# OllieBoyne/FIND

Hardware: AMD Instinct MI355X
Metric: deformed vertices x rendered views / sec (fwd+bwd) (higher is better)
Workload: dtype f32; 1 GPU; train_3d.yaml network-stage step: 16 feet x 6890-vertex template per GPU, 10002-vertex GT scans, chamf(5000)+smooth+texture(1000) losses, backward, Adam(main_params) step; nothing rendered, views:=1; feet_per_gpu=16, template_verts=6890, parallelism=dp1

## Files before the change

find_amd/_lib.py:

```python
import ctypes
import os
from ctypes import POINTER, Structure, c_char_p, c_float, c_int, c_int16, c_int32, c_int64, c_void_p

_PKG = os.path.dirname(os.path.abspath(__file__))
LIB_PATH = os.path.join(_PKG, 'lib', 'libfind_hip.so')
MAX_LAYERS = 8
ABI_VERSION = 3

_lib = None


class MlpParams(Structure):
	_fields_ = [
		('width', c_int32), ('in_dim', c_int32), ('pe_size', c_int32), ('n_trunk', c_int32),
		('n_disp', c_int32), ('n_col', c_int32), ('lat_disp', c_int32), ('lat_col', c_int32),
		('B', c_void_p),
		('trunk_w', c_void_p * MAX_LAYERS), ('trunk_b', c_void_p * MAX_LAYERS),
		('disp_w', c_void_p * MAX_LAYERS), ('disp_b', c_void_p * MAX_LAYERS),
		('col_w', c_void_p * MAX_LAYERS), ('col_b', c_void_p * MAX_LAYERS),
		('avg_col', c_void_p),
		('precision', c_int32),
	]


class MlpGrads(Structure):
	_fields_ = [
		('trunk_w', c_void_p * MAX_LAYERS), ('trunk_b', c_void_p * MAX_LAYERS),
		('disp_w', c_void_p * MAX_LAYERS), ('disp_b', c_void_p * MAX_LAYERS),
		('col_w', c_void_p * MAX_LAYERS), ('col_b', c_void_p * MAX_LAYERS),
		('lat_disp', c_void_p), ('lat_col', c_void_p),
	]


class RenderParams(Structure):
	_fields_ = [
		('image_h', c_int32), ('image_w', c_int32), ('fov_deg', c_float), ('znear', c_float), ('zfar', c_float),
		('sil_blur_radius', c_float), ('sil_sigma', c_float), ('sil_faces_per_pixel', c_int16), ('clip_faces', c_int16),
		('rgb_sigma', c_float), ('rgb_gamma', c_float), ('background', c_float * 3), ('light_pos', c_float * 3),
		('ambient', c_float), ('diffuse', c_float), ('specular', c_float), ('shininess', c_float), ('z_clip', c_float),
	]


class PointsParams(Structure):
	_fields_ = [('image_h', c_int32), ('image_w', c_int32), ('fov_deg', c_float), ('radius', c_float), ('points_per_pixel', c_int32)]


_P = c_void_p
_I = c_int64
PROTOTYPES = {
	'find_abi_version': (c_int, []),
	'find_last_error': (c_char_p, []),
	'find_build_arch': (c_char_p, []),
	'find_ctx_create': (c_int, [c_int, POINTER(c_void_p)]),
	'find_ctx_destroy': (c_int, [_P]),
	'find_ctx_stream_groups': (c_int, [_P, _P, _P]),
	'find_ctx_stream_beside': (c_int, [_P, _P, _P, c_int32, c_int32, _P]),
	'find_ctx_set': (c_int, [_P, c_char_p, _I]),
	'find_ctx_get': (c_int, [_P, c_char_p, POINTER(c_int64)]),
	'find_ctx_join': (c_int, [_P, _P]),
	'find_render_switches': (c_int, [_I]),
	'find_mlp_ws_bytes': (c_int64, [POINTER(MlpParams), _I, _I, _I, c_int]),
	'find_mlp_fwd': (c_int, [_P, POINTER(MlpParams), _P, _I, _I, _I, _P, _P, _P, _P, _P, _I, c_int, _P]),
	'find_mlp_bwd_scratch_bytes': (c_int64, [POINTER(MlpParams), _I, _I, _I]),
	'find_mlp_bwd': (c_int, [_P, POINTER(MlpParams), _P, _I, _I, _I, _P, _P, _P, _P, _P, _I, _P, _I, POINTER(MlpGrads), _P]),
	'find_linear_relu_fwd': (c_int, [_P, _P, _P, _P, _I, _I, _P, _P]),
	'find_linear_wgrad_scratch_bytes': (c_int64, [_I]),
	'find_linear_wgrad': (c_int, [_P, _P, _P, _I, _I, _P, _P, _P, _I, _P]),
	'find_latent_gather_fwd': (c_int, [_P, _I, _I, _P, _I, _P, _P]),
	'find_latent_gather_bwd': (c_int, [_P, _P, _I, _I, _I, _P, _P]),
	'find_latent_gather_many_fwd': (c_int, [_I, _P, _P, _P, _P, _I, _P, _P]),
	'find_latent_gather_many_bwd': (c_int, [_I, _P, _P, _P, _P, _I, _P, _P]),
	'find_weighted_terms_fwd': (c_int, [_I, _P, _P, _P, _P, _P]),
	'find_weighted_terms_bwd': (c_int, [_I, _P, _P, _P, _P, _P]),
	'find_contrastive_fwd': (c_int, [_P, _I, _I, _P, _I, _P, _I, c_float, _P, _P, _P]),
	'find_contrastive_bwd': (c_int, [_P, _I, _I, _P, _I, _P, _P, _P, _P]),
	'find_part_labels': (c_int, [_P, _I, _I, _I, _I, _I, _I, _P, _P]),
	'find_part_ce_fwd': (c_int, [_P, _P, _P, _I, _I, _P, _P, _P, _I, _P]),
	'find_part_ce_bwd': (c_int, [_P, _P, _P, _I, _I, _P, _P, _P, _I, _P]),
	'find_vertex_normals_fwd': (c_int, [_P, _P, _I, _P, _P, _I, _I, _I, _P, _P]),
	'find_vertex_normals_bwd': (c_int, [_P, _P, _I, _P, _P, _I, _I, _I, _P, _P, _P, _P]),
	'find_normal_map_fwd': (c_int, [_P, _P, _I, _I, _I, _I, c_int, _P, _P]),
	'find_normal_map_bwd': (c_int, [_P, _P, _P, _I, _I, _I, _I, c_int, _P, _P]),
	'find_normal_loss_ws_bytes': (c_int64, [_I]),
	'find_normal_loss_fwd': (c_int, [_P, _P, _P, _I, _P, _P, _I, _P]),
	'find_normal_loss_bwd': (c_int, [_P, _P, _P, _I, _P, _P, _P, _P]),
	'find_point_face_ws_bytes': (c_int64, [_I, _I]),
	'find_point_face_fwd': (c_int, [_P, _P, _P, _P, _I, _I, _I, _I, _I, _P, _P, _P, _P, _I, _P]),
	'find_point_face_bwd': (c_int, [_P, _P, _P, _I, _P, _P, _P, _I, _I, _I, _I, _P, _P, _P]),
	'find_uv_sample': (c_int, [_P, _I, _I, _I, _P, _I, _P, _I, _I, _P, _P, _I, _I, _P, _P]),
	'find_render_frags': (c_int, [POINTER(RenderParams), _I, _I, _I, _I, _P, _P, _P, _P]),
	'find_adam_step': (c_int, [_I, _P, _P, _P, _P, _P, c_float, c_float, c_float, c_float, c_float, _I, _P]),
	'find_adam_step_dev': (c_int, [_I, _P, _P, _P, _P, _P, c_float, c_float, c_float, c_float, c_float, _P, _P]),
	'find_sgd_step': (c_int, [_I, _P, _P, _P, _P, c_float, c_float, c_float, c_float, c_int, c_int, _P]),
	'find_register_fwd': (c_int, [_P, _I, _P, _P, _I, _I, _P, _P]),
	'find_register_bwd_ws_bytes': (c_int64, [_I, _I]),
	'find_register_bwd': (c_int, [_P, _I, _P, _P, _P, _I, _I, _P, _P, _P, _I, _P]),
	'find_pca_fwd': (c_int, [_P, _I, _I, _P, _I, _P, _P]),
	'find_pca_bwd_ws_bytes': (c_int64, [_I, _I, _I]),
	'find_pca_bwd': (c_int, [_P, _I, _I, _P, _I, _P, _P, _I, _P]),
	'find_sample_points_fwd': (c_int, [_P, _P, _I, _P, _P, _I, _I, _I, _I, _P, _P, _P, _P]),
	'find_sample_points_bwd': (c_int, [_P, _I, _P, _P, _P, _I, _I, _I, _I, _P, _P]),
	'find_face_areas': (c_int, [_P, _P, _I, _I, _I, _I, _P, _P]),
	'find_nn_fwd': (c_int, [_P, _P, _P, _P, _I, _I, _I, _P, _P, _P]),
	'find_nn_bwd': (c_int, [_P, _P, _P, _P, _P, _I, _I, _I, _P, _P, _P]),
	'find_sample_surface_ws_bytes': (c_int64, [_I, _I]),
	'find_sample_surface_fwd': (c_int, [_P, _P, _I, _P, _I, _I, _I, _I, _P, _P, _P, _P, _P, _P, _I, _P]),
	'find_sample_surface_again': (c_int, [_P, _P, _I, _P, _I, _I, _I, _I, _P, _P, _P, _P, _P, _P, _I, _P]),
	'find_chamfer_ws_bytes': (c_int64, [_I, _I, _I]),
	'find_chamfer_fwd': (c_int, [_P, _P, _P, _P, _I, _I, _I, _P, _P, _I, _P]),
	'find_chamfer_bwd': (c_int, [_P, _P, _P, _P, _I, _I, _I, _P, _P, _I, _P, _P, _P]),
	'find_masked_mse_fwd': (c_int, [_P, _P, _I, _P, _P]),
	'find_masked_mse_bwd': (c_int, [_P, _P, _I, _P, _P, _P]),
	'find_image_mse_ws_bytes': (c_int64, []),
	'find_image_mse_fwd': (c_int, [_P, _P, _P, _P, _I, _I, _P, _P, _I, _P]),
	'find_image_mse_bwd': (c_int, [_P, _P, _P, _P, _I, _I, _P, _P, _P, _P]),
	'find_image_metrics_ws_bytes': (c_int64, [_I, _I]),
	'find_image_metrics': (c_int, [_P, _P, _P, _P, _P, _P, _I, _I, _I, _P, _P, _I, _P]),
	'find_smooth_loss_fwd': (c_int, [_P, _P, _P, _P, _P, _P, _I, _I, _I, _I, c_float, c_float, _P, _P, _I, _P]),
	'find_smooth_loss_bwd': (c_int, [_P, _P, _P, _P, _P, _P, _I, _I, _I, _I, c_float, c_float, _P, _P, _I, _P, _P]),
	'find_smooth_ws_bytes': (c_int64, [_I, _I, _I]),
	'find_smooth_fwd': (c_int, [_P, _P, _P, _P, _P, _P, _I, _I, _I, _I, _P, _P, _P, _I, _P]),
	'find_smooth_bwd': (c_int, [_P, _P, _P, _P, _P, _P, _I, _I, _I, _I, _P, _P, _P, _I, _P, _P]),
	'find_render_ws_bytes': (c_int64, [POINTER(RenderParams), _I, _I, _I, _I]),
	'find_render_fwd': (c_int, [POINTER(RenderParams), _P, _P, _I, _P, _P, _P, _I, _I, _I, _I, _P, _P, _P, _P, _P, _I, _P]),
	'find_render_bwd': (c_int, [POINTER(RenderParams), _P, _P, _I, _P, _P, _P, _I, _I, _I, _I, _P, _P, _P, _P, _P, _P, _I, _P]),
	'find_render_flags': (c_int, [_P, _P, _P]),
	'find_render_features_ws_bytes': (c_int64, [POINTER(RenderParams), _I, _I, _I]),
	'find_render_features_fwd': (c_int, [POINTER(RenderParams), _P, _P, _I, _P, _P, _I, _I, _I, _I, _P, _I, _P, _P, _I, _P, _I, _P]),
	'find_render_features_bwd': (c_int, [POINTER(RenderParams), _P, _P, _I, _P, _P, _I, _I, _I, _I, _P, _I, _P, _P, _P, _P, _P, _I, _P, _I, _P]),
	'find_points_render': (c_int, [POINTER(PointsParams), _P, _P, _P, _P, _I, _I, _I, _P, _P, _P, _P, _P]),
	'find_frames_u8': (c_int, [_P, _I, _I, _I, _I, c_int, _P, _P]),
}


def lib():
	global _lib
	if _lib is not None:
		return _lib
	if not os.path.exists(LIB_PATH):
		raise RuntimeError(f'find_amd: HIP library not built: {LIB_PATH} is missing. Run `python -m find_amd.build` '
						   '(or __graft_entry__.build()). There is no CPU fallback.')
	import torch
	L = ctypes.CDLL(LIB_PATH)
	for name, (res, args) in PROTOTYPES.items():
		try:
			fn = getattr(L, name)
		except AttributeError as e:
# ... 91 lines not shown
```

find_amd/csrc/mlp.hip:

```cpp
#include "mlp_dw2.h"
#include "mlp_dw4.h"
#include "mlp_dwpe.h"
#include "mlp_dwpe6.h"
#include "mlp_gemm5.h"
#include "mlp_gemm6.h"
#include "mlp_gemm7.h"
#include "mlp_dw3.h"
#include "mlp_dw6.h"
#include "mlp_gemm4.h"
#include "mlp_fused.h"
#include "mlp_fused6.h"
#include "mlp_ctx.h"

namespace find {
namespace mlp {

struct Dims {
	int64_t pos_batch, n_feet, V;
	bool shared;
	int64_t rows_t;
	int64_t rows_h;
	int64_t feet_t;
	int nchunk0;
	int nkt0;
// ... 43 lines not shown

static int64_t chain_w6_bytes(const find_mlp_params* p) {
	const int64_t steps = 2 * (KP0 / KC + 1) + 16 * (int64_t)(p->n_trunk + p->n_disp + p->n_col + 4);
	return 8 * steps * F6_STEP_BYTES;
}

struct FwdWs {
	float* w0p;
	float* wd0;
	float* wc0;
	float* fbd;
	float* fbc;
	float* H[FIND_MAX_LAYERS];
	float* D[FIND_MAX_LAYERS];
	float* C[FIND_MAX_LAYERS];
	float* zd;
	float* zc;
	float* hp;
	float* hp2;
	void* w6;
	int64_t bytes;
};

static void carve_fwd(const find_mlp_params* p, const Dims& d, bool save, void* ws, FwdWs* o) {
	Carver c(ws);
	o->w0p = c.take<float>((int64_t)W * KP0);
	o->wd0 = c.take<float>((int64_t)W * W);
	o->wc0 = c.take<float>((int64_t)W * W);
	o->fbd = c.take<float>(d.n_feet * W);
	o->fbc = c.take<float>(d.n_feet * W);
	o->zd = c.take<float>(d.rows_h * 3);
	o->zc = c.take<float>(d.rows_h * 3);
	o->hp = (d.shared && d.n_feet > 1) ? c.take<float>(d.V * W) : nullptr;
	o->hp2 = (d.shared && d.n_feet > 1) ? c.take<float>(d.V * W) : nullptr;
	o->w6 = c.take<char>(chain_w6_bytes(p));
	float* pt[2] = {nullptr, nullptr};
	float* pd[2] = {nullptr, nullptr};
	float* pc[2] = {nullptr, nullptr};
	for (int i = 0; i < p->n_trunk; ++i) {
		if (save || !pt[i & 1]) pt[i & 1] = c.take<float>(d.rows_t * W);
		o->H[i] = pt[i & 1];
	}
	for (int i = 0; i < p->n_disp; ++i) {
		if (save || !pd[i & 1]) pd[i & 1] = c.take<float>(d.rows_h * W);
		o->D[i] = pd[i & 1];
	}
	for (int i = 0; i < p->n_col; ++i) {
		if (save || !pc[i & 1]) pc[i & 1] = c.take<float>(d.rows_h * W);
		o->C[i] = pc[i & 1];
	}
	o->bytes = c.off;
}

static void split_policy(int64_t n_feet, int64_t V, int* spf, int* cps, int64_t target = 128) {
	const int64_t cpf = cdiv(V, 32);
	int64_t s0 = std::max<int64_t>(1, std::min<int64_t>(cpf, cdiv(target, n_feet)));
	*cps = (int)cdiv(cpf, s0);
	*spf = (int)cdiv(cpf, *cps);
}

struct BwdWs {
	float* Tt[FIND_MAX_LAYERS];
	float* Dt[FIND_MAX_LAYERS];
	float* Ct[FIND_MAX_LAYERS];
	float* dzD[FIND_MAX_LAYERS];
	float* dzC[FIND_MAX_LAYERS];
	float* dzT[FIND_MAX_LAYERS];
	float* pw;
	float* pb;
	float* pw_t[4];
	float* pb_t[4];
	float* Sd;
	float* Sc;
	float* zsD;
	float* zsC;
	float* fs1D;
	float* fs1C;
	float* pS;
	float* pS2;
	int nblk_fs;
	float* pwo[2];
	float* pbo[2];
	int nblk_out;
	int64_t max_split;
	float* grp_pw;
	int64_t grp_slabs;
	int grp_jobs;
	void* w6;
	int64_t bytes;
};

constexpr int64_t GROUP_MAX_UNITS = 1024;
constexpr int GROUP_MIN_CPS = 8;

static void carve_bwd(const find_mlp_params* p, const Dims& d, void* scratch, BwdWs* o) {
	Carver c(scratch);
	for (int i = 1; i < p->n_trunk; ++i) o->Tt[i] = c.take<float>((int64_t)W * W);
	for (int i = 0; i < p->n_disp; ++i) o->Dt[i] = c.take<float>((int64_t)W * W);
	for (int i = 0; i < p->n_col; ++i) o->Ct[i] = c.take<float>((int64_t)W * W);
	for (int i = 0; i < std::max(p->n_disp, 1); ++i) o->dzD[i] = c.take<float>(d.rows_h * W);
	for (int i = 0; i < std::max(p->n_col, 1); ++i) o->dzC[i] = c.take<float>(d.rows_h * W);
	for (int i = 0; i < std::max(p->n_trunk, 1); ++i) o->dzT[i] = c.take<float>(d.rows_t * W);
	int spf, cps;
	split_policy(d.n_feet, d.V, &spf, &cps);
	int64_t ms = d.n_feet * spf;
	split_policy(1, d.V, &spf, &cps);
	ms = std::max<int64_t>(ms, spf);
	o->max_split = ms;
	const int64_t ms2 = std::max<int64_t>(512, d.n_feet) + d.n_feet + 16;
	o->pw = c.take<float>(std::max<int64_t>(ms * W * KP0, ms2 * W * W));
	o->pb = c.take<float>(std::max<int64_t>(ms, ms2) * W);
	o->pw_t[0] = o->pw; o->pb_t[0] = o->pb;
	for (int i = 1; i < 4; ++i) {
		o->pw_t[i] = c.take<float>(ms2 * W * W);
		o->pb_t[i] = c.take<float>(ms2 * W);
	}
	o->Sd = c.take<float>(d.n_feet * W);
	o->Sc = c.take<float>(d.n_feet * W);
	o->nblk_fs = (int)cdiv(d.V, FS_ROWS);
	if (d.shared) {
		o->zsD = c.take<float>(d.V * W);
		o->zsC = c.take<float>(d.V * W);
		o->fs1D = c.take<float>(d.V * W);
		o->fs1C = c.take<float>(d.V * W);
	} else {
		o->zsD = o->zsC = o->fs1D = o->fs1C = nullptr;
	}
	o->pS = c.take<float>((int64_t)o->nblk_fs * d.n_feet * W);
	o->pS2 = c.take<float>((int64_t)o->nblk_fs * d.n_feet * W);
	o->w6 = c.take<char>(chain_w6_bytes(p));
	o->grp_pw = nullptr; o->grp_slabs = 0; o->grp_jobs = 0;
	if (cdiv(d.V, 32) * d.feet_t <= GROUP_MAX_UNITS) {
		o->grp_jobs = d.shared ? (p->n_trunk - 1) + 2 : (p->n_trunk - 1) + p->n_disp + p->n_col;
		o->grp_slabs = std::max<int64_t>(d.feet_t * (cdiv(d.V / 16, GROUP_MIN_CPS) + 1), std::min<int64_t>(d.feet_t * cdiv(d.V / 16, 2), 32));
		if (o->grp_jobs > 0) o->grp_pw = c.take<float>((int64_t)o->grp_jobs * o->grp_slabs * ((int64_t)W * W + W));
	}
	o->nblk_out = (int)std::max<int64_t>(1, std::min<int64_t>(cdiv(d.rows_h, 64), 512));
	for (int i = 0; i < 2; ++i) {
		o->pwo[i] = c.take<float>((int64_t)o->nblk_out * 3 * W);
		o->pbo[i] = c.take<float>((int64_t)o->nblk_out * 4);
	}
	o->bytes = c.off;
}

struct TileLaunch { int id; int lds; int rows; int grid; int block; };

static int ntiles_of(int64_t V, int rows, int64_t feet) { return (int)((int)cdiv(V, rows) * feet); }

template <typename K>
static int launch_tiles(find_ctx* c, K kernel, const TileLaunch& t, Gemm2Args a, int64_t feet, hipStream_t s) {
	int lds = 0;
	FIND_TRY(prepare_kernel(c, t.id, kernel, t.lds, &lds));
	a.tiles_per_foot = (int)cdiv(a.V, t.rows);
	a.ntiles = (int)(a.tiles_per_foot * feet);
	hipLaunchKernelGGL(kernel, dim3(t.grid), dim3(t.block), lds, s, a);
	return FIND_OK;
}

template <typename F>
static int with_epi(int epi, F&& f) {
	if (epi == EPI_BIAS_RELU) return f(std::integral_constant<int, EPI_BIAS_RELU>{});
	if (epi == EPI_MASK) return f(std::integral_constant<int, EPI_MASK>{});
	return f(std::integral_constant<int, EPI_NONE>{});
}
constexpr int epi_slot(int epi) { return epi == EPI_BIAS_RELU ? 0 : epi == EPI_MASK ? 1 : 2; }

static int launch_gemm2_pe(find_ctx* c, const Gemm2Args& a, int64_t feet, hipStream_t s) {
	constexpr int BM = 64;
	const int grid = std::min(ntiles_of(a.V, BM, feet), c->num_cus);
	return launch_tiles(c, &gemm2_kernel<BM, AMODE_PE, EPI_BIAS_RELU>, TileLaunch{K_GEMM2_PE, gemm2_lds_bytes<BM>(), BM, grid, 256}, a, feet, s);
}

static int launch_gemm3(find_ctx* c, int epi, const Gemm2Args& a, int64_t feet, hipStream_t s) {
	return with_epi(epi, [&](auto E) -> int {
		constexpr int EPI = decltype(E)::value, BM = 64;
		const int grid = std::min(ntiles_of(a.V, BM, feet), c->num_cus);
		return launch_tiles(c, &gemm3_kernel<BM, EPI>, TileLaunch{K_GEMM3_RELU + epi_slot(EPI), gemm2_lds_bytes<BM>(), BM, grid, 256}, a, feet, s);
	});
}

template <int NI>
static int launch_gemm4(find_ctx* c, int epi, const Gemm2Args& a, int64_t feet, hipStream_t s) {
	return with_epi(epi, [&](auto E) -> int {
		constexpr int EPI = decltype(E)::value, NW = 8;
		constexpr int G = 8 * (8 / NI);
		const int grid = std::max(G, (c->num_cus / G) * G);
		const int id = (NI == 4 ? K_GEMM4_4_RELU : K_GEMM4_2_RELU) + epi_slot(EPI);
		return launch_tiles(c, &gemm4_kernel<EPI, NI, NW>, TileLaunch{id, NI * 32 * 1024, 32, grid, NW * 64}, a, feet, s);
	});
}

static int launch_gemm5(find_ctx* c, int epi, const Gemm2Args& a, int64_t feet, hipStream_t s, bool h16) {
	return with_epi(epi, [&](auto E) -> int {
		constexpr int EPI = decltype(E)::value;
		const int grid = (int)std::min<int64_t>(c->num_cus, cdiv(ntiles_of(a.V, 32, feet), GEMM5_NW));
		const int block = GEMM5_NW * 64;
		if constexpr (EPI != EPI_NONE) {
			if (h16 && (EPI == EPI_BIAS_RELU ? a.va_bias : a.vm_bias)) {
				Gemm2Args v = a;
				v.tile_major = 1;
				return launch_tiles(c, &gemm5_kernel<EPI, true, true>, TileLaunch{EPI == EPI_BIAS_RELU ? K_GEMM5_RELU_V : K_GEMM5_MASK_V, GEMM5_LDS_VIRT, 32, grid, block}, v, feet, s);
			}
			if (h16) return launch_tiles(c, &gemm5_kernel<EPI, true>, TileLaunch{EPI == EPI_BIAS_RELU ? K_GEMM5_RELU_H : K_GEMM5_MASK_H, GEMM5_LDS, 32, grid, block}, a, feet, s);
		} else if (h16) {
			set_error("launch_gemm5: no fp16-stored variant of this epilogue");
			return FIND_EINVAL;
		}
		return launch_tiles(c, &gemm5_kernel<EPI>, TileLaunch{K_GEMM5_RELU + epi_slot(EPI), GEMM5_LDS, 32, grid, block}, a, feet, s);
	});
}

static int gemm7_fsum_pairs(const find_ctx* c, int64_t V, int64_t feet) {
	const int64_t upf = cdiv(V, 32);
	const int def = std::max(16, (c->num_cus / 16) * 16) / 2;
	const int pairs = (int)std::min<int64_t>(def, (upf / 8) * 8);
	return (feet >= 2 && feet <= 64 && pairs >= 8) ? pairs : 0;
}

static int launch_gemm7(find_ctx* c, int epi, const Gemm2Args& a, int64_t feet, hipStream_t s) {
	return with_epi(epi, [&](auto E) -> int {
		constexpr int EPI = decltype(E)::value;
		const int grid = std::max(16, (c->num_cus / 16) * 16);
		const int block = GEMM7_NW * 64;
		if constexpr (EPI == EPI_MASK) {
// ... 62 lines not shown
		SplitWArgs sa;
		memset(&sa, 0, sizeof(sa));
		int maxn = 0;
		for (int i = 0; i < ch.a.n_steps; ++i) {
			const FusedStep& st = ch.a.step[i];
			if (st.kind != FS_GEMM) continue;
			const int n = 2 * st.nchunk;
			sa.job[sa.njobs++] = SplitWJob{st.w, st.ldw, n, sa.total, st.wmode, ch.a.pe, ch.in_dim};
			sa.total += n;
			maxn = std::max(maxn, n);
		}
		if (sa.njobs > 0 && 8 * (int64_t)sa.total * F6_STEP_BYTES <= w6_bytes) {
			sa.dst = reinterpret_cast<u32x4*>(w6);
			hipLaunchKernelGGL(split_w_kernel, dim3((unsigned)cdiv(8 * maxn * 64, 256), (unsigned)sa.njobs), dim3(256), 0, s, sa);
			FIND_LAUNCH_CHECK("split_w_kernel");
			ch.a.w6 = w6;
			ch.a.total_steps = sa.total;
			ch.x3 = true;
		}
	}
	if (!ch.x3)
		for (int i = 0; i < ch.a.n_steps; ++i)
			FIND_REQUIRE(ch.a.step[i].kind != FS_GEMM || ch.a.step[i].wmode == 0, "find_mlp: a chain with weights in model order did not get its bf16x3 kernel (chain_direct and chain_prepare disagree)");
	return FIND_OK;
}

static int chain_launch(find_ctx* c, Chain& ch, hipStream_t s) {
	const int nt = ch.nt;
	int lds = 0;
	if (ch.x3) {
		if (nt == 2) FIND_TRY(prepare_kernel(c, K_FUSED6_2, &fused6_kernel<2>, fused6_lds(2), &lds, false));
		else FIND_TRY(prepare_kernel(c, K_FUSED6, &fused6_kernel<1>, fused6_lds(1), &lds, false));
		if (nt == 2) hipLaunchKernelGGL(fused6_kernel<2>, dim3(ch.a.ntiles), dim3(FUSED_NW * 64), lds, s, ch.a);
		else hipLaunchKernelGGL(fused6_kernel<1>, dim3(ch.a.ntiles), dim3(FUSED_NW * 64), lds, s, ch.a);
		FIND_LAUNCH_CHECK("fused6_kernel");
		return FIND_OK;
	}
	const int grid = std::min(ch.a.ntiles, c->num_cus);
	if (nt == 2) FIND_TRY(prepare_kernel(c, K_FUSED2, &fused_chain_kernel<2>, fused_lds(2), &lds, false));
	else FIND_TRY(prepare_kernel(c, K_FUSED, &fused_chain_kernel<1>, fused_lds(1), &lds, false));
	if (nt == 2) hipLaunchKernelGGL(fused_chain_kernel<2>, dim3(grid), dim3(FUSED_NW * 64), lds, s, ch.a);
	else hipLaunchKernelGGL(fused_chain_kernel<1>, dim3(grid), dim3(FUSED_NW * 64), lds, s, ch.a);
	FIND_LAUNCH_CHECK("fused_chain_kernel");
	return FIND_OK;
}

static int launch_chain(find_ctx* c, Chain& ch, int64_t V, int64_t feet, hipStream_t s, void* w6 = nullptr, int64_t w6_bytes = 0) {
	if (!ch.prepared) FIND_TRY(chain_prepare(c, ch, V, feet, s, w6, w6_bytes));
	return chain_launch(c, ch, s);
}

static bool use_fused(const find_ctx* c, int64_t V, int64_t feet) {
	const int64_t units = cdiv(V, 32) * feet;
	if (c->f16 && units >= c->gemm5_min_units) return false;
	return c->fused_max_units > 0 && units <= c->fused_max_units;
}

static Gemm2Args gemm_args() {
	Gemm2Args a;
	memset(&a, 0, sizeof(a));
	a.nseg = 1;
	return a;
}

static Gemm2Args linear_args(const float* x, int64_t x_foot_stride, const float* w, int ldw, const float* bias, int64_t bias_foot_stride, float* y, int64_t V) {
	Gemm2Args a = gemm_args();
	a.a0 = x; a.a_foot_stride = x_foot_stride; a.lda = W;
	a.w0 = w; a.ldw = ldw; a.nchunk = W / KC;
	a.bias = bias; a.bias_foot_stride = bias_foot_stride;
	a.y = y; a.y_foot_stride = V * W; a.ldy = W; a.V = (int)V;
	return a;
}

static bool use_act16(const find_ctx* c, bool f16, bool shared, int64_t n_feet, int64_t V) {
	return f16 && c->act16 && shared && n_feet > 1 && cdiv(V, 32) * n_feet >= c->gemm5_min_units;
}
static bool use_fold(const find_ctx* c, bool a16, bool shared, int64_t n_feet, int64_t V, const find_mlp_params* p) {
	if (!c->bcast_fold || p->n_disp < 2 || p->n_col < 2) return false;
	if (a16) return true;
	const int64_t units = cdiv(V, 32) * n_feet;
	return c->x3 && !c->f16 && shared && n_feet > 1 && units >= c->gemm6_min_units;
}
static void note_act16(find_ctx* c, const void* ws, bool a16, bool fold) {
	for (auto& n : c->act16_notes) if (n.ws == ws) { n.a16 = a16; n.fold = fold; return; }
	c->act16_notes[c->act16_next] = find_ctx::Act16Note{ws, a16, fold};
	c->act16_next = (c->act16_next + 1) & 15;
}
static int noted_act16(const find_ctx* c, const void* ws, bool by_rule, bool fold_by_rule) {
	for (const auto& n : c->act16_notes) if (n.ws == ws) return (n.a16 ? 1 : 0) | (n.fold ? 2 : 0);
	return (by_rule ? 1 : 0) | (fold_by_rule ? 2 : 0);
}

static bool call_f16(const find_ctx* c, const find_mlp_params* p) { return p->precision == 2 || (p->precision == 0 && c->mlp_f16 == 1); }
static bool call_x3(const find_ctx* c, const find_mlp_params* p) { return p->precision == 3 || (p->precision == 0 && c->mlp_f16 == 2); }

struct Head {
	bool colour;
	int nl;
	const float* const* w;
	const float* const* b;
	int ld0;
	int L;
	const float* lat;
	const float* w0; int ldw0;
	float* fb;
	const float* bias0; int64_t bstride0;
	float* const* act;
	float* z;
	float* hp;
	float* out;
	const float* gout;
	float* const* gw; float* const* gb; float* glat;
	float* const* dz; int cur;
	float* const* wt;
	float* S; float* zs; float* fs1; float* pS;
	int side;
};

static void make_heads(Head* heads, const find_mlp_params* p, const FwdWs& w, const float* lat_disp, const float* lat_col, const BwdWs* b, const find_mlp_grads* g) {
	memset(heads, 0, 2 * sizeof(Head));
	Head& d = heads[0];
	Head& c = heads[1];
	c.colour = true;
	d.nl = p->n_disp; c.nl = p->n_col;
	d.w = p->disp_w; c.w = p->col_w;
	d.b = p->disp_b; c.b = p->col_b;
	d.L = p->lat_disp; c.L = p->lat_col;
	d.lat = lat_disp; c.lat = lat_col;
	d.w0 = w.wd0; c.w0 = w.wc0;
	d.fb = w.fbd; c.fb = w.fbc;
	d.act = w.D; c.act = w.C;
	d.z = w.zd; c.z = w.zc;
	d.hp = w.hp; c.hp = w.hp2;
	for (int k = 0; k < 2; ++k) {
		Head& h = heads[k];
		h.ld0 = W + h.L;
		h.ldw0 = W;
		h.bias0 = h.L > 0 ? h.fb : h.b[0];
		h.bstride0 = h.L > 0 ? W : 0;
		h.side = 1 + k;
	}
	if (!b) return;
	d.gw = g->disp_w; c.gw = g->col_w;
	d.gb = g->disp_b; c.gb = g->col_b;
	d.glat = g->lat_disp; c.glat = g->lat_col;
	d.dz = b->dzD; c.dz = b->dzC;
	d.wt = b->Dt; c.wt = b->Ct;
	d.S = b->Sd; c.S = b->Sc;
	d.zs = b->zsD; c.zs = b->zsC;
	d.fs1 = b->fs1D; c.fs1 = b->fs1C;
	d.pS = b->pS; c.pS = b->pS2;
}

static int mlp_fwd_body(Fork& fk, const find_mlp_params* p, const Dims& d, const FwdWs& w, const float* pos, Head* heads) {
	find_ctx* c = fk.c;
	hipStream_t s = fk.s;
	const int64_t V = d.V, n_feet = d.n_feet;
	Head& hd = heads[0];
	Head& hc = heads[1];
	const bool a16 = use_act16(c, c->f16, d.shared, n_feet, V);
	const bool fold = use_fold(c, a16, d.shared, n_feet, V, p);
	note_act16(c, w.fbd, a16, fold);

	const bool fused = use_fused(c, V, d.feet_t) && p->pe_size > 0;
	const bool direct = fused && chain_direct(c);
	if (!direct) {
		RepackArgs ra;
		memset(&ra, 0, sizeof(ra));
		ra.njobs = 3;
		ra.job[0] = RepackJob{p->trunk_w[0], w.w0p, W, KP0, p->in_dim + 2 * p->pe_size, 0, KP0, 2, p->pe_size, p->in_dim};
		ra.job[1] = RepackJob{hd.w[0], w.wd0, W, W, hd.ld0, 0, W, 0, 0, 0};
		ra.job[2] = RepackJob{hc.w[0], w.wc0, W, W, hc.ld0, 0, W, 0, 0, 0};
		hipLaunchKernelGGL(repack_kernel, dim3(96, ra.njobs), dim3(256), 0, s, ra);
		FIND_LAUNCH_CHECK("repack_kernel");
	} else {
		for (int k = 0; k < 2; ++k) { heads[k].w0 = heads[k].w[0]; heads[k].ldw0 = heads[k].ld0; }
	}
	for (int k = 0; k < 2; ++k) {
		const Head& h = heads[k];
		if (h.L > 0 && h.out != nullptr)
			hipLaunchKernelGGL(latent_bias_kernel, dim3(W / 4, (unsigned)n_feet), dim3(256), 0, s, h.w[0], h.ld0, h.b[0], h.lat, h.L, h.fb);
	}
	FIND_LAUNCH_CHECK("latent_bias_kernel");

	const bool forked = hd.out && hc.out && fk.on;
	if (!(fold || forked || (fused && hd.out))) hc.hp = w.hp;

	const bool fused_heads = fused && !(d.shared && n_feet > 1);
	if (fused) {
		Chain ch;
		ch.a.pos = pos; ch.a.pos_foot_stride = V * 3; ch.a.Bm = p->B; ch.a.pe = p->pe_size; ch.in_dim = p->in_dim;
		{
			FusedStep& s0 = direct ? ch.gemm(p->trunk_w[0], p->in_dim + 2 * p->pe_size, (d.nchunk0 + 1) & ~1) : ch.gemm(w.w0p, KP0, (d.nchunk0 + 1) & ~1);
			s0.wmode = direct ? 2 : 0;
			s0.src_kind = FS_SRC_PE; s0.relu = 1; s0.bias = p->trunk_b[0]; s0.dst = w.H[0]; s0.to_lds = 1;
		}
		for (int i = 1; i < p->n_trunk; ++i) {
			FusedStep& st = ch.gemm(p->trunk_w[i], W, W / KC);
			st.relu = 1; st.bias = p->trunk_b[i]; st.dst = w.H[i]; st.to_lds = 1;
		}
		const float* hlast = w.H[p->n_trunk - 1];
		if (!fused_heads) {
			for (int k = 0; k < 2; ++k)
				if (heads[k].out) { FusedStep& st = ch.gemm(heads[k].w0, heads[k].ldw0, W / KC); st.dst = heads[k].hp; }
		} else {
			auto head = [&](const Head& h, bool reload) {
				FusedStep& f0 = ch.gemm(h.w0, h.ldw0, W / KC, reload ? hlast : nullptr);
				f0.relu = 1; f0.bias = h.bias0; f0.bias_foot_stride = (int)h.bstride0; f0.dst = h.act[0]; f0.to_lds = 1;
				for (int i = 1; i < h.nl; ++i) {
					FusedStep& st = ch.gemm(h.w[i], W, W / KC);
					st.relu = 1; st.bias = h.b[i]; st.dst = h.act[i]; st.to_lds = 1;
				}
				FusedStep& o = ch.add();
				o.kind = FS_OUT; o.w = h.w[h.nl]; o.bias = h.b[h.nl]; o.dst = h.out; o.dst2 = h.z; o.head = (unsigned char)h.colour;
				o.aux = h.colour ? p->avg_col : nullptr;
			};
			if (hd.out) head(hd, false);
			if (hc.out) head(hc, hd.out != nullptr);
		}
		FIND_TRY(launch_chain(c, ch, V, d.feet_t, s, w.w6, chain_w6_bytes(p)));
		if (fused_heads) return FIND_OK;
	} else {
		Gemm2Args a = gemm_args();
		a.pos = pos; a.pos_foot_stride = V * 3; a.Bm = p->B; a.pe = p->pe_size;
		a.w0 = w.w0p; a.ldw = KP0; a.nchunk = d.nchunk0;
		a.bias = p->trunk_b[0]; a.bias_foot_stride = 0;
		a.y = w.H[0]; a.y_foot_stride = V * W; a.ldy = W; a.V = (int)V;
		FIND_TRY(launch_gemm(c, AMODE_PE, EPI_BIAS_RELU, a, d.feet_t, s));
		for (int i = 1; i < p->n_trunk; ++i)
			FIND_TRY(launch_gemm(c, AMODE_MAT, EPI_BIAS_RELU, linear_args(w.H[i - 1], V * W, p->trunk_w[i], W, p->trunk_b[i], 0, w.H[i], V), d.feet_t, s));
		FIND_LAUNCH_CHECK("trunk gemm");
	}

	const float* hl = w.H[p->n_trunk - 1];
	const int64_t hl_stride = d.shared ? 0 : V * W;
	auto head_first = [&](const Head& h, hipStream_t st) -> int {
		if (h.hp) {
			if (!fused) {
				Gemm2Args a = gemm_args();
				a.a0 = hl; a.a_foot_stride = 0; a.lda = W;
				a.w0 = h.w0; a.ldw = W; a.nchunk = W / KC;
				a.y = h.hp; a.y_foot_stride = V * W; a.ldy = W; a.V = (int)V;
				FIND_TRY(launch_gemm(c, AMODE_MAT, EPI_NONE, a, 1, st));
			}
			if (fold) return FIND_OK;
			hipLaunchKernelGGL(bias_relu_bcast_kernel, dim3((unsigned)cdiv(V * (W / 4), 256), (unsigned)cdiv(n_feet, BCAST_FEET)), dim3(256), 0, st, h.hp, h.bias0,
							   h.bstride0, (int)n_feet, V, h.act[0], a16 ? 1 : 0);
			return FIND_OK;
		}
		FIND_REQUIRE(!a16, "find_mlp_fwd: act16 without a shared template");
		return launch_gemm(c, AMODE_MAT, EPI_BIAS_RELU, linear_args(hl, hl_stride, h.w0, W, h.bias0, h.bstride0, h.act[0], V), n_feet, st);
	};
	auto head_out = [&](int head, hipStream_t st) {
		HeadOutArgs h;
		memset(&h, 0, sizeof(h));
		for (int k = 0; k < 2; ++k) {
			h.x[k] = heads[k].act[heads[k].nl - 1];
			h.w[k] = heads[k].w[heads[k].nl];
			h.b[k] = heads[k].b[heads[k].nl];
			h.z[k] = heads[k].z;
			h.out[k] = heads[k].out;
		}
		h.avg_col = p->avg_col;
		h.rows = d.rows_h;
		h.head0 = head;
		h.x_half = a16 ? 1 : 0;
		const unsigned gx = (unsigned)std::min<int64_t>(cdiv(d.rows_h, 32), 2048);
		if (a16) hipLaunchKernelGGL(head_out_fwd_h16_kernel, dim3(gx, 1), dim3(256), 0, st, h);
		else hipLaunchKernelGGL(head_out_fwd_kernel, dim3(gx, 1), dim3(256), 0, st, h);
	};
	auto head = [&](const Head& h, hipStream_t st) -> int {
		FIND_TRY(head_first(h, st));
		for (int i = 1; i < h.nl; ++i) {
			Gemm2Args a = linear_args(h.act[i - 1], V * W, h.w[i], W, h.b[i], 0, h.act[i], V);
			if (i == 1 && fold) {
				a.a0 = h.hp; a.a_foot_stride = 0;
				a.va_bias = h.bias0; a.va_bias_stride = h.bstride0;
			}
			FIND_TRY(launch_gemm(c, AMODE_MAT, EPI_BIAS_RELU, a, n_feet, st, a16));
		}
		head_out(h.colour, st);
		return FIND_OK;
	};
	hipStream_t sc = s;
	if (forked) {
		fk.fork_to(1);
		sc = fk.stream(1);
	}
	if (hd.out) FIND_TRY(head(hd, s));
	if (hc.out) FIND_TRY(head(hc, sc));
	FIND_LAUNCH_CHECK("head layers");
	return FIND_OK;
}

struct Wgrad {
	const float* dz = nullptr;
	const float* x = nullptr;
	int64_t x_foot_stride = 0;
	const float* pos = nullptr;
	int64_t pos_foot_stride = 0;
	int nkt = 1;
	int64_t feet = 1, V = 0;
	float* dw = nullptr;
	int ld_out = W;
	int k_valid = W;
	int pe_map = 0;
	float* db = nullptr;
	float* S = nullptr;
	hipStream_t s = nullptr;
	int s_side = -1;
	int reduce_side = -1;
	bool h16 = false;
	const float* vx_bias = nullptr;
	int64_t vx_bias_stride = 0;
};

struct Slabs { float* pw; float* pb; };
static Slabs slabs(const BwdWs& b, int k) { return Slabs{b.pw_t[k], b.pb_t[k]}; }

static int reduce_lds(find_ctx* c) {
	if (c->reduce_exclusive != 1) return 0;
	const int dyn = c->lds_bytes - 16 * 1024 - 256;
	if (!c->attr_done[K_REDUCE]) {
		if (hipFuncSetAttribute(reinterpret_cast<const void*>(&reduce_w_kernel), hipFuncAttributeMaxDynamicSharedMemorySize, dyn) != hipSuccess) return 0;
		c->attr_done[K_REDUCE] = true;
	}
	return dyn;
}

static int launch_reduce(find_ctx* c, const ReduceWArgs& r, hipStream_t s) {
	const unsigned grid = (unsigned)(r.nwblk + (r.pb ? r.n_feet + 1 : 0));
	if (c->reduce_exclusive == 2) hipLaunchKernelGGL(reduce_w_nolds_kernel, dim3(grid), dim3(1024), 0, s, r);
	else hipLaunchKernelGGL(reduce_w_kernel, dim3(grid), dim3(1024), reduce_lds(c), s, r);
	FIND_LAUNCH_CHECK("reduce_w_kernel");
	return FIND_OK;
}

static int weight_grad(find_ctx* c, Fork* fk, const find_mlp_params* p, const Wgrad& in, Slabs sl) {
	const int64_t feet = in.feet, V = in.V;
	hipStream_t s = in.s;
	FIND_REQUIRE(!in.vx_bias || (!in.pos && ((in.h16 && c->f16) || (!c->f16 && c->x3 && cdiv(V, 32) * feet >= c->gemm6_min_units))),
				 "weight_grad: a virtual operand reached a kernel that cannot form it (bcast_fold and the kernel selection disagree)");
	float* pbuf = (in.db || in.S) ? sl.pb : nullptr;
	const int cus = c->num_cus;
	int nsplit, spf, Kp = 256;
	if (!in.pos) {
		auto dw3_args = [&](int cpf, int cps) {
			Dw3Args a;
			memset(&a, 0, sizeof(a));
			a.dz = in.dz; a.dz_foot_stride = V * W; a.x = in.x; a.x_foot_stride = in.x_foot_stride;
			a.V = (int)V; a.chunks_per_foot = cpf; a.spf = spf; a.cps = cps; a.pw = sl.pw; a.pb = pbuf;
			a.xbias = in.vx_bias; a.xbias_stride = in.vx_bias_stride;
// ... 76 lines not shown
	memset(&r, 0, sizeof(r));
	r.pw = sl.pw; r.nsplit = nsplit; r.Kp = Kp; r.out = in.dw; r.ld_out = in.ld_out; r.K_valid = in.k_valid;
	if (in.pos) { r.pe_map = in.pe_map; r.pe = p->pe_size; r.in_dim = p->in_dim; }
	r.pb = pbuf; r.n_feet = (int)feet; r.spf = spf; r.db = in.db; r.S = in.S;
	r.nwblk = 256 * Kp / 4 / 64;
	hipStream_t rs = s;
	if (fk && fk->on && in.reduce_side >= 0 && in.s_side >= 0 && in.reduce_side != in.s_side) {
		fk->chain(in.s_side, in.reduce_side);
		rs = fk->stream(in.reduce_side);
	}
	return launch_reduce(c, r, rs);
}

struct WgradGroup {
	Dw2Group d;
	Dw6Group d6;
	bool x3 = false;
	ReduceWGroup r;
	int n = 0, nmain = 0;
	int live_jobs = 0;
	int64_t feet = 0;
	WgradGroup() { memset(&d, 0, sizeof(d)); memset(&d6, 0, sizeof(d6)); memset(&r, 0, sizeof(r)); }
};

static void group_geometry(const find_ctx* c, int cpf16, int64_t feet, int jobs, int64_t max_slabs, int* spf_out, int* cps_out) {
	auto take = [&](int s) { *cps_out = (int)cdiv(cpf16, s); *spf_out = (int)cdiv(cpf16, *cps_out); };
	const int s_max = (int)std::max<int64_t>(1, std::min<int64_t>(cpf16, max_slabs / std::max<int64_t>(feet, 1)));
	double best = 1e30;
	take(1);
	for (int s = 1; s <= s_max; ++s) {
		const int cps = (int)cdiv(cpf16, s);
		if ((int)cdiv(cpf16, cps) != s || (cps < 2 && s > 1)) continue;
		const int64_t wgs = feet * s * std::max(jobs, 1);
		const double cost = (double)cdiv(wgs, c->num_cus) * (cps * 3.6 + 6.0) + wgs * 0.06;
		if (cost < best) { best = cost; take(s); }
	}
}

static int wgrad_group_add(find_ctx* c, WgradGroup& G, const BwdWs& b, const Wgrad& in) {
	FIND_REQUIRE(G.n < b.grp_jobs && G.n < DW2_MAX_JOBS && G.n < DW6_MAX_JOBS, "find_mlp_bwd: too many grouped weight gradients");
	const int64_t feet = in.feet, V = in.V;
	G.x3 = c->x3 && c->dw_lds_free == 1;
	const int cpf16 = G.x3 ? (int)cdiv(V, 16) : (int)(V / 16);
	int spf = 1, cps2 = 1;
	if (cpf16 > 0) group_geometry(c, cpf16, feet, G.live_jobs > 0 ? G.live_jobs : b.grp_jobs, b.grp_slabs, &spf, &cps2);
	const int nmain = (int)(feet * spf);
	FIND_REQUIRE(nmain <= b.grp_slabs, "find_mlp_bwd: grouped weight gradient needs %d slabs, %lld reserved", nmain, (long long)b.grp_slabs);
	float* pw = b.grp_pw + (int64_t)G.n * b.grp_slabs * W * W;
	float* pb = b.grp_pw + (int64_t)b.grp_jobs * b.grp_slabs * W * W + (int64_t)G.n * b.grp_slabs * W;
	Dw2Args& d2 = G.d.job[G.n];
	d2.dz = in.dz; d2.dz_foot_stride = V * W; d2.x = in.x; d2.x_foot_stride = in.x_foot_stride;
	d2.chunks_per_foot = cpf16; d2.tail_rows = (int)(V % 16); d2.spf = spf; d2.cps = cps2; d2.pw = pw; d2.pb = (in.db || in.S) ? pb : nullptr;
	Dw3Args& d6 = G.d6.job[G.n];
	d6.dz = in.dz; d6.dz_foot_stride = V * W; d6.x = in.x; d6.x_foot_stride = in.x_foot_stride;
	d6.V = (int)V; d6.chunks_per_foot = cpf16; d6.spf = spf; d6.cps = cps2; d6.pw = pw; d6.pb = d2.pb;
	ReduceWArgs& r = G.r.job[G.n];
	r.pw = pw; r.nsplit = nmain; r.Kp = 256; r.out = in.dw; r.ld_out = in.ld_out; r.K_valid = W;
	r.pb = d2.pb; r.n_feet = (int)feet; r.spf = spf; r.db = in.db; r.S = in.S;
	r.nwblk = 256 * 256 / 4 / 64;
	G.nmain = nmain; G.feet = feet;
	G.n += 1;
	return FIND_OK;
}

static int wgrad_group_launch(find_ctx* c, WgradGroup& G, hipStream_t s) {
	if (G.n == 0) return FIND_OK;
	if (G.x3) {
		int lds = 0;
		FIND_TRY(prepare_kernel(c, K_DW6G, &dw6_group_kernel, DW6_LDS, &lds));
		hipLaunchKernelGGL(dw6_group_kernel, dim3((unsigned)G.nmain, (unsigned)G.n), dim3(256), lds, s, G.d6);
	} else if (c->dw_lds_free == 1) {
		hipLaunchKernelGGL(dw4_group_kernel, dim3((unsigned)G.nmain, (unsigned)G.n), dim3(512), 0, s, G.d);
	} else {
		int lds = 0;
		FIND_TRY(prepare_kernel(c, K_DW2G, &dw2_group_kernel, DW2_LDS, &lds));
		hipLaunchKernelGGL(dw2_group_kernel, dim3((unsigned)G.nmain, (unsigned)G.n), dim3(256), lds, s, G.d);
	}
	FIND_LAUNCH_CHECK("grouped weight-gradient kernel");
	hipLaunchKernelGGL(reduce_w_group_kernel, dim3((unsigned)(256 * 256 / 4 / 64 + (int)G.feet + 1), (unsigned)G.n), dim3(1024), 0, s, G.r);
	FIND_LAUNCH_CHECK("reduce_w_group_kernel");
	return FIND_OK;
}

static int mlp_bwd_body(Fork& fk, const find_mlp_params* p, const Dims& d, const FwdWs& w, const BwdWs& b, const float* pos, Head* heads, const find_mlp_grads* g) {
	find_ctx* c = fk.c;
	hipStream_t s = fk.s;
	const bool defer = fk.deferring;
	const int64_t V = d.V, n_feet = d.n_feet;
	const int K0 = p->in_dim + 2 * p->pe_size;
	Head& hd = heads[0];
	Head& hc = heads[1];
	const bool act_d = hd.gout != nullptr, act_c = hc.gout != nullptr;
	const bool frozen = g->trunk_w[0] == nullptr;
	enum { Q = 0, T1 = 1, T2 = 2, R = 3 };

	ZeroArgs za;
	memset(&za, 0, sizeof(za));
	int mrc = FIND_OK;
	auto zero = [&](float* ptr, int64_t n) {
		if (!ptr || n <= 0) return;
		if (za.njobs == ZERO_MAX_JOBS) { hipLaunchKernelGGL(zero_many_kernel, dim3(32, za.njobs), dim3(256), 0, s, za); za.njobs = 0; }
		za.p[za.njobs] = ptr; za.n[za.njobs] = n; za.njobs += 1;
	};
	auto zero_flush = [&]() {
		if (za.njobs > 0) hipLaunchKernelGGL(zero_many_kernel, dim3(32, za.njobs), dim3(256), 0, s, za);
		za.njobs = 0;
		if (hipGetLastError() != hipSuccess) { set_error("find_mlp_bwd: zero_many_kernel launch failed"); mrc = FIND_ELAUNCH; }
	};
	for (int k = 0; k < 2; ++k) {
		const Head& h = heads[k];
		if (h.gout) continue;
		zero(h.gw[0], (int64_t)W * h.ld0); zero(h.gb[0], W);
		for (int i = 1; i < h.nl; ++i) { zero(h.gw[i], (int64_t)W * W); zero(h.gb[i], W); }
		zero(h.gw[h.nl], 3 * W); zero(h.gb[h.nl], 3);
		if (h.L) zero(h.glat, n_feet * h.L);
	}
	if (!act_d && !act_c) {
		zero(g->trunk_w[0], (int64_t)W * K0); zero(g->trunk_b[0], W);
		for (int i = 1; i < p->n_trunk; ++i) { zero(g->trunk_w[i], (int64_t)W * W); zero(g->trunk_b[i], W); }
		zero_flush();
		return mrc;
	}
	zero_flush();
	if (mrc != FIND_OK) return mrc;

	const bool fused = use_fused(c, V, d.feet_t) && p->pe_size > 0;
	const bool small_chain = fused && !d.shared;
	const bool t_heads = !(small_chain ? chain_direct(c) : gemm7_direct(c, V, n_feet));
	const bool t_trunk = !(fused ? chain_direct(c) : gemm7_direct(c, V, d.feet_t));
	const bool t_first = !(fused && chain_direct(c));
	struct WT { const float* w; int ld; int tr; };
	auto wt_of = [&](bool need_t, const float* orig, int ld_orig, const float* transposed) -> WT { return need_t ? WT{transposed, W, 0} : WT{orig, ld_orig, 1}; };
	auto wt_H = [&](const Head& h, int l) -> WT { return l == 0 ? wt_of(t_first, h.w[0], h.ld0, h.wt[0]) : wt_of(t_heads, h.w[l], W, h.wt[l]); };
	auto wt_T = [&](int l) -> WT { return wt_of(t_trunk, p->trunk_w[l], W, b.Tt[l]); };
	{
		RepackArgs ra;
		memset(&ra, 0, sizeof(ra));
		int n = 0;
		if (!frozen) {
			if (t_trunk) for (int i = 1; i < p->n_trunk; ++i) ra.job[n++] = RepackJob{p->trunk_w[i], b.Tt[i], W, W, W, 0, W, 1, 0, 0};
			if (t_first) for (int k = 0; k < 2; ++k) ra.job[n++] = RepackJob{heads[k].w[0], heads[k].wt[0], W, W, heads[k].ld0, 0, W, 1, 0, 0};
		}
		if (t_heads)
			for (int k = 0; k < 2; ++k)
				for (int i = 1; i < heads[k].nl; ++i) ra.job[n++] = RepackJob{heads[k].w[i], heads[k].wt[i], W, W, W, 0, W, 1, 0, 0};
		ra.njobs = n;
		if (n > 0) hipLaunchKernelGGL(repack_kernel, dim3(64, n), dim3(256), 0, s, ra);
		FIND_LAUNCH_CHECK("repack_kernel(T)");
	}

	const bool a16_rule = use_act16(c, c->f16, d.shared, n_feet, V);
	const int note16 = noted_act16(c, w.fbd, a16_rule, use_fold(c, a16_rule, d.shared, n_feet, V, p));
	const bool a16 = (note16 & 1) != 0;
	const bool fold = (note16 & 2) != 0;
	struct Virt { const float* P; const float* bias; int64_t bstride; };
	auto virt = [&](const Head& h, int l) -> Virt {
		if (!fold || l != 1) return Virt{nullptr, nullptr, 0};
		return Virt{h.hp, h.bias0, h.bstride0};
	};
	{
		HeadOutBwdArgs h;
		memset(&h, 0, sizeof(h));
		HeadOutReduceArgs hr;
		memset(&hr, 0, sizeof(hr));
		for (int k = 0; k < 2; ++k) {
			const Head& hk = heads[k];
			h.y[k] = hk.act[hk.nl - 1];
			h.w[k] = hk.w[hk.nl];
			h.z[k] = hk.z;
			h.gout[k] = hk.gout;
			h.dy[k] = hk.dz[hk.cur];
			h.pw[k] = b.pwo[k]; h.pb[k] = b.pbo[k];
			hr.pw[k] = b.pwo[k]; hr.pb[k] = b.pbo[k];
			hr.dw[k] = hk.gout ? hk.gw[hk.nl] : nullptr; hr.db[k] = hk.gb[hk.nl];
		}
		h.rows = d.rows_h;
		h.half = a16 ? 1 : 0;
		hipLaunchKernelGGL(head_out_bwd_kernel, dim3((unsigned)b.nblk_out, 2), dim3(256), 0, s, h);
		hr.nblk = b.nblk_out;
		if (!frozen) {
			fk.fork_to(T2);
			hipLaunchKernelGGL(head_out_reduce_kernel, dim3(12, 2), dim3(1024), 0, fk.stream(T2), hr);
		}
		FIND_LAUNCH_CHECK("head_out_bwd");
	}

	const float* hl = w.H[p->n_trunk - 1];
	const int64_t hl_stride = d.shared ? 0 : V * W;

	auto head_chain = [&](Chain& ch, Head& h) {
		for (int l = h.nl - 1; l >= 1; --l) {
			const WT t = wt_H(h, l);
			FusedStep& st = ch.gemm(t.w, t.ld, W / KC, h.cur == 0 ? h.dz[0] : nullptr);
			st.wmode = (unsigned char)t.tr;
			st.mask = 1; st.aux = h.act[l - 1]; st.dst = h.dz[h.cur + 1]; st.to_lds = 1;
			h.cur += 1;
		}
	};
	auto trunk_out_steps = [&](Chain& ch, const float* dz_d, const float* dz_c) {
		const float* A[2]; WT Wt[2]; int nb = 0;
		if (act_d) { A[nb] = dz_d; Wt[nb] = wt_H(hd, 0); ++nb; }
		if (act_c) { A[nb] = dz_c; Wt[nb] = wt_H(hc, 0); ++nb; }
		for (int i = 0; i < nb; ++i) {
			FusedStep& st = ch.gemm(Wt[i].w, Wt[i].ld, W / KC, A[i]);
			st.wmode = (unsigned char)Wt[i].tr;
			st.accum = i > 0;
			if (i + 1 < nb) { st.keep = 1; continue; }
			st.mask = 1; st.aux = hl; st.dst = b.dzT[0]; st.to_lds = 1;
		}
	};
	auto trunk_steps = [&](Chain& ch) {
		for (int l = p->n_trunk - 1; l >= 1; --l) {
			const WT t = wt_T(l);
			FusedStep& st = ch.gemm(t.w, t.ld, W / KC);
			st.wmode = (unsigned char)t.tr;
			st.mask = 1; st.aux = w.H[l - 1]; st.dst = b.dzT[p->n_trunk - l]; st.to_lds = 1;
		}
	};
	auto dx_args = [&](const float* dz, const WT& t, const float* mask, float* y, const Virt& v) {
		Gemm2Args a = gemm_args();
		a.a0 = dz; a.a_foot_stride = V * W; a.lda = W;
		a.w0 = t.w; a.ldw = t.ld; a.w_tr = t.tr; a.nchunk = W / KC;
		a.mask = mask; a.mask_foot_stride = v.bias ? 0 : V * W;
		a.vm_bias = v.bias; a.vm_bias_stride = v.bstride;
		a.y = y; a.y_foot_stride = V * W; a.ldy = W; a.V = (int)V;
		return a;
	};
	auto layer_wgrad = [&](const float* dz, const float* x, int64_t x_foot_stride, int64_t feet, float* dw, float* db) {
		Wgrad wg;
		wg.dz = dz; wg.x = x; wg.x_foot_stride = x_foot_stride; wg.feet = feet; wg.V = V; wg.dw = dw; wg.db = db;
		return wg;
	};
	auto fourier_wgrad = [&](const float* dz, int side, int set) -> int {
		Wgrad wg;
		wg.dz = dz; wg.pos = pos; wg.pos_foot_stride = V * 3; wg.nkt = d.nkt0; wg.feet = d.feet_t; wg.V = V;
		wg.dw = g->trunk_w[0]; wg.ld_out = K0; wg.k_valid = 0; wg.pe_map = 1; wg.db = g->trunk_b[0];
		wg.s = fk.stream(side);
		return weight_grad(c, &fk, p, wg, slabs(b, set));
	};
	auto foot_partials = [&](const Head& h, float* zs) {
		hipLaunchKernelGGL(footsum_kernel, dim3((unsigned)b.nblk_fs * 4), dim3(256), 0, s, h.dz[h.cur], (int)n_feet, (int)V, zs, h.pS, a16 ? 1 : 0);
	};
	auto foot_reduce = [&](const Head& h, int nblk, hipStream_t st) {
		hipLaunchKernelGGL(footsum_reduce_kernel, dim3((unsigned)n_feet, 4), dim3(1024), 0, st, h.pS, nblk, (int)n_feet, h.S);
	};
	auto latent_grad = [&](const Head& h, float* gw0, float* db_late, hipStream_t st) {
		hipLaunchKernelGGL(latent_grad_kernel, dim3((unsigned)(n_feet + (gw0 ? W : 0) + (db_late ? 1 : 0))), dim3(256), 0, st, h.w[0], h.ld0, h.lat, h.L, h.S, (int)n_feet,
						   h.glat, gw0, db_late);
	};

	Chain tch;
	if (fused && !frozen && d.shared) {
		trunk_out_steps(tch, hd.zs, hc.zs);
		trunk_steps(tch);
		FIND_TRY(chain_prepare(c, tch, V, d.feet_t, s, b.w6, chain_w6_bytes(p)));
	}
	if (frozen) {
		auto want = [&](const Head& h) { return h.gout && h.L > 0 && h.glat != nullptr; };
		if (!want(hd) && !want(hc)) return FIND_OK;
		if (small_chain) {
			Chain ch;
			if (want(hc)) head_chain(ch, hc);
			if (want(hd)) head_chain(ch, hd);
			if (ch.a.n_steps > 0) FIND_TRY(launch_chain(c, ch, V, d.feet_t, s, b.w6, chain_w6_bytes(p)));
		} else {
			for (int k = 0; k < 2; ++k) {
				Head& h = heads[k];
				if (!want(h)) continue;
				for (int l = h.nl - 1; l >= 1; --l) {
					const Virt v = virt(h, l);
					FIND_TRY(launch_gemm(c, AMODE_MAT, EPI_MASK, dx_args(h.dz[h.cur], wt_H(h, l), v.P ? v.P : h.act[l - 1], h.dz[h.cur + 1], v), n_feet, s, a16));
					h.cur += 1;
				}
			}
		}
		for (int k = 0; k < 2; ++k) {
			const Head& h = heads[k];
			if (!want(h)) continue;
			foot_partials(h, nullptr);
			foot_reduce(h, b.nblk_fs, s);
			latent_grad(h, nullptr, nullptr, s);
			FIND_LAUNCH_CHECK("latent gradients of a frozen network");
		}
		return FIND_OK;
	}
	if (small_chain) {
		Chain ch;
		if (act_c) head_chain(ch, hc);
		if (act_d) head_chain(ch, hd);
		trunk_out_steps(ch, hd.dz[hd.cur], hc.dz[hc.cur]);
		trunk_steps(ch);
		FIND_TRY(launch_chain(c, ch, V, d.feet_t, s, b.w6, chain_w6_bytes(p)));
		const bool grouped = !c->f16 && b.grp_pw != nullptr;
		WgradGroup G;
		G.live_jobs = (act_d ? p->n_disp : 0) + (act_c ? p->n_col : 0) + (p->n_trunk - 1);
		int rr = 0;
		auto one = [&](Wgrad wg) -> int {
			if (grouped) return wgrad_group_add(c, G, b, wg);
			const int k = fk.on ? 1 + rr % 2 : 0;
			rr += 1;
			fk.fork_to(k);
			wg.s = fk.stream(k);
			return weight_grad(c, &fk, p, wg, slabs(b, k));
		};
		const Head* lats[2]; int nlat = 0;
		auto head_wgrads = [&](const Head& h) -> int {
			for (int l = h.nl - 1; l >= 1; --l) FIND_TRY(one(layer_wgrad(h.dz[h.nl - 1 - l], h.act[l - 1], V * W, n_feet, h.gw[l], h.gb[l])));
			if (defer && h.L > 0) {
				foot_partials(h, nullptr);
				foot_reduce(h, b.nblk_fs, s);
				latent_grad(h, h.gw[0], nullptr, s);
				FIND_LAUNCH_CHECK("latent gradients (deferred join)");
			}
			Wgrad wg = layer_wgrad(h.dz[h.cur], hl, hl_stride, n_feet, h.gw[0], h.gb[0]);
			wg.ld_out = h.ld0;
			wg.S = (h.L > 0 && !defer) ? h.S : nullptr;
			FIND_TRY(one(wg));
			if (h.L > 0 && !defer) lats[nlat++] = &h;
			return FIND_OK;
		};
		if (act_d) FIND_TRY(head_wgrads(hd));
		if (act_c) FIND_TRY(head_wgrads(hc));
		for (int l = p->n_trunk - 1; l >= 1; --l)
			FIND_TRY(one(layer_wgrad(b.dzT[p->n_trunk - 1 - l], w.H[l - 1], V * W, d.feet_t, g->trunk_w[l], g->trunk_b[l])));
		hipStream_t sl = s;
		if (grouped) {
			fk.fork_to(1);
			sl = fk.stream(1);
			FIND_TRY(wgrad_group_launch(c, G, sl));
		} else if (fk.on) {
			fk.chain(2, 1);
			sl = fk.stream(1);
		}
		for (int i = 0; i < nlat; ++i) {
			latent_grad(*lats[i], lats[i]->gw[0], nullptr, sl);
			FIND_LAUNCH_CHECK("latent_grad_kernel");
		}
		{
			const int k = fk.on ? 2 : 0;
			fk.fork_to(k);
			FIND_TRY(fourier_wgrad(b.dzT[p->n_trunk - 1], k, 0));
// ... 49 lines not shown
			Wgrad wg = layer_wgrad(h.zs, hl, 0, 1, h.gw[0], nullptr);
			wg.ld_out = h.ld0;
			wg.s = q0;
			if (grouped_v) FIND_TRY(wgrad_group_add(c, G, b, wg));
			else FIND_TRY(weight_grad(c, &fk, p, wg, slabs(b, h.side)));
		} else {
			fk.fork_to(Q);
			q0 = fk.stream(Q);
			fk.wait(Q, set_free[0]);
			Wgrad wg = layer_wgrad(h.dz[h.cur], hl, hl_stride, n_feet, h.gw[0], h.gb[0]);
			wg.ld_out = h.ld0;
			wg.S = (h.L > 0) ? h.S : nullptr;
			wg.s = q0;
			FIND_TRY(weight_grad(c, &fk, p, wg, slabs(b, 0)));
		}
		if (h.L > 0) {
			latent_grad(h, h.gw[0], db_late, q0);
			FIND_LAUNCH_CHECK("latent_grad_kernel");
		}
		return FIND_OK;
	};
	if (act_d) FIND_TRY(head_bwd(hd));
	if (act_c) FIND_TRY(head_bwd(hc));

	auto trunk_wgrad = [&](int l, const float* dz) -> int {
		Wgrad wg = layer_wgrad(dz, w.H[l - 1], V * W, d.feet_t, g->trunk_w[l], g->trunk_b[l]);
		if (grouped_v) return wgrad_group_add(c, G, b, wg);
		const int k = fk.on ? 1 + (l & 1) : 0;
		fk.fork_to(k);
		wg.s = fk.stream(k);
		return weight_grad(c, &fk, p, wg, slabs(b, k));
	};
	int ct = 0;
	if (fused) {
		FIND_TRY(launch_chain(c, tch, V, d.feet_t, s, b.w6, chain_w6_bytes(p)));
		for (int l = p->n_trunk - 1; l >= 1; --l, ++ct) FIND_TRY(trunk_wgrad(l, b.dzT[ct]));
		if (grouped_v) {
			fk.fork_to(T1);
			FIND_TRY(wgrad_group_launch(c, G, fk.stream(T1)));
		}
	} else {
		{
			Gemm2Args a = gemm_args();
			const float* A[2]; const float* Wt[2]; int nb = 0;
			if (act_d) { A[nb] = d.shared ? hd.zs : hd.dz[hd.cur]; Wt[nb] = hd.wt[0]; ++nb; }
			if (act_c) { A[nb] = d.shared ? hc.zs : hc.dz[hc.cur]; Wt[nb] = hc.wt[0]; ++nb; }
			a.nseg = nb; a.a0 = A[0]; a.w0 = Wt[0];
			if (nb > 1) { a.a1 = A[1]; a.w1 = Wt[1]; }
			a.lda = W; a.ldw = W; a.nchunk = W / KC;
			a.a_foot_stride = d.shared ? 0 : V * W;
			a.mask = hl; a.mask_foot_stride = V * W;
			a.y = b.dzT[ct]; a.y_foot_stride = V * W; a.ldy = W; a.V = (int)V;
			FIND_TRY(launch_gemm(c, AMODE_MAT, EPI_MASK, a, d.feet_t, s));
			FIND_LAUNCH_CHECK("trunk-out dX gemm");
		}
		for (int l = p->n_trunk - 1; l >= 1; --l, ++ct) {
			FIND_TRY(trunk_wgrad(l, b.dzT[ct]));
			FIND_TRY(launch_gemm(c, AMODE_MAT, EPI_MASK, dx_args(b.dzT[ct], wt_T(l), w.H[l - 1], b.dzT[ct + 1], Virt{nullptr, nullptr, 0}), d.feet_t, s));
		}
	}
	if (fused && d.shared && fk.on) {
		fk.fork_to(T2);
		FIND_TRY(fourier_wgrad(b.dzT[ct], T2, T2));
	} else {
		fk.fork_to(Q);
		fk.wait(Q, set_free[0]);
		FIND_TRY(fourier_wgrad(b.dzT[ct], Q, 0));
	}
	FIND_LAUNCH_CHECK("find_mlp_bwd");
	return FIND_OK;
}

}
}

extern "C" int64_t find_mlp_ws_bytes(const find_mlp_params* p, int64_t pos_batch, int64_t n_feet, int64_t n_pts, int save_for_bwd) {
	Dims d;
	if (make_dims(p, pos_batch, n_feet, n_pts, &d) != FIND_OK) return -1;
	FwdWs w;
	carve_fwd(p, d, save_for_bwd != 0, nullptr, &w);
	return w.bytes;
}

extern "C" int find_mlp_fwd(find_ctx* c, const find_mlp_params* p, const float* pos, int64_t pos_batch, int64_t n_feet, int64_t n_pts,
							const float* lat_disp, const float* lat_col, float* disp, float* col, void* ws,
							int64_t ws_bytes, int save_for_bwd, void* stream) {
	FIND_TRY(check_ctx(c, "find_mlp_fwd"));
	Dims d;
	FIND_TRY(make_dims(p, pos_batch, n_feet, n_pts, &d));
	FIND_TRY(check_weights(p));
	FIND_REQUIRE(pos && ws, "find_mlp_fwd: pos/ws is NULL");
	FIND_REQUIRE(disp || col, "find_mlp_fwd: both outputs NULL");
	FIND_REQUIRE(p->lat_disp == 0 ? lat_disp == nullptr : (lat_disp != nullptr || disp == nullptr), "find_mlp_fwd: lat_disp pointer does not match params.lat_disp=%d", p->lat_disp);
	FIND_REQUIRE(p->lat_col == 0 ? lat_col == nullptr : (lat_col != nullptr || col == nullptr), "find_mlp_fwd: lat_col pointer does not match params.lat_col=%d", p->lat_col);
	FIND_REQUIRE(p->precision >= 0 && p->precision <= 3, "find_mlp_fwd: params.precision must be 0 (context default), 1 (fp32 MFMA), 2 (fp16) or 3 (bf16x3), got %d", p->precision);
	FwdWs w;
	carve_fwd(p, d, save_for_bwd != 0, ws, &w);
	if (ws_bytes < w.bytes) {
		set_error("find_mlp_fwd: workspace too small (%lld < %lld)", (long long)ws_bytes, (long long)w.bytes);
		return FIND_EWORKSPACE;
	}
	c->f16 = call_f16(c, p);
	c->x3 = call_x3(c, p);
	Fork fk(c, reinterpret_cast<hipStream_t>(stream), c->fwd_streams != 0);
	Head heads[2];
	make_heads(heads, p, w, lat_disp, lat_col, nullptr, nullptr);
	heads[0].out = disp; heads[1].out = col;
	const int rc = mlp_fwd_body(fk, p, d, w, pos, heads);
	const int rj = fk.join();
	return rc != FIND_OK ? rc : rj;
}

extern "C" int find_linear_relu_fwd(find_ctx* c, const float* x, const float* w, const float* b, int64_t n_feet, int64_t n_pts, float* y, void* stream) {
	FIND_TRY(check_ctx(c, "find_linear_relu_fwd"));
	FIND_REQUIRE(x && w && b && y, "find_linear_relu_fwd: NULL argument");
	FIND_REQUIRE(n_feet >= 1 && n_pts >= 1 && n_feet < (1 << 16), "find_linear_relu_fwd: bad sizes");
	FIND_REQUIRE(aligned16(w) && aligned16(x), "find_linear_relu_fwd: x and w must be 16-byte aligned");
	c->f16 = c->mlp_f16 == 1;
	c->x3 = c->mlp_f16 == 2;
	FIND_TRY(launch_gemm(c, AMODE_MAT, EPI_BIAS_RELU, linear_args(x, n_pts * W, w, W, b, 0, y, n_pts), n_feet, reinterpret_cast<hipStream_t>(stream)));
	FIND_LAUNCH_CHECK("find_linear_relu_fwd");
	return FIND_OK;
}

static int64_t wgrad_slabs(int64_t n_feet) { return std::max<int64_t>(512, n_feet) + n_feet + 16; }

extern "C" int64_t find_linear_wgrad_scratch_bytes(int64_t n_feet) {
	if (n_feet < 1) return -1;
	return wgrad_slabs(n_feet) * ((int64_t)W * W + W) * (int64_t)sizeof(float);
}

extern "C" int find_linear_wgrad(find_ctx* c, const float* dz, const float* x, int64_t n_feet, int64_t n_pts, float* dw, float* db,
								 void* scratch, int64_t scratch_bytes, void* stream) {
	FIND_TRY(check_ctx(c, "find_linear_wgrad"));
	FIND_REQUIRE(dz && x && dw && scratch, "find_linear_wgrad: NULL argument");
	FIND_REQUIRE(n_feet >= 1 && n_pts >= 1 && n_feet < (1 << 16), "find_linear_wgrad: bad sizes");
	FIND_REQUIRE(aligned16(dz) && aligned16(x) && aligned16(scratch), "find_linear_wgrad: dz, x and scratch must be 16-byte aligned");
	if (scratch_bytes < find_linear_wgrad_scratch_bytes(n_feet)) {
		set_error("find_linear_wgrad: scratch too small (%lld < %lld)", (long long)scratch_bytes, (long long)find_linear_wgrad_scratch_bytes(n_feet));
		return FIND_EWORKSPACE;
	}
	float* const pw = static_cast<float*>(scratch);
	Wgrad wg;
	wg.dz = dz; wg.x = x; wg.x_foot_stride = n_pts * W; wg.feet = n_feet; wg.V = n_pts; wg.dw = dw; wg.db = db;
	wg.s = reinterpret_cast<hipStream_t>(stream);
	c->f16 = c->mlp_f16 == 1;
	c->x3 = c->mlp_f16 == 2;
	FIND_TRY(weight_grad(c, nullptr, nullptr, wg, Slabs{pw, pw + wgrad_slabs(n_feet) * W * W}));
	FIND_LAUNCH_CHECK("find_linear_wgrad");
	return FIND_OK;
}

extern "C" int64_t find_mlp_bwd_scratch_bytes(const find_mlp_params* p, int64_t pos_batch, int64_t n_feet, int64_t n_pts) {
	Dims d;
	if (make_dims(p, pos_batch, n_feet, n_pts, &d) != FIND_OK) return -1;
	BwdWs b;
	carve_bwd(p, d, nullptr, &b);
	return b.bytes;
}

extern "C" int find_mlp_bwd(find_ctx* c, const find_mlp_params* p, const float* pos, int64_t pos_batch, int64_t n_feet, int64_t n_pts,
							const float* lat_disp, const float* lat_col, const float* d_disp, const float* d_col,
							const void* ws, int64_t ws_bytes, void* scratch, int64_t scratch_bytes,
							const find_mlp_grads* g, void* stream) {
	FIND_TRY(check_ctx(c, "find_mlp_bwd"));
	Dims d;
	FIND_TRY(make_dims(p, pos_batch, n_feet, n_pts, &d));
	FIND_TRY(check_weights(p));
	FIND_REQUIRE(pos && ws && scratch && g, "find_mlp_bwd: NULL argument");
	FIND_REQUIRE(p->lat_disp == 0 ? lat_disp == nullptr : (lat_disp != nullptr || d_disp == nullptr), "find_mlp_bwd: lat_disp pointer does not match params");
	FIND_REQUIRE(p->lat_col == 0 ? lat_col == nullptr : (lat_col != nullptr || d_col == nullptr), "find_mlp_bwd: lat_col pointer does not match params");
	FIND_REQUIRE(p->precision >= 0 && p->precision <= 3, "find_mlp_bwd: params.precision must be 0, 1, 2 or 3 (got %d)", p->precision);
	{
		const bool frozen = g->trunk_w[0] == nullptr;
		bool ok = true;
		for (int i = 0; i < p->n_trunk; ++i) ok = ok && ((g->trunk_w[i] == nullptr) == frozen) && ((g->trunk_b[i] == nullptr) == frozen);
		for (int i = 0; i <= p->n_disp; ++i) ok = ok && (frozen ? !g->disp_w[i] && !g->disp_b[i] : (d_disp == nullptr || (g->disp_w[i] && g->disp_b[i])));
		for (int i = 0; i <= p->n_col; ++i) ok = ok && (frozen ? !g->col_w[i] && !g->col_b[i] : (d_col == nullptr || (g->col_w[i] && g->col_b[i])));
		FIND_REQUIRE(ok, "find_mlp_bwd: grads must name every weight-gradient buffer of the evaluated heads and the trunk, or none at all (frozen network)");
	}
	FwdWs w;
	carve_fwd(p, d, true, const_cast<void*>(ws), &w);
	if (ws_bytes < w.bytes) {
		set_error("find_mlp_bwd: forward workspace too small (%lld < %lld)", (long long)ws_bytes, (long long)w.bytes);
		return FIND_EWORKSPACE;
	}
	BwdWs b;
	carve_bwd(p, d, scratch, &b);
	if (scratch_bytes < b.bytes) {
		set_error("find_mlp_bwd: scratch too small (%lld < %lld)", (long long)scratch_bytes, (long long)b.bytes);
		return FIND_EWORKSPACE;
	}
	c->f16 = call_f16(c, p);
	c->x3 = call_x3(c, p);
	Fork fk(c, reinterpret_cast<hipStream_t>(stream), c->bwd_streams != 0);
	const bool defer = c->defer_join != 0 && fk.on && !fk.capturing && !d.shared && use_fused(c, d.V, d.feet_t) && p->pe_size > 0 && g->trunk_w[0] != nullptr;
	c->defer_join = 0;
	fk.deferring = defer;
	Head heads[2];
	make_heads(heads, p, w, lat_disp, lat_col, &b, g);
	heads[0].gout = d_disp; heads[1].gout = d_col;
	const int rc = mlp_bwd_body(fk, p, d, w, b, pos, heads, g);
	const int rj = (defer && rc == FIND_OK) ? fk.defer() : fk.join();
	return rc != FIND_OK ? rc : rj;
}

extern "C" int find_render_switches(int64_t bits) {
	FIND_REQUIRE(bits >= 0 && (bits & ~(int64_t)find::RASTER_SWITCHES) == 0, "find_render_switches: bits 0x%llx outside the result-preserving switches 0x%x", (unsigned long long)bits, find::RASTER_SWITCHES);
	find::g_raster_ablate = (int)bits;
	return FIND_OK;
}
```

find_amd/csrc/mlp_ctx.h:

```cpp
#pragma once
#include "mlp_kernels.h"

enum { K_GEMM2_PE = 0, K_GEMM3_RELU, K_GEMM3_MASK, K_GEMM3_NONE, K_GEMM4_4_RELU, K_GEMM4_4_MASK, K_GEMM4_4_NONE, K_GEMM4_2_RELU, K_GEMM4_2_MASK,
	   K_GEMM4_2_NONE, K_GEMM5_RELU, K_GEMM5_MASK, K_GEMM5_NONE, K_GEMM7_RELU, K_GEMM7_MASK, K_GEMM7_NONE, K_DW2, K_DW3, K_DW6, K_DW6G, K_FUSED, K_FUSED2, K_FUSED6, K_FUSED6_2, K_DW2G, K_REDUCE, K_GEMM5_RELU_H, K_GEMM5_MASK_H, K_DW3_H, K_GEMM5_RELU_V, K_GEMM5_MASK_V, K_DW3_V, K_GEMM7_RELU_V, K_GEMM7_MASK_V, K_DW6_V, K_GEMM7_MASK_VF, K_COUNT };
constexpr int N_SIDE = 4;
constexpr int N_EVENTS = 512;

struct find_ctx {
	int device = 0;
	int num_cus = 256;
	int lds_bytes = 160 * 1024;
	int ablate = 0;
	int64_t gemm4_min_units = 1024;
	int gemm4_small = 64;
	int gemm5_min_units = 1024;
	int gemm6_min_units = 1024;
	int mlp_f16 = 0;
	int fused_max_units = 512;
	int fused6 = 1;
	int dw2_min_cps = 8;
	int dw_lds_free = 1;
	int lds_exclusive = 0;
	int reduce_exclusive = 0;
	int bwd_streams = 1;
	int fwd_streams = 1;
	int reduce_stream = 0;
	int bind_streams = 1;
	int defer_join = 0;
	int act16 = 1;
	int bcast_fold = 1;
	int footsum_fold = 1;
	hipStream_t side[N_SIDE] = {nullptr, nullptr, nullptr, nullptr};
	bool side_bound = false;
	hipEvent_t ev[N_EVENTS];
	int n_events = 0;
	int next = 0;
	int events_per_call_max = 0;
	hipEvent_t pend_ev[N_SIDE] = {nullptr, nullptr, nullptr, nullptr};
	bool pend[N_SIDE] = {};
	bool attr_done[K_COUNT] = {};
	struct Act16Note { const void* ws; bool a16; bool fold; };
	Act16Note act16_notes[16] = {};
	int act16_next = 0;
	bool f16 = false;
	bool x3 = false;
};

namespace find {
namespace mlp {

#define FIND_HIP_OK(expr, what)                                                                  \
	do {                                                                                         \
		hipError_t _e = (expr);                                                                  \
		if (_e != hipSuccess) {                                                                  \
			set_error("%s: %s", what, hipGetErrorString(_e));                                    \
			return FIND_ELAUNCH;                                                                 \
		}                                                                                        \
	} while (0)

#define FIND_TRY(expr)                    \
	do {                                  \
		const int _r = (expr);            \
		if (_r != FIND_OK) return _r;     \
	} while (0)

template <typename K>
static int prepare_kernel(find_ctx* c, int id, K kernel, int need_bytes, int* launch_bytes, bool reserve = true) {
	const int want = (reserve && c->lds_exclusive) ? c->lds_bytes : need_bytes;
	if (need_bytes > c->lds_bytes) {
		set_error("find_mlp: kernel needs %d bytes of LDS, device %d grants %d per workgroup", need_bytes, c->device, c->lds_bytes);
		return FIND_EINVAL;
	}
	if (!c->attr_done[id]) {
		FIND_HIP_OK(hipFuncSetAttribute(reinterpret_cast<const void*>(kernel), hipFuncAttributeMaxDynamicSharedMemorySize, c->lds_bytes),
					"hipFuncSetAttribute(MaxDynamicSharedMemorySize)");
		c->attr_done[id] = true;
	}
	*launch_bytes = want;
	return FIND_OK;
}

static int bind_side_streams(find_ctx* c, hipStream_t caller);

struct Fork {
	find_ctx* c;
	hipStream_t s;
	bool on;
	bool capturing = false;
	bool deferring = false;
	bool used[N_SIDE] = {};
	int n_ev = 0;
	int rc = FIND_OK;

	Fork(find_ctx* ctx, hipStream_t caller, bool enable) : c(ctx), s(caller), on(enable && ctx->side[0] != nullptr) {
		hipStreamCaptureStatus st = hipStreamCaptureStatusNone;
		if (hipStreamIsCapturing(caller, &st) == hipSuccess) capturing = st != hipStreamCaptureStatusNone;
		if (on && !capturing && !ctx->side_bound && ctx->bind_streams) (void)bind_side_streams(ctx, caller);
	}
	hipStream_t stream(int k) const { return on ? c->side[k] : s; }
	void fail(hipError_t e, const char* what) {
		if (e != hipSuccess && rc == FIND_OK) {
			set_error("%s: %s", what, hipGetErrorString(e));
			rc = FIND_ELAUNCH;
		}
	}
	hipEvent_t event() {
		hipEvent_t e = c->ev[c->next];
		c->next = (c->next + 1) % N_EVENTS;
		if (++n_ev > N_EVENTS && rc == FIND_OK) {
			set_error("find_mlp: more than %d events in one call", N_EVENTS);
			rc = FIND_ELAUNCH;
		}
		return e;
	}
	void order(hipStream_t from, hipStream_t to) {
		hipEvent_t e = event();
		fail(hipEventRecord(e, from), "hipEventRecord");
		fail(hipStreamWaitEvent(to, e, 0), "hipStreamWaitEvent");
	}
	void fork_to(int k) {
		if (!on) return;
		order(s, c->side[k]);
		used[k] = true;
	}
// ... 162 lines not shown
	}
	const bool ok = rc == FIND_OK && pick[0] > 0 && pick[1] > 0 && pick[2] > 0 && pick[3] > 0;
	hipStream_t chosen[N_SIDE];
	for (int k = 0; k < N_SIDE; ++k) chosen[k] = ok ? st[pick[k]] : c->side[k];
	for (int i = 1; i < n; ++i) {
		bool keep = false;
		for (int k = 0; k < N_SIDE; ++k) keep = keep || st[i] == chosen[k];
		if (!keep) (void)hipStreamDestroy(st[i]);
	}
	for (int k = 0; k < N_SIDE; ++k) c->side[k] = chosen[k];
	return rc;
}
}
}

extern "C" int find_ctx_create(int device, find_ctx** out) {
	FIND_REQUIRE(out != nullptr, "find_ctx_create: out is NULL");
	*out = nullptr;
	int prev = 0, ndev = 0;
	FIND_HIP_OK(hipGetDeviceCount(&ndev), "hipGetDeviceCount");
	FIND_REQUIRE(device >= 0 && device < ndev, "find_ctx_create: device %d out of range (%d visible)", device, ndev);
	FIND_HIP_OK(hipGetDevice(&prev), "hipGetDevice");
	FIND_HIP_OK(hipSetDevice(device), "hipSetDevice");
	find_ctx* c = new find_ctx();
	c->device = device;
	auto fail = [&](const char* what, hipError_t e) {
		set_error("find_ctx_create: %s: %s", what, hipGetErrorString(e));
		for (int i = 0; i < c->n_events; ++i) (void)hipEventDestroy(c->ev[i]);
		for (int i = 0; i < N_SIDE; ++i) if (c->side[i]) (void)hipStreamDestroy(c->side[i]);
		delete c;
		(void)hipSetDevice(prev);
		return FIND_ELAUNCH;
	};
	hipError_t e;
	int v = 0;
	if ((e = hipDeviceGetAttribute(&v, hipDeviceAttributeMultiprocessorCount, device)) != hipSuccess) return fail("CU count", e);
	c->num_cus = v > 0 ? v : 256;
	if ((e = hipDeviceGetAttribute(&v, hipDeviceAttributeMaxSharedMemoryPerBlock, device)) != hipSuccess) return fail("LDS size", e);
	c->lds_bytes = v;
	for (int i = 0; i < N_SIDE; ++i)
		if ((e = hipStreamCreateWithFlags(&c->side[i], hipStreamNonBlocking)) != hipSuccess) return fail("hipStreamCreateWithFlags", e);
	for (c->n_events = 0; c->n_events < N_EVENTS; ++c->n_events)
		if ((e = hipEventCreateWithFlags(&c->ev[c->n_events], hipEventDisableTiming)) != hipSuccess) return fail("hipEventCreateWithFlags", e);
	for (int i = 0; i < N_SIDE; ++i)
		if ((e = hipEventCreateWithFlags(&c->pend_ev[i], hipEventDisableTiming)) != hipSuccess) return fail("hipEventCreateWithFlags", e);
	FIND_HIP_OK(hipSetDevice(prev), "hipSetDevice");
	*out = c;
	return FIND_OK;
}

extern "C" int find_ctx_destroy(find_ctx* c) {
	if (!c) return FIND_OK;
	int prev = 0;
	(void)hipGetDevice(&prev);
	(void)hipSetDevice(c->device);
	for (int i = 0; i < N_SIDE; ++i) if (c->side[i]) (void)hipStreamDestroy(c->side[i]);
	for (int i = 0; i < c->n_events; ++i) (void)hipEventDestroy(c->ev[i]);
	(void)hipSetDevice(prev);
	delete c;
	return FIND_OK;
}

namespace {
struct Knob { const char* key; int find_ctx::*field; int64_t lo, hi; };
const Knob KNOBS[] = {
	{"gemm4_small", &find_ctx::gemm4_small, 0, INT32_MAX},
	{"gemm5_min_units", &find_ctx::gemm5_min_units, 0, INT32_MAX},
	{"gemm6_min_units", &find_ctx::gemm6_min_units, 0, INT32_MAX},
	{"mlp_f16", &find_ctx::mlp_f16, 0, 2},
	{"fused_max_units", &find_ctx::fused_max_units, 0, 1024},
	{"fused6", &find_ctx::fused6, 0, 1},
	{"dw2_min_cps", &find_ctx::dw2_min_cps, 1, INT32_MAX},
	{"dw_lds_free", &find_ctx::dw_lds_free, 0, 1},
	{"lds_exclusive", &find_ctx::lds_exclusive, 0, 1},
	{"reduce_exclusive", &find_ctx::reduce_exclusive, 0, 2},
	{"bwd_streams", &find_ctx::bwd_streams, 0, 1},
	{"fwd_streams", &find_ctx::fwd_streams, 0, 1},
	{"reduce_stream", &find_ctx::reduce_stream, 0, 1},
	{"bind_streams", &find_ctx::bind_streams, 0, 1},
	{"defer_join", &find_ctx::defer_join, 0, 1},
	{"act16", &find_ctx::act16, 0, 1},
	{"bcast_fold", &find_ctx::bcast_fold, 0, 1},
	{"footsum_fold", &find_ctx::footsum_fold, 0, 1},
};
}

extern "C" int find_ctx_set(find_ctx* c, const char* key, int64_t value) {
	FIND_REQUIRE(c != nullptr && key != nullptr, "find_ctx_set: NULL argument");
	if (strcmp(key, "ablate") == 0) {
		FIND_REQUIRE(value >= 0 && value <= INT32_MAX && (value & ~(int64_t)find::MLP_SWITCHES) == 0,
		             "find_ctx_set: ablate = %lld has bits outside the result-preserving switches 0x%x", (long long)value, find::MLP_SWITCHES);
		c->ablate = (int)value;
		return FIND_OK;
	}
	if (strcmp(key, "gemm4_min_units") == 0) {
		FIND_REQUIRE(value >= 0, "find_ctx_set: gemm4_min_units must be >= 0");
		c->gemm4_min_units = value;
		return FIND_OK;
	}
	for (const Knob& k : KNOBS)
		if (strcmp(key, k.key) == 0) {
			FIND_REQUIRE(value >= k.lo && value <= k.hi, "find_ctx_set: %s = %lld out of range [%lld, %lld]", key, (long long)value, (long long)k.lo, (long long)k.hi);
			c->*(k.field) = (int)value;
			return FIND_OK;
		}
	set_error("find_ctx_set: unknown key %s", key);
	return FIND_EINVAL;
}

extern "C" int find_ctx_get(const find_ctx* c, const char* key, int64_t* value) {
	FIND_REQUIRE(c != nullptr && key != nullptr && value != nullptr, "find_ctx_get: NULL argument");
	if (strcmp(key, "num_cus") == 0) { *value = c->num_cus; return FIND_OK; }
	if (strcmp(key, "pending") == 0) { *value = (c->pend[0] || c->pend[1] || c->pend[2] || c->pend[3]) ? 1 : 0; return FIND_OK; }
	if (strcmp(key, "lds_bytes") == 0) { *value = c->lds_bytes; return FIND_OK; }
	if (strcmp(key, "device") == 0) { *value = c->device; return FIND_OK; }
	if (strcmp(key, "events_per_call_max") == 0) { *value = c->events_per_call_max; return FIND_OK; }
	if (strcmp(key, "gemm4_min_units") == 0) { *value = c->gemm4_min_units; return FIND_OK; }
	if (strcmp(key, "ablate") == 0) { *value = c->ablate; return FIND_OK; }
	for (const Knob& k : KNOBS)
		if (strcmp(key, k.key) == 0) { *value = c->*(k.field); return FIND_OK; }
	set_error("find_ctx_get: unknown key %s", key);
	return FIND_EINVAL;
}
```

find_amd/csrc/mlp_kernels.h:

```cpp
#pragma once
#include "common.h"

namespace find {
namespace mlp {

typedef float f32x16 __attribute__((ext_vector_type(16)));

#define FIND_CLAIM_WHOLE_REGISTER_FILE() asm volatile("" ::: "v255")

constexpr int W = 256;
constexpr int KC = 32;
constexpr int LDSLD = 36;
constexpr int KP0 = 768;

__device__ __forceinline__ float pe_value(int kp, int pe, float x, float y, float z, const float* Bl) {
	const int c = kp >> 5, j = kp & 31;
	const int nsc = pe >> 4;
	if (c < nsc) {
		const int f = (c >> 1) * 32 + j;
		float t = fmaf(z, Bl[2 * pe + f], fmaf(y, Bl[pe + f], x * Bl[f]));
		t = 2.0f * t;
		return (c & 1) ? cospif(t) : sinpif(t);
	}
	const int q = kp - nsc * 32;
	return q == 0 ? x : (q == 1 ? y : (q == 2 ? z : 0.0f));
}

__host__ __device__ __forceinline__ int pe_col_to_orig(int kp, int pe, int in_dim) {
	const int c = kp >> 5, j = kp & 31;
	const int nsc = pe >> 4;
	if (c < nsc) {
		const int f = (c >> 1) * 32 + j;
		return in_dim + ((c & 1) ? pe : 0) + f;
	}
	const int q = kp - nsc * 32;
	return q < in_dim ? q : -1;
}

enum { AMODE_MAT = 0, AMODE_PE = 1 };
enum { EPI_NONE = 0, EPI_BIAS_RELU = 1, EPI_MASK = 2 };

struct DwArgs {
	const float* dz;
	int64_t dz_foot_stride;
	const float* x;
	int64_t x_foot_stride;
	int ldx;
	const float* pos;
	int64_t pos_foot_stride;
	const float* Bm;
	int pe;
	int V;
	int spf;
	int cps;
	int v_begin;
	int Kp;
	float* pw;
	float* pb;
	int all_blocks;
};

template <int AMODE>
__global__ __launch_bounds__(512) void dw_kernel(const DwArgs g) {
	__shared__ __attribute__((aligned(16))) float Zs[32 * 256];
	__shared__ __attribute__((aligned(16))) float Xs[32 * 256];
	__shared__ float Bl[(AMODE == AMODE_PE) ? 3 * 256 : 4];

	const int tid = threadIdx.x;
	const int lane = tid & 63;
	const int wave = tid >> 6;
	const int wn = wave >> 2;
	const int wk = wave & 3;
	const int kt = blockIdx.x;
	const int split = blockIdx.y;
	const int foot = split / g.spf;
	const int sidx = split - foot * g.spf;
	const int cpf = (g.V - g.v_begin + 31) / 32;
	const int q0 = sidx * g.cps;
	const int q1 = min(q0 + g.cps, cpf);
	const int lr = tid >> 6;
	const int lc = (tid & 63) * 4;
	int nact = 2;
	if constexpr (AMODE == AMODE_PE) {
		const int live = ((g.pe >> 4) + 1) * 32 - (kt * 256 + wk * 64);
// ... 377 lines not shown
	const int lane = threadIdx.x & 63;
	const int n = blockIdx.x * 4 + (threadIdx.x >> 6);
	const int foot = blockIdx.y;
	const float* wr = Wfull + (int64_t)n * ldw + W;
	const float* lv = lat + (int64_t)foot * L;
	float s = 0.f;
	for (int j = lane; j < L; j += 64) s = fmaf(wr[j], lv[j], s);
	s = wave_sum(s);
	if (lane == 0) fb[(int64_t)foot * W + n] = b[n] + s;
}

__global__ __launch_bounds__(256) void latent_grad_kernel(const float* Wfull, int ldw, const float* lat, int L, const float* S, int n_feet,
														   float* dlat, float* dWfull, float* db) {
	__shared__ float red[4][64];
	const int b = blockIdx.x;
	const int lane = threadIdx.x & 63, q = threadIdx.x >> 6;
	if (b == n_feet + W) {
		float s = 0.f;
		for (int f = 0; f < n_feet; ++f) s += S[(int64_t)f * W + threadIdx.x];
		db[threadIdx.x] = s;
		return;
	}
	if (b < n_feet) {
		if (dlat == nullptr) return;
		for (int j0 = 0; j0 < L; j0 += 64) {
			const int j = j0 + lane;
			float s0 = 0.f, s1 = 0.f, s2 = 0.f, s3 = 0.f;
			if (j < L) {
				const float* wp = Wfull + (int64_t)(q * 64) * ldw + W + j;
				const float* sp = S + (int64_t)b * W + q * 64;
#pragma unroll
				for (int n = 0; n < 64; n += 4) {
					s0 = fmaf(sp[n + 0], wp[(int64_t)(n + 0) * ldw], s0);
					s1 = fmaf(sp[n + 1], wp[(int64_t)(n + 1) * ldw], s1);
					s2 = fmaf(sp[n + 2], wp[(int64_t)(n + 2) * ldw], s2);
					s3 = fmaf(sp[n + 3], wp[(int64_t)(n + 3) * ldw], s3);
				}
			}
			red[q][lane] = (s0 + s1) + (s2 + s3);
			__syncthreads();
			if (q == 0 && j < L) dlat[(int64_t)b * L + j] = (red[0][lane] + red[1][lane]) + (red[2][lane] + red[3][lane]);
			__syncthreads();
		}
	} else {
		const int n = b - n_feet;
		for (int j = threadIdx.x; j < L; j += blockDim.x) {
			float s = 0.f;
			for (int f = 0; f < n_feet; ++f) s = fmaf(S[(int64_t)f * W + n], lat[(int64_t)f * L + j], s);
			dWfull[(int64_t)n * ldw + W + j] = s;
		}
	}
}

constexpr int BCAST_FEET = 4;
__global__ __launch_bounds__(256) void bias_relu_bcast_kernel(const float* __restrict__ P, const float* __restrict__ bias, int64_t bias_foot_stride,
															   int n_feet, int64_t V, float* __restrict__ out, int out_half) {
	const int64_t per_foot = V * (W / 4);
	const int64_t r = (int64_t)blockIdx.x * blockDim.x + threadIdx.x;
	if (r >= per_foot) return;
	const int c4 = (int)(r & (W / 4 - 1));
	const float4 p = reinterpret_cast<const float4*>(P)[r];
	const int f0 = blockIdx.y * BCAST_FEET;
#pragma unroll
	for (int k = 0; k < BCAST_FEET; ++k) {
		const int foot = f0 + k;
		if (foot >= n_feet) break;
		const float4 b = *reinterpret_cast<const float4*>(bias + foot * bias_foot_stride + c4 * 4);
		float4 o;
		o.x = fmaxf(p.x + b.x, 0.f); o.y = fmaxf(p.y + b.y, 0.f); o.z = fmaxf(p.z + b.z, 0.f); o.w = fmaxf(p.w + b.w, 0.f);
		st4_any(out, (foot * per_foot + r) * 4, out_half, o);
	}
}

struct HeadOutArgs {
	const float* x[2];
	const float* w[2];
	const float* b[2];
	float* z[2];
	float* out[2];
	const float* avg_col;
	int64_t rows;
	int head0;
	int x_half;
};

__device__ __forceinline__ float row16_sum(float t) {
	t += __int_as_float(__builtin_amdgcn_update_dpp(0, __float_as_int(t), 0xB1, 0xF, 0xF, false));
	t += __int_as_float(__builtin_amdgcn_update_dpp(0, __float_as_int(t), 0x4E, 0xF, 0xF, false));
	t += __int_as_float(__builtin_amdgcn_update_dpp(0, __float_as_int(t), 0x141, 0xF, 0xF, false));
	t += __int_as_float(__builtin_amdgcn_update_dpp(0, __float_as_int(t), 0x140, 0xF, 0xF, false));
	return t;
}

__global__ __launch_bounds__(256) void head_out_fwd_kernel(const HeadOutArgs g) {
	const int head = blockIdx.y + g.head0;
	const int lane = threadIdx.x & 63, wave = threadIdx.x >> 6;
	const float* x = head ? g.x[1] : g.x[0];
	const float* w = head ? g.w[1] : g.w[0];
	const float* b = head ? g.b[1] : g.b[0];
	float* z = head ? g.z[1] : g.z[0];
	float* out = head ? g.out[1] : g.out[0];
	if (out == nullptr) return;
	const int part = lane & 15, sub = lane >> 4;
	float4 wv[3][4];
#pragma unroll
	for (int c = 0; c < 3; ++c)
#pragma unroll
		for (int i = 0; i < 4; ++i) wv[c][i] = *reinterpret_cast<const float4*>(w + c * W + part * 4 + 64 * i);
	const int c3 = part < 3 ? part : 0;
	const float bc = b[c3];
	const float av = (head && g.avg_col) ? g.avg_col[c3] : 0.f;
	constexpr int U = 2;
	for (int64_t r0 = ((int64_t)blockIdx.x * 4 + wave) * (4 * U); r0 < g.rows; r0 += (int64_t)gridDim.x * 4 * (4 * U)) {
		float4 xv[U][4];
#pragma unroll
		for (int u = 0; u < U; ++u) {
			const int64_t row = r0 + u * 4 + sub;
#pragma unroll
			for (int i = 0; i < 4; ++i)
				xv[u][i] = (row < g.rows) ? ld4_any(x, row * W + part * 4 + 64 * i, g.x_half) : make_float4(0.f, 0.f, 0.f, 0.f);
		}
#pragma unroll
		for (int u = 0; u < U; ++u) {
			const int64_t row = r0 + u * 4 + sub;
			float sc[3];
#pragma unroll
			for (int c = 0; c < 3; ++c) {
				float t = 0.f;
#pragma unroll
				for (int i = 0; i < 4; ++i) t += xv[u][i].x * wv[c][i].x + xv[u][i].y * wv[c][i].y + xv[u][i].z * wv[c][i].z + xv[u][i].w * wv[c][i].w;
				sc[c] = row16_sum(t);
			}
			if (part < 3 && row < g.rows) {
				const float zz = (part == 0 ? sc[0] : (part == 1 ? sc[1] : sc[2])) + bc;
				const float t = tanhf(zz);
				if (z) z[row * 3 + part] = zz;
				out[row * 3 + part] = head ? (av + 0.5f * (1.0f + t)) : 0.1f * t;
			}
		}
	}
}

typedef _Float16 find_h8 __attribute__((ext_vector_type(8)));
typedef float find_f4 __attribute__((ext_vector_type(4)));
__global__ __launch_bounds__(256) void head_out_fwd_h16_kernel(const HeadOutArgs g) {
	const int head = blockIdx.y + g.head0;
	const int lane = threadIdx.x & 63, wave = threadIdx.x >> 6;
	const _Float16* x = reinterpret_cast<const _Float16*>(head ? g.x[1] : g.x[0]);
	const float* w = head ? g.w[1] : g.w[0];
	const float* b = head ? g.b[1] : g.b[0];
	float* z = head ? g.z[1] : g.z[0];
	float* out = head ? g.out[1] : g.out[0];
	if (out == nullptr) return;
	const int m = lane & 15, kq = lane >> 4;
	const int ch = m < 3 ? m : 0;
	find_h8 wh[8], wl[8];
#pragma unroll
	for (int s = 0; s < 8; ++s)
#pragma unroll
		for (int j = 0; j < 8; ++j) {
			const float v = m < 3 ? 16.0f * w[ch * W + 32 * s + 8 * kq + j] : 0.f;
			const _Float16 hi = (_Float16)v;
			wh[s][j] = hi;
			wl[s][j] = (_Float16)(v - (float)hi);
		}
	const float bc = b[ch];
	const float av = (head && g.avg_col) ? g.avg_col[ch] : 0.f;
	constexpr int U = 4;
	const int64_t nblk = (g.rows + 15) >> 4;
	for (int64_t b0 = ((int64_t)blockIdx.x * 4 + wave) * U; b0 < nblk; b0 += (int64_t)gridDim.x * 4 * U) {
		find_h8 xa[U][8];
#pragma unroll
		for (int u = 0; u < U; ++u) {
			const int64_t row = min((b0 + u) * 16 + m, g.rows - 1);
			const find_h8* p = reinterpret_cast<const find_h8*>(x + row * W + 8 * kq);
#pragma unroll
			for (int s = 0; s < 8; ++s) xa[u][s] = p[4 * s];
		}
#pragma unroll
		for (int u = 0; u < U; ++u) {
			find_f4 acc = {0.f, 0.f, 0.f, 0.f};
#pragma unroll
			for (int s = 0; s < 8; ++s) {
				acc = __builtin_amdgcn_mfma_f32_16x16x32_f16(xa[u][s], wl[s], acc, 0, 0, 0);
				acc = __builtin_amdgcn_mfma_f32_16x16x32_f16(xa[u][s], wh[s], acc, 0, 0, 0);
			}
			if (m < 3) {
#pragma unroll
				for (int i = 0; i < 4; ++i) {
					const int64_t row = (b0 + u) * 16 + 4 * kq + i;
					if (row < g.rows) {
						const float zz = acc[i] * 0.0625f + bc;
						const float t = tanhf(zz);
						if (z) z[row * 3 + m] = zz;
						out[row * 3 + m] = head ? (av + 0.5f * (1.0f + t)) : 0.1f * t;
					}
				}
			}
		}
	}
}

struct HeadOutBwdArgs {
	const float* y[2];
	const float* w[2];
	const float* z[2];
	const float* gout[2];
	float* dy[2];
	float* pw[2];
	float* pb[2];
	int64_t rows;
	int half;
};

template <int U>
__device__ __forceinline__ void head_out_bwd_body(const HeadOutBwdArgs& g) {
	const int head = blockIdx.y;
	const float* gout = head ? g.gout[1] : g.gout[0];
	if (gout == nullptr) return;
	const int lane = threadIdx.x & 63, wave = threadIdx.x >> 6;
	const float* y = head ? g.y[1] : g.y[0];
	const float* w = head ? g.w[1] : g.w[0];
	const float* z = head ? g.z[1] : g.z[0];
	float* dy = head ? g.dy[1] : g.dy[0];
	float* pw = head ? g.pw[1] : g.pw[0];
	float* pb = head ? g.pb[1] : g.pb[0];
	const float4 w0 = *reinterpret_cast<const float4*>(w + 0 * W + lane * 4);
	const float4 w1 = *reinterpret_cast<const float4*>(w + 1 * W + lane * 4);
	const float4 w2 = *reinterpret_cast<const float4*>(w + 2 * W + lane * 4);
	const float scale = head ? 0.5f : 0.1f;
	float4 aw0 = make_float4(0, 0, 0, 0), aw1 = aw0, aw2 = aw0;
	float ab0 = 0.f, ab1 = 0.f, ab2 = 0.f;
	for (int64_t r0 = ((int64_t)blockIdx.x * 4 + wave) * U; r0 < g.rows; r0 += (int64_t)gridDim.x * 4 * U) {
		float4 yv[U];
		float d[U][3];
#pragma unroll
		for (int u = 0; u < U; ++u) {
			const int64_t row = r0 + u;
			yv[u] = (row < g.rows) ? ld4_any(y, row * W + lane * 4, g.half) : make_float4(0, 0, 0, 0);
		}
		float dmine = 0.f;
		if (lane < U * 3) {
			const int64_t e = r0 * 3 + lane;
			if (e < g.rows * 3) {
				const float t = tanhf(z[e]);
				dmine = gout[e] * scale * (1.f - t * t);
			}
		}
#pragma unroll
		for (int u = 0; u < U; ++u)
#pragma unroll
			for (int c = 0; c < 3; ++c) d[u][c] = __builtin_bit_cast(float, __builtin_amdgcn_readlane(__builtin_bit_cast(int, dmine), u * 3 + c));
#pragma unroll
		for (int u = 0; u < U; ++u) {
			const int64_t row = r0 + u;
			if (row >= g.rows) break;
			const float d0 = d[u][0], d1 = d[u][1], d2 = d[u][2];
			float4 o;
			o.x = (yv[u].x > 0.f) ? d0 * w0.x + d1 * w1.x + d2 * w2.x : 0.f;
			o.y = (yv[u].y > 0.f) ? d0 * w0.y + d1 * w1.y + d2 * w2.y : 0.f;
			o.z = (yv[u].z > 0.f) ? d0 * w0.z + d1 * w1.z + d2 * w2.z : 0.f;
			o.w = (yv[u].w > 0.f) ? d0 * w0.w + d1 * w1.w + d2 * w2.w : 0.f;
			st4_any(dy, row * W + lane * 4, g.half, o);
			aw0.x += d0 * yv[u].x; aw0.y += d0 * yv[u].y; aw0.z += d0 * yv[u].z; aw0.w += d0 * yv[u].w;
			aw1.x += d1 * yv[u].x; aw1.y += d1 * yv[u].y; aw1.z += d1 * yv[u].z; aw1.w += d1 * yv[u].w;
			aw2.x += d2 * yv[u].x; aw2.y += d2 * yv[u].y; aw2.z += d2 * yv[u].z; aw2.w += d2 * yv[u].w;
			ab0 += d0; ab1 += d1; ab2 += d2;
		}
	}
	__shared__ __attribute__((aligned(16))) float red[4][3][256];
	__shared__ float redb[4][4];
	*reinterpret_cast<float4*>(&red[wave][0][lane * 4]) = aw0;
	*reinterpret_cast<float4*>(&red[wave][1][lane * 4]) = aw1;
	*reinterpret_cast<float4*>(&red[wave][2][lane * 4]) = aw2;
	if (lane == 0) { redb[wave][0] = ab0; redb[wave][1] = ab1; redb[wave][2] = ab2; }
	__syncthreads();
	const int k = threadIdx.x;
	for (int c = 0; c < 3; ++c)
		pw[((int64_t)blockIdx.x * 3 + c) * 256 + k] = red[0][c][k] + red[1][c][k] + red[2][c][k] + red[3][c][k];
	if (k < 3) pb[(int64_t)blockIdx.x * 4 + k] = redb[0][k] + redb[1][k] + redb[2][k] + redb[3][k];
}
__global__ __launch_bounds__(256) void head_out_bwd_kernel(const HeadOutBwdArgs g) {
	if (g.half) head_out_bwd_body<8>(g);
	else head_out_bwd_body<4>(g);
}

struct HeadOutReduceArgs {
	const float* pw[2];
	const float* pb[2];
	float* dw[2];
	float* db[2];
	int nblk;
};
__global__ __launch_bounds__(1024) void head_out_reduce_kernel(const HeadOutReduceArgs g) {
	const int head = blockIdx.y;
	float* dw = head ? g.dw[1] : g.dw[0];
	if (dw == nullptr) return;
	const float* pw = head ? g.pw[1] : g.pw[0];
	const float* pb = head ? g.pb[1] : g.pb[0];
	float* db = head ? g.db[1] : g.db[0];
	__shared__ float red[16][64];
	__shared__ float redb[16][4];
	const int j = threadIdx.x & 63, q = threadIdx.x >> 6;
	const int o = blockIdx.x * 64 + j;
	float s0 = 0.f, s1 = 0.f;
	int i = q;
	for (; i + 16 < g.nblk; i += 32) { s0 += pw[(int64_t)i * 768 + o]; s1 += pw[(int64_t)(i + 16) * 768 + o]; }
	if (i < g.nblk) s0 += pw[(int64_t)i * 768 + o];
	red[q][j] = s0 + s1;
	if (blockIdx.x == 0 && j < 3) {
		float t = 0.f;
		for (int k = q; k < g.nblk; k += 16) t += pb[(int64_t)k * 4 + j];
		redb[q][j] = t;
	}
	__syncthreads();
	if (q == 0) {
		float t = 0.f;
#pragma unroll
		for (int k = 0; k < 16; ++k) t += red[k][j];
		dw[o] = t;
		if (blockIdx.x == 0 && j < 3) {
			float u = 0.f;
#pragma unroll
			for (int k = 0; k < 16; ++k) u += redb[k][j];
			db[j] = u;
		}
	}
}

}
}
```

find_amd/csrc/register.hip:

```cpp
#include "common.h"

namespace find {
namespace reg {

constexpr int VPB = 1024;

struct Rot {
	float m[9];
};

__device__ __forceinline__ void euler_xyz(const float* e, float* R) {
	float s0, c0, s1, c1, s2, c2;
	sincosf(e[0], &s0, &c0);
	sincosf(e[1], &s1, &c1);
	sincosf(e[2], &s2, &c2);
	R[0] = c1 * c2;                  R[1] = -c1 * s2;                 R[2] = s1;
	R[3] = c0 * s2 + s0 * s1 * c2;   R[4] = c0 * c2 - s0 * s1 * s2;   R[5] = -s0 * c1;
	R[6] = s0 * s2 - c0 * s1 * c2;   R[7] = s0 * c2 + c0 * s1 * s2;   R[8] = c0 * c1;
}

__global__ __launch_bounds__(256) void register_fwd_kernel(const float* __restrict__ verts, int64_t verts_foot_stride,
															const float* __restrict__ disp, const float* __restrict__ reg,
															int V, float* __restrict__ out) {
	__shared__ float R[9];
	const int foot = blockIdx.y;
	const float* rg = reg + (int64_t)foot * 9;
	if (threadIdx.x == 0) euler_xyz(rg + 3, R);
	__syncthreads();
	const float tx = rg[0], ty = rg[1], tz = rg[2], sx = rg[6], sy = rg[7], sz = rg[8];
	const float* vp = verts + (int64_t)foot * verts_foot_stride;
	const float* dp = disp + (int64_t)foot * V * 3;
	float* op = out + (int64_t)foot * V * 3;
	for (int i = 0; i < 4; ++i) {
		const int v = blockIdx.x * VPB + i * 256 + threadIdx.x;
		if (v >= V) break;
		const float qx = (vp[v * 3 + 0] + dp[v * 3 + 0]) * sx;
		const float qy = (vp[v * 3 + 1] + dp[v * 3 + 1]) * sy;
		const float qz = (vp[v * 3 + 2] + dp[v * 3 + 2]) * sz;
		op[v * 3 + 0] = qx * R[0] + qy * R[3] + qz * R[6] + tx;
		op[v * 3 + 1] = qx * R[1] + qy * R[4] + qz * R[7] + ty;
		op[v * 3 + 2] = qx * R[2] + qy * R[5] + qz * R[8] + tz;
	}
}

__global__ __launch_bounds__(256) void register_bwd_kernel(const float* __restrict__ verts, int64_t verts_foot_stride,
															const float* __restrict__ disp, const float* __restrict__ reg,
															const float* __restrict__ dout, int V, float* __restrict__ d_disp,
															float* __restrict__ partial) {
	__shared__ float R[9];
	__shared__ float red[4][16];
	const int foot = blockIdx.y;
	const float* rg = reg + (int64_t)foot * 9;
	if (threadIdx.x == 0) euler_xyz(rg + 3, R);
	__syncthreads();
	const float sx = rg[6], sy = rg[7], sz = rg[8];
	const float* vp = verts + (int64_t)foot * verts_foot_stride;
	const float* dp = disp + (int64_t)foot * V * 3;
	const float* gp = dout + (int64_t)foot * V * 3;
	float* ddp = d_disp + (int64_t)foot * V * 3;
	float acc[15];
#pragma unroll
	for (int k = 0; k < 15; ++k) acc[k] = 0.f;
	for (int i = 0; i < 4; ++i) {
		const int v = blockIdx.x * VPB + i * 256 + threadIdx.x;
		if (v >= V) break;
		const float ux = vp[v * 3 + 0] + dp[v * 3 + 0], uy = vp[v * 3 + 1] + dp[v * 3 + 1], uz = vp[v * 3 + 2] + dp[v * 3 + 2];
		const float gx = gp[v * 3 + 0], gy = gp[v * 3 + 1], gz = gp[v * 3 + 2];
		const float dqx = gx * R[0] + gy * R[1] + gz * R[2];
		const float dqy = gx * R[3] + gy * R[4] + gz * R[5];
		const float dqz = gx * R[6] + gy * R[7] + gz * R[8];
		ddp[v * 3 + 0] = dqx * sx;
		ddp[v * 3 + 1] = dqy * sy;
		ddp[v * 3 + 2] = dqz * sz;
		acc[0] += gx; acc[1] += gy; acc[2] += gz;
		acc[3] += ux * dqx; acc[4] += uy * dqy; acc[5] += uz * dqz;
		const float qx = ux * sx, qy = uy * sy, qz = uz * sz;
		acc[6] += qx * gx; acc[7] += qx * gy; acc[8] += qx * gz;
		acc[9] += qy * gx; acc[10] += qy * gy; acc[11] += qy * gz;
		acc[12] += qz * gx; acc[13] += qz * gy; acc[14] += qz * gz;
	}
	const int lane = threadIdx.x & 63, wave = threadIdx.x >> 6;
#pragma unroll
	for (int k = 0; k < 15; ++k) {
		const float s = wave_sum(acc[k]);
		if (lane == 0) red[wave][k] = s;
	}
	__syncthreads();
	if (threadIdx.x < 15) {
		const int k = threadIdx.x;
		partial[((int64_t)foot * gridDim.x + blockIdx.x) * 16 + k] = red[0][k] + red[1][k] + red[2][k] + red[3][k];
	}
}

__global__ void register_finalize_kernel(const float* __restrict__ reg, const float* __restrict__ partial, int nblk,
										 float* __restrict__ d_reg) {
	const int foot = blockIdx.x;
	__shared__ float tot[16];
	if (threadIdx.x < 15) {
		float s = 0.f;
		for (int b = 0; b < nblk; ++b) s += partial[((int64_t)foot * nblk + b) * 16 + threadIdx.x];
		tot[threadIdx.x] = s;
	}
	__syncthreads();
	if (threadIdx.x == 0) {
		const float* e = reg + (int64_t)foot * 9 + 3;
		float s0, c0, s1, c1, s2, c2;
		sincosf(e[0], &s0, &c0);
		sincosf(e[1], &s1, &c1);
		sincosf(e[2], &s2, &c2);
		const float* G = tot + 6;
		const float dR0[9] = {0.f, 0.f, 0.f,
							  -s0 * s2 + c0 * s1 * c2, -s0 * c2 - c0 * s1 * s2, -c0 * c1,
							  c0 * s2 + s0 * s1 * c2, c0 * c2 - s0 * s1 * s2, -s0 * c1};
		const float dR1[9] = {-s1 * c2, s1 * s2, c1,
							  s0 * c1 * c2, -s0 * c1 * s2, s0 * s1,
							  -c0 * c1 * c2, c0 * c1 * s2, -c0 * s1};
		const float dR2[9] = {-c1 * s2, -c1 * c2, 0.f,
							  c0 * c2 - s0 * s1 * s2, -c0 * s2 - s0 * s1 * c2, 0.f,
							  s0 * c2 + c0 * s1 * s2, -s0 * s2 + c0 * s1 * c2, 0.f};
		float de0 = 0.f, de1 = 0.f, de2 = 0.f;
		for (int k = 0; k < 9; ++k) {
			de0 += G[k] * dR0[k];
			de1 += G[k] * dR1[k];
			de2 += G[k] * dR2[k];
		}
		float* o = d_reg + (int64_t)foot * 9;
		o[0] = tot[0]; o[1] = tot[1]; o[2] = tot[2];
		o[3] = de0; o[4] = de1; o[5] = de2;
		o[6] = tot[3]; o[7] = tot[4]; o[8] = tot[5];
	}
}

}
}

using namespace find;

extern "C" int find_register_fwd(const float* verts, int64_t verts_batch, const float* disp, const float* reg,
								 int64_t n_feet, int64_t n_pts, float* out, void* stream) {
	FIND_REQUIRE(verts && disp && reg && out, "find_register_fwd: NULL argument");
	FIND_REQUIRE(n_feet >= 1 && n_pts >= 1 && n_pts < (1ll << 29), "find_register_fwd: bad sizes");
	FIND_REQUIRE(verts_batch == 1 || verts_batch == n_feet, "find_register_fwd: verts_batch must be 1 or n_feet");
	hipStream_t s = reinterpret_cast<hipStream_t>(stream);
	dim3 grid((unsigned)cdiv(n_pts, reg::VPB), (unsigned)n_feet);
	hipLaunchKernelGGL(reg::register_fwd_kernel, grid, dim3(256), 0, s, verts, verts_batch == 1 ? 0 : n_pts * 3, disp, reg, (int)n_pts, out);
	FIND_LAUNCH_CHECK("register_fwd_kernel");
	return FIND_OK;
}

extern "C" int64_t find_register_bwd_ws_bytes(int64_t n_feet, int64_t n_pts) {
	return align_up(n_feet * cdiv(n_pts, reg::VPB) * 16 * (int64_t)sizeof(float), 256);
}

extern "C" int find_register_bwd(const float* verts, int64_t verts_batch, const float* disp, const float* reg,
								 const float* d_out, int64_t n_feet, int64_t n_pts, float* d_disp, float* d_reg,
								 void* ws, int64_t ws_bytes, void* stream) {
	FIND_REQUIRE(verts && disp && reg && d_out && d_disp && d_reg && ws, "find_register_bwd: NULL argument");
	FIND_REQUIRE(n_feet >= 1 && n_pts >= 1 && n_pts < (1ll << 29), "find_register_bwd: bad sizes");
	FIND_REQUIRE(verts_batch == 1 || verts_batch == n_feet, "find_register_bwd: verts_batch must be 1 or n_feet");
	if (ws_bytes < find_register_bwd_ws_bytes(n_feet, n_pts)) {
		set_error("find_register_bwd: workspace too small");
		return FIND_EWORKSPACE;
	}
	hipStream_t s = reinterpret_cast<hipStream_t>(stream);
	const int nblk = (int)cdiv(n_pts, reg::VPB);
	dim3 grid((unsigned)nblk, (unsigned)n_feet);
	hipLaunchKernelGGL(reg::register_bwd_kernel, grid, dim3(256), 0, s, verts, verts_batch == 1 ? 0 : n_pts * 3, disp, reg, d_out,
					   (int)n_pts, d_disp, reinterpret_cast<float*>(ws));
	hipLaunchKernelGGL(reg::register_finalize_kernel, dim3((unsigned)n_feet), dim3(64), 0, s, reg, reinterpret_cast<const float*>(ws), nblk, d_reg);
	FIND_LAUNCH_CHECK("register_bwd");
	return FIND_OK;
}
```

find_amd/functional.py:

```python
import ctypes

import torch

from . import _lib
from ._lib import MlpGrads, MlpParams, check, current_stream, ptr


def _require_gpu(*tensors):
	for t in tensors:
		if t is None:
			continue
		if not t.is_cuda:
			raise RuntimeError('find_amd: the HIP path needs tensors on a ROCm device (got a CPU tensor); '
							   'there is no CPU fallback -- use oracle/ only for testing')
		if t.dtype != torch.float32 and t.is_floating_point():
			raise RuntimeError(f'find_amd: fp32 tensors required, got {t.dtype}')


def _c(t):
	return None if t is None else t.contiguous()


def _ws(nbytes, device):
	return torch.empty(max(int(nbytes), 256), dtype=torch.uint8, device=device)
# ... 23 lines not shown


def _grads_like(tensors):
	out = [None] * len(tensors)
	rest = []
	if _GRAD_ARENA:
		ents = [_GRAD_ARENA.get((t.data_ptr(), t.numel())) for t in tensors]
		b0 = next((e[0] for e in ents if e is not None), None)
		if b0 is not None and all(e is not None and e[0] is b0 for e in ents):
			return _fill_rest(b0.take_many([e[1] for e in ents], tensors), tensors)
		for i, (t, ent) in enumerate(zip(tensors, ents)):
			out[i] = ent[0].take(ent[1], t.shape, t.device) if ent is not None else None
	return _fill_rest(out, tensors)


def _fill_rest(out, tensors):
	rest = [i for i, v in enumerate(out) if v is None]
	if rest:
		offs, n = [], 0
		for i in rest:
			offs.append(n)
			n += (tensors[i].numel() + 3) & ~3
		flat = torch.empty(n, dtype=tensors[rest[0]].dtype, device=tensors[rest[0]].device)
		for i, o in zip(rest, offs):
			shape = tensors[i].shape
			out[i] = flat.as_strided(shape, _contiguous_strides(shape), o)
	return out


_STRIDES = {}


def _contiguous_strides(shape):
	st = _STRIDES.get(shape)
	if st is None:
		acc, rev = 1, []
		for d in reversed(shape):
			rev.append(acc)
			acc *= d
		st = _STRIDES[shape] = tuple(reversed(rev))
	return st


class MLPSpec:

	def __init__(self, n_trunk, n_disp, n_col, pe_size, lat_disp, lat_col, in_dim=3, width=256, precision=None):
		self.n_trunk, self.n_disp, self.n_col = n_trunk, n_disp, n_col
		self.pe_size, self.lat_disp, self.lat_col = pe_size, lat_disp, lat_col
		self.in_dim, self.width = in_dim, width
		self.precision = precision

	@property
	def n_weights(self):
		return 2 * (self.n_trunk + self.n_disp + 1 + self.n_col + 1)


_PRECISION_CODE = {None: 0, 'fp32': 1, 'fp16': 2, 'bf16x3': 3}


def _fill_params(spec, B, avg_col, weights):
	p = MlpParams()
	p.precision = _PRECISION_CODE[spec.precision if spec.precision is not None else _MLP_PRECISION]
	p.width, p.in_dim, p.pe_size = spec.width, spec.in_dim, spec.pe_size
	p.n_trunk, p.n_disp, p.n_col = spec.n_trunk, spec.n_disp, spec.n_col
	p.lat_disp, p.lat_col = spec.lat_disp, spec.lat_col
	p.B = None if B is None else B.data_ptr()
	p.avg_col = None if avg_col is None else avg_col.data_ptr()
	it = iter(weights)
	for i in range(spec.n_trunk):
		p.trunk_w[i] = next(it).data_ptr()
		p.trunk_b[i] = next(it).data_ptr()
	for i in range(spec.n_disp + 1):
		p.disp_w[i] = next(it).data_ptr()
		p.disp_b[i] = next(it).data_ptr()
	for i in range(spec.n_col + 1):
		p.col_w[i] = next(it).data_ptr()
		p.col_b[i] = next(it).data_ptr()
	return p


class _MLP(torch.autograd.Function):

	@staticmethod
	def forward(ctx, spec, pos, lat_disp, lat_col, B, avg_col, *weights):
		spec, heads, defer = spec if isinstance(spec, tuple) else (spec, 3, False)
		if len(weights) != spec.n_weights:
			raise RuntimeError(f'find_amd.mlp: expected {spec.n_weights} weight tensors, got {len(weights)}')
		_require_gpu(pos, lat_disp, lat_col, B, avg_col, *weights)
		if pos.requires_grad:
			raise RuntimeError('find_amd.mlp: gradient w.r.t. positions is not part of the FIND path (template / sampled '
							   'GT points carry no grad, model.py:285, losses.py:39-51)')
		L = _lib.lib()
		pos, lat_disp, lat_col, B, avg_col = _c(pos), _c(lat_disp), _c(lat_col), _c(B), _c(avg_col)
		leaves = all(w.is_leaf for w in weights)
		weights = tuple(w.contiguous() for w in weights)
		if pos.dim() != 3 or pos.shape[-1] != spec.in_dim:
			raise RuntimeError(f'find_amd.mlp: pos must be (B|1, V, {spec.in_dim}), got {tuple(pos.shape)}')
		pos_batch, V, _ = pos.shape
		n_feet = pos_batch
		batches = set()
		for name, lat, width, bit in (('lat_disp', lat_disp, spec.lat_disp, 1), ('lat_col', lat_col, spec.lat_col, 2)):
			if lat is None:
				if width != 0 and heads & bit:
					raise RuntimeError(f'find_amd.mlp: {name} is missing but the head expects {width} latent columns')
				continue
			if lat.dim() != 2 or lat.shape[1] != width:
				raise RuntimeError(f'find_amd.mlp: {name} must be (n_feet, {width}), got {tuple(lat.shape)}')
			batches.add(int(lat.shape[0]))
		if len(batches) > 1:
			raise RuntimeError(f'find_amd.mlp: lat_disp and lat_col have different batch sizes {sorted(batches)}')
		if batches:
			n_feet = batches.pop()
		if pos_batch != 1 and pos_batch != n_feet:
			raise RuntimeError(f'find_amd.mlp: pos batch {pos_batch} does not match latent batch {n_feet}')
		p = _fill_params(spec, B, avg_col, weights)
		save = any(ctx.needs_input_grad)
		nbytes = L.find_mlp_ws_bytes(ctypes.byref(p), pos_batch, n_feet, V, int(save))
		if nbytes < 0:
			check(-1, 'find_mlp_ws_bytes')
		ws = _ws(nbytes, pos.device)
		disp = torch.empty(n_feet, V, 3, device=pos.device, dtype=torch.float32) if heads & 1 else None
		col = torch.empty(n_feet, V, 3, device=pos.device, dtype=torch.float32) if heads & 2 else None
		check(L.find_mlp_fwd(_lib.ctx(pos.device), ctypes.byref(p), ptr(pos), pos_batch, n_feet, V, ptr(lat_disp), ptr(lat_col), ptr(disp), ptr(col),
							 ptr(ws), ws.numel(), int(save), current_stream(pos.device)), 'find_mlp_fwd')
		if save:
			ctx.spec = spec
			ctx.precision = p.precision
			ctx.dims = (pos_batch, n_feet, V)
			ctx.ws = ws
			ctx.leaves = leaves
			ctx.defer = bool(defer)
			ctx.set_materialize_grads(False)
			ctx.save_for_backward(pos, lat_disp, lat_col, B, avg_col, *weights)
		return disp, col

	@staticmethod
	def backward(ctx, g_disp, g_col):
		L = _lib.lib()
		spec = ctx.spec
		pos, lat_disp, lat_col, B, avg_col, *weights = ctx.saved_tensors
		pos_batch, n_feet, V = ctx.dims
		g_disp, g_col = _c(g_disp), _c(g_col)
		p = _fill_params(spec, B, avg_col, weights)
		p.precision = ctx.precision
		nt, nd = 2 * spec.n_trunk, 2 * (spec.n_disp + 1)
		frozen = not any(ctx.needs_input_grad[6:])
		live = [False] * len(weights)
		if not frozen and (g_disp is not None or g_col is not None):
			live[:nt] = [True] * nt
			if g_disp is not None:
				live[nt:nt + nd] = [True] * nd
			if g_col is not None:
				live[nt + nd:] = [True] * (len(weights) - nt - nd)
		idx = [i for i, on in enumerate(live) if on]
		grads = [None] * len(weights)
		for i, g in zip(idx, _grads_like([weights[i] for i in idx]) if idx else []):
			grads[i] = g
		task = _graph_task_id()
		key = tuple(w.data_ptr() for w in weights)
		pending = _PENDING_WGRADS.get(key)
		can_park = ctx.leaves and not torch.is_grad_enabled() and task >= 0 and all(ctx.needs_input_grad[6:])
		cur = torch.cuda.current_stream(pos.device)
		fold = pending is not None and can_park and pending[0] == task
		cross = fold and pending[2] != cur
		g_lat_disp = torch.empty_like(lat_disp) if (lat_disp is not None and g_disp is not None and ctx.needs_input_grad[2]) else None
		g_lat_col = torch.empty_like(lat_col) if (lat_col is not None and g_col is not None and ctx.needs_input_grad[3]) else None
		if not idx and g_lat_disp is None and g_lat_col is None:
			return (None,) * (6 + len(weights))
		G = MlpGrads()
		it = iter(grads)
		for i in range(spec.n_trunk):
			G.trunk_w[i] = ptr(next(it))
			G.trunk_b[i] = ptr(next(it))
		for i in range(spec.n_disp + 1):
			G.disp_w[i] = ptr(next(it))
			G.disp_b[i] = ptr(next(it))
		for i in range(spec.n_col + 1):
			G.col_w[i] = ptr(next(it))
			G.col_b[i] = ptr(next(it))
		G.lat_disp = ptr(g_lat_disp)
		G.lat_col = ptr(g_lat_col)
		sb = L.find_mlp_bwd_scratch_bytes(ctypes.byref(p), pos_batch, n_feet, V)
		scratch = _ws(sb, pos.device)
		h = _lib.ctx(pos.device)
		defer = (DEFER_WGRAD_JOIN and ctx.defer and can_park and not fold and (pending is None or pending[0] != task) and idx
				 and all(w.grad is None and not w._backward_hooks
						 and (not getattr(w, '_post_accumulate_grad_hooks', None) or getattr(w, '_find_hooks_are_stream_safe', False)) for w in weights))
		if defer:
			check(L.find_ctx_set(h, b'defer_join', 1), 'find_ctx_set(defer_join)')
		check(L.find_mlp_bwd(h, ctypes.byref(p), ptr(pos), pos_batch, n_feet, V, ptr(lat_disp), ptr(lat_col), ptr(g_disp), ptr(g_col),
							 ptr(ctx.ws), ctx.ws.numel(), ptr(scratch), scratch.numel(), ctypes.byref(G),
							 current_stream(pos.device)), 'find_mlp_bwd')
		if defer and _lib.get_tuning('pending', pos.device):
			bases = {id(g._base): g._base for g in grads if g is not None and g._base is not None}
			_hold_until_join(pos.device, [scratch, ctx.ws, g_disp, g_col, pos, lat_disp, lat_col, *weights, *bases.values()])
		elif _DEFERRED:
			_join_deferred()
		if fold:
			slots = pending[1]
			both = [i for i in idx if slots[i] is not None]
			if cross:
				cur.wait_event(pending[3])
				_sync_at_end_of_backward(cur)
			if both:
				b0, g0 = slots[both[0]][0], grads[both[0]]._base
				lo, hi = slots[both[0]][1], slots[both[-1]][1] + grads[both[-1]].numel()
				shift = grads[both[0]].storage_offset() - lo
				if (FOLD_FLAT and g0 is not None and g0.dim() == 1 and b0.dim() == 1 and all(slots[i][0] is b0 and grads[i]._base is g0 and slots[i][1] + shift == grads[i].storage_offset() for i in both)
						and all(slots[both[k + 1]][1] - (slots[both[k]][1] + ((grads[both[k]].numel() + 3) & ~3)) == 0 for k in range(len(both) - 1))):
					b0[lo:hi].add_(g0[lo + shift:hi + shift])
				else:
					torch._foreach_add_([slots[i][0][slots[i][1]:slots[i][1] + grads[i].numel()].view(grads[i].shape) for i in both], [grads[i] for i in both])
			out = [None if slots[i] is not None else grads[i] for i in range(len(weights))]
			return (None, None, g_lat_disp, g_lat_col, None, None, *out)
		_PENDING_WGRADS.clear()
		if can_park and idx and all(grads[i]._base is not None and grads[i]._base.dim() == 1 for i in idx):
			done = torch.cuda.Event()
			done.record(cur)
			_PENDING_WGRADS[key] = (task, [(g._base, g.storage_offset()) if g is not None else None for g in grads], cur, done)
		return (None, None, g_lat_disp, g_lat_col, None, None, *grads)


import os as _os
DEFER_WGRAD_JOIN = _os.environ.get('FIND_DEFER_WGRADS', '1') != '0'
FOLD_FLAT = _os.environ.get('FIND_FOLD_FLAT', '1') != '0'
_DEFERRED = {}


_DEFERRED_TASK = [None]


def _hold_until_join(device, tensors):
	task = _graph_task_id()
	if _DEFERRED and _DEFERRED_TASK[0] != task:
		_join_deferred()
	first = not _DEFERRED
	_DEFERRED.setdefault(device, []).extend(t for t in tensors if t is not None)
	if first:
		_DEFERRED_TASK[0] = task
		torch.autograd.Variable._execution_engine.queue_callback(_join_deferred)


def _join_deferred():
	L = _lib.lib()
	for device in list(_DEFERRED):
		check(min(L.find_ctx_join(_lib.ctx(device), current_stream(device)), 0), 'find_ctx_join')
	_DEFERRED.clear()


_CROSS_STREAMS = []


def _sync_at_end_of_backward(stream):
	if not _CROSS_STREAMS:
		torch.autograd.Variable._execution_engine.queue_callback(_join_cross)
	if stream not in _CROSS_STREAMS:
		_CROSS_STREAMS.append(stream)


def _join_cross():
	try:
		for s in _CROSS_STREAMS:
			torch.cuda.current_stream(s.device).wait_stream(s)
	finally:
		_CROSS_STREAMS.clear()


_PENDING_WGRADS = {}


def _graph_task_id():
	f = getattr(torch._C, '_current_graph_task_id', None)
	return int(f()) if f is not None else -1


def mlp(spec, pos, lat_disp, lat_col, B, avg_col, weights, want=('disp', 'col'), defer_wgrad_join=False):
	heads = (1 if 'disp' in want else 0) | (2 if 'col' in want else 0)
	if heads == 0:
		raise ValueError("find_amd.mlp: want must name 'disp', 'col' or both")
	return _MLP.apply((spec, heads, defer_wgrad_join), pos, lat_disp, lat_col, B, avg_col, *weights)


class _LatentGather(torch.autograd.Function):

	@staticmethod
	def forward(ctx, table, idx):
		_require_gpu(table, idx)
		L = _lib.lib()
		if table.dim() != 2 or idx.dim() != 1 or idx.dtype != torch.int64:
			raise RuntimeError(f'find_amd.latent_gather: table (rows, dim) and int64 idx (n) expected, got {tuple(table.shape)} / {tuple(idx.shape)} {idx.dtype}')
		table, idx = _c(table), _c(idx)
		out = torch.empty(idx.shape[0], table.shape[1], device=table.device, dtype=torch.float32)
		check(L.find_latent_gather_fwd(ptr(table), table.shape[0], table.shape[1], ptr(idx), idx.shape[0], ptr(out), current_stream(table.device)),
			  'find_latent_gather_fwd')
		ctx.save_for_backward(idx)
		ctx.shape = tuple(table.shape)
		ctx.table_key = (table.data_ptr(), table.numel())
		return out

	@staticmethod
	def backward(ctx, g):
		L = _lib.lib()
		idx, = ctx.saved_tensors
		g = _c(g)
		d_table = _grad_for(ctx.table_key, ctx.shape, g.device)
		check(L.find_latent_gather_bwd(ptr(g), ptr(idx), idx.shape[0], ctx.shape[0], ctx.shape[1], ptr(d_table), current_stream(g.device)),
			  'find_latent_gather_bwd')
		return d_table, None


def latent_gather(table, idx):
	return _LatentGather.apply(table, idx)


def _ptr_array(tensors):
	return (ctypes.c_void_p * len(tensors))(*[None if t is None else t.data_ptr() for t in tensors])


class _LatentGatherMany(torch.autograd.Function):

	@staticmethod
	def forward(ctx, n, *args):
		tables, idxs = args[:n], args[n:]
		_require_gpu(*tables)
		L = _lib.lib()
		tables = [_c(t) for t in tables]
		idxs = [_c(i) for i in idxs]
		n_idx = idxs[0].shape[0]
		for t, i in zip(tables, idxs):
			if t.dim() != 2 or i.dim() != 1 or i.dtype != torch.int64 or i.shape[0] != n_idx or not i.is_cuda:
				raise RuntimeError(f'find_amd.latent_gather_many: tables (rows, dim) and device int64 idx ({n_idx}) expected, got {tuple(t.shape)} / {tuple(i.shape)} {i.dtype}')
		dev = tables[0].device
		outs = [torch.empty(n_idx, t.shape[1], device=dev, dtype=torch.float32) for t in tables]
		rows = (ctypes.c_int64 * n)(*[t.shape[0] for t in tables])
		dims = (ctypes.c_int64 * n)(*[t.shape[1] for t in tables])
		check(L.find_latent_gather_many_fwd(n, _ptr_array(tables), rows, dims, _ptr_array(idxs), n_idx, _ptr_array(outs), current_stream(dev)),
			  'find_latent_gather_many_fwd')
		ctx.save_for_backward(*idxs)
		ctx.shapes = [tuple(t.shape) for t in tables]
		ctx.keys = [(t.data_ptr(), t.numel()) for t in tables]
		return tuple(outs)

	@staticmethod
	def backward(ctx, *gs):
		L = _lib.lib()
		idxs = ctx.saved_tensors
		n = len(idxs)
		dev = idxs[0].device
		gs = [_c(g) for g in gs]
		d_tables = [_grad_for(k, sh, dev) for k, sh in zip(ctx.keys, ctx.shapes)]
		rows = (ctypes.c_int64 * n)(*[sh[0] for sh in ctx.shapes])
		dims = (ctypes.c_int64 * n)(*[sh[1] for sh in ctx.shapes])
		check(L.find_latent_gather_many_bwd(n, _ptr_array(gs), rows, dims, _ptr_array(idxs), idxs[0].shape[0], _ptr_array(d_tables), current_stream(dev)),
			  'find_latent_gather_many_bwd')
		return (None, *d_tables, *([None] * n))


def latent_gather_many(tables, idxs):
	if not 1 <= len(tables) <= 8 or len(tables) != len(idxs):
		raise ValueError('find_amd.latent_gather_many: 1 .. 8 tables, one index tensor each')
	return list(_LatentGatherMany.apply(len(tables), *tables, *idxs))


# ... 880 lines not shown
```

find_amd/model.py:

```python
import os

import numpy as np
import torch

from . import functional as FN
from .structures import LazyTexturesVertex, Meshes, TexturesVertex, extend_template

nn = torch.nn


def make_params_list(*params):
	out = []
	for prm in params:
		if prm is None:
			continue
		if isinstance(prm, nn.Parameter):
			out.append(prm)
		elif hasattr(prm, 'parameters'):
			out.extend(prm.parameters())
		else:
			raise ValueError(f'Param type {type(prm)} not understood.')
	return out


# ... 297 lines not shown
		for i in range(dispdepth):
			disp_layers += [nn.Linear(width + self._lat_disp if i == 0 else width, width), nn.ReLU()]
		disp_layers.append(nn.Linear(width, 3))
		self.mlp_disp = nn.Sequential(*disp_layers)
		col_layers = []
		for i in range(coldepth):
			col_layers += [nn.Linear(width + self._lat_col if i == 0 else width, width), nn.ReLU()]
		self.use_avg_colour = use_avg_colour
		col_layers.append(nn.Linear(width, 3))
		self.mlp_col = nn.Sequential(*col_layers)

		self.restyle_features_per_vertex = restyle_features_per_vertex
		self.per_vertex_features = None
		if opts is not None and getattr(opts, 'template_features_pth', None) is not None:
			self.per_vertex_features = nn.Parameter(load_template_classes(opts.template_features_pth, device=device).unsqueeze(0))
			if template_mesh_loc is not None:
				self._check_per_vertex_features()

		self.main_params = make_params_list(self.base, self.mlp_disp, self.mlp_col, self.shapevec, self.texvec, self.posevec)
		self.templ_params = make_params_list(self.template_verts, self.reg)
		self.val_params = make_params_list(self.shapevec_val, self.texvec_val, self.posevec_val)
		self.reg_params = make_params_list(self.reg, self.reg_val)
		self.latent_params = make_params_list(self.shapevec, self.shapevec_val, self.texvec, self.texvec_val, self.posevec, self.posevec_val)

		if dispdepth < 1 or coldepth < 1:
			raise NotImplementedError('dispdepth/coldepth must be >= 1')
		self._spec = FN.MLPSpec(n_trunk=depth + 1, n_disp=dispdepth, n_col=coldepth, pe_size=width if use_pe else 0,
								lat_disp=self._lat_disp, lat_col=self._lat_col, in_dim=input_dim, width=width)
		self.reset_weights()
		self.onnx_mode = False

	def set_mlp_precision(self, precision):
		if precision not in (None, 'fp32', 'fp16', 'bf16x3'):
			raise ValueError(f"set_mlp_precision: None, 'fp32', 'bf16x3' or 'fp16', got {precision!r}")
		self._spec.precision = precision

	def _check_per_vertex_features(self):
		f = self.per_vertex_features
		if f is not None and (f.dim() != 3 or f.shape[1] != self.template_verts.shape[1]):
			raise ValueError(f'template_features_pth holds per-vertex features of shape {tuple(f.shape[1:])}, the template has '
							 f'{self.template_verts.shape[1]} vertices: (V, C) with the template\'s V expected')

	def _rebuild_template_mesh(self):
		self.template_mesh = Meshes(verts=self.template_verts.data, faces=self.template_faces.data[0])

	def _weights(self):
		c = self.__dict__.get('_wlist')
		if c is not None:
			ws, checks, seqs = c
			mods = self._modules
			ok = mods['base'] is seqs[0] and mods['mlp_disp'] is seqs[1] and mods['mlp_col'] is seqs[2]
			if ok:
				for i, (md, key, layer, pd) in enumerate(checks):
					if md.get(key) is not layer or pd.get('weight') is not ws[2 * i] or pd.get('bias') is not ws[2 * i + 1]:
						ok = False
						break
				ok = ok and sum(len(q) for q in seqs) == self.__dict__['_wcount']
			if ok:
				return ws
		ws, checks = [], []
		seqs = (self.base, self.mlp_disp, self.mlp_col)
		for seq in seqs:
			for key, layer in seq._modules.items():
				if isinstance(layer, nn.Linear):
					ws += [layer.weight, layer.bias]
					checks.append((seq._modules, key, layer, layer._parameters))
		self.__dict__['_wlist'] = (ws, checks, seqs)
		self.__dict__['_wcount'] = sum(len(q) for q in seqs)
		return ws

	def _apply(self, fn, *args, **kwargs):
		self.__dict__.pop('_wlist', None)
		out = super()._apply(fn, *args, **kwargs)
		self._rebuild_template_mesh()
		return out

	@staticmethod
	def _cat_latents(*vecs):
		vecs = [v for v in vecs if v is not None]
		if not vecs:
			return None
		return vecs[0] if len(vecs) == 1 else torch.cat(vecs, dim=-1)

	def forward(self, pos, shapevec=None, texvec=None, posevec=None, want=('disp', 'col'), defer_wgrad_join=False):
		if self.onnx_mode:
			raise NotImplementedError('onnx_mode (web export) is out of scope')
		if pos.dim() != 3 or pos.shape[-1] != self.input_dim:
			raise ValueError(f'pos must be [B, V, {self.input_dim}], got {tuple(pos.shape)}')
		lat_disp = self._cat_latents(shapevec, posevec) if 'disp' in want else None
		lat_col = self._cat_latents(texvec) if 'col' in want else None
		got_d = self._lat_disp if 'disp' not in want else (0 if lat_disp is None else lat_disp.shape[-1])
		got_c = self._lat_col if 'col' not in want else (0 if lat_col is None else lat_col.shape[-1])
		if got_d != self._lat_disp or got_c != self._lat_col:
			raise RuntimeError(f'latent widths do not match the head input sizes: disp head expects {self._lat_disp} latent columns '
							   f'(got {got_d}), col head expects {self._lat_col} (got {got_c}); cf. model.py:352,361')
		enc = self.encoder[0] if len(self.encoder) else None
		B = enc.B(pos.device) if enc is not None else None
		avg = self.avg_col if self.use_avg_colour else None
		disp, col = FN.mlp(self._spec, pos, lat_disp, lat_col, B, avg, self._weights(), want=want, defer_wgrad_join=defer_wgrad_join)
		return {k: v for k, v in (('disp', disp), ('col', col)) if v is not None}

	def get_meshes(self, shapevec=None, reg=None, texvec=None, posevec=None, no_displacement=False, include_texture=True, lazy_colours=False):
		N = 0 if shapevec is None else shapevec.shape[0]
		self._check_per_vertex_features()
		meshes = extend_template(self.template_mesh, N=N)
		tv = self.template_verts.data
		if not self.use_texvec:
			raise NotImplementedError('use_texvec=False: the template-texture fallback of get_meshes does not exist upstream either (model.py:288-295, 500)')
		if lazy_colours:
			cell = _Once(lambda: self(tv, shapevec=shapevec, texvec=texvec, posevec=posevec, want=('col',))['col'])
			res = _LazyColours(self(tv, shapevec=shapevec, texvec=texvec, posevec=posevec, want=('disp',)), cell)
		else:
			res = self(tv, shapevec=shapevec, texvec=texvec, posevec=posevec)
		offsets = res['disp']
		if reg is not None:
			X = FN.register_points(tv, offsets, reg)
		else:
			X = tv + offsets
		if not no_displacement:
			meshes = meshes.update_padded(X)
		if lazy_colours:
			meshes.textures = LazyTexturesVertex(lambda: cell()[..., :3])
		else:
			meshes.textures = TexturesVertex(res['col'][..., :3])
		res.update(meshes=meshes, offsets=offsets, verts=X)
		if self.per_vertex_features is not None:
			res['cpv'] = self.per_vertex_features
		return res

	def get_meshes_from_batch(self, batch, is_train=True, no_displacement=False, lazy_colours=False):
		sfx = 'train' if is_train else 'val'
		return self.get_meshes(shapevec=batch.get(f'shapevec_{sfx}', None), reg=batch.get(f'reg_{sfx}', None),
							   texvec=batch.get(f'texvec_{sfx}', None), posevec=batch.get(f'posevec_{sfx}', None),
							   include_texture=True, no_displacement=no_displacement, lazy_colours=lazy_colours)

	def reset_weights(self):
		self.mlp_disp[-1].weight.data.zero_()
		self.mlp_disp[-1].bias.data.zero_()

	def configure_template(self, state_dict, device='cuda'):
		self.template_verts = nn.Parameter(state_dict['template_verts'].float().to(device), requires_grad=False)
		self.template_faces = nn.Parameter(state_dict['template_faces'].to(device), requires_grad=False)
		self._rebuild_template_mesh()
		self._check_per_vertex_features()
		if 'avg_col' in state_dict:
			self.avg_col = nn.Parameter(state_dict['avg_col'].to(device), requires_grad=False)

	def set_template(self, verts, faces):
		dev = self.template_verts.device
		self.configure_template({'template_verts': verts.reshape(1, -1, 3), 'template_faces': faces.reshape(1, -1, 3)}, device=dev)

	def to(self, device):
		out = super().to(device)
		self._rebuild_template_mesh()
		return out


class PCAModel(Model):

	def __init__(self, *args, train_size=None, val_size=None, device='cuda', **kwargs):
		super().__init__()
		self.params = dict(train_size=train_size, val_size=val_size)
		self.train_size, self.val_size = train_size, val_size
		self.template_verts = self.template_faces = self.template_mesh = None
		self.pca_var = None
		self.pca_coefs = None
		self.latent_vectors_train, self.latent_vectors_val = [], []
		self.shapevec, self.shapevec_val = None, None
		ident = np.array([0] * 6 + [1] * 3)
		self.reg = LatentVector(train_size, vec_size=9, name='reg_train', device=device, init_values=ident)
		self.reg_val = LatentVector(val_size, vec_size=9, name='reg_val', device=device, init_values=ident)
		self.latent_vectors_train.append(self.reg)
		self.latent_vectors_val.append(self.reg_val)
		self.configure_params()

	def configure_params(self):
		self.main_params = make_params_list(self.shapevec)
		self.val_params = make_params_list(self.shapevec_val)
		self.reg_params = make_params_list(self.reg, self.reg_val)
		self.latent_params = make_params_list(self.shapevec, self.shapevec_val)

	def _rebuild_template_mesh(self):
		if self.template_verts is not None:
			self.template_mesh = Meshes(verts=self.template_verts.data, faces=self.template_faces.data[0])

	def _apply(self, fn, *args, **kwargs):
		out = super()._apply(fn, *args, **kwargs)
		self._rebuild_template_mesh()
		return out

	def get_meshes(self, shapevec=None, reg=None, **kwargs):
		N = shapevec.shape[0]
		meshes = extend_template(self.template_mesh, N=N)
		tv = self.template_verts.data
		offsets = FN.pca_offsets(self.pca_coefs, shapevec)
		X = FN.register_points(tv, offsets, reg) if reg is not None else tv + offsets
		meshes = meshes.update_padded(X)
		meshes.textures = TexturesVertex(torch.full(X.shape, 0.5, dtype=torch.float32, device=X.device))
		return dict(meshes=meshes, offsets=offsets, verts=X)
# ... 52 lines not shown
```

include/find_hip.h:

```cpp
#ifndef FIND_HIP_H
#define FIND_HIP_H

#include <stdint.h>

#ifdef __cplusplus
extern "C" {
#endif

#define FIND_ABI_VERSION 3

#define FIND_OK 0
#define FIND_EINVAL (-1)
#define FIND_EWORKSPACE (-2)
#define FIND_ELAUNCH (-3)

#define FIND_MAX_LAYERS 8

int find_abi_version(void);
const char* find_last_error(void);
const char* find_build_arch(void);

typedef struct find_ctx find_ctx;
int find_ctx_create(int device, find_ctx** out);
int find_ctx_destroy(find_ctx* ctx);
int find_ctx_stream_groups(find_ctx* ctx, void* caller_stream, int32_t* groups );
int find_ctx_stream_beside(find_ctx* ctx, void* caller_stream, void* const* candidates, int32_t n, int32_t role, int32_t* index);
int find_ctx_set(find_ctx* ctx, const char* key, int64_t value);
int find_ctx_get(const find_ctx* ctx, const char* key, int64_t* value);

typedef struct find_mlp_params {
	int32_t width;
	int32_t in_dim;
	int32_t pe_size;
	int32_t n_trunk;
	int32_t n_disp;
	int32_t n_col;
	int32_t lat_disp;
	int32_t lat_col;
	const float* B;
	const float* trunk_w[FIND_MAX_LAYERS];
	const float* trunk_b[FIND_MAX_LAYERS];
	const float* disp_w[FIND_MAX_LAYERS];
	const float* disp_b[FIND_MAX_LAYERS];
	const float* col_w[FIND_MAX_LAYERS];
	const float* col_b[FIND_MAX_LAYERS];
	const float* avg_col;
	int32_t precision;
} find_mlp_params;

typedef struct find_mlp_grads {
	float* trunk_w[FIND_MAX_LAYERS];
	float* trunk_b[FIND_MAX_LAYERS];
	float* disp_w[FIND_MAX_LAYERS];
	float* disp_b[FIND_MAX_LAYERS];
	float* col_w[FIND_MAX_LAYERS];
	float* col_b[FIND_MAX_LAYERS];
	float* lat_disp;
	float* lat_col;
} find_mlp_grads;

int64_t find_mlp_ws_bytes(const find_mlp_params* p, int64_t pos_batch, int64_t n_feet, int64_t n_pts, int save_for_bwd);

int find_mlp_fwd(find_ctx* ctx, const find_mlp_params* p, const float* pos, int64_t pos_batch, int64_t n_feet, int64_t n_pts,
				 const float* lat_disp, const float* lat_col, float* disp, float* col,
				 void* ws, int64_t ws_bytes, int save_for_bwd, void* stream);

int64_t find_mlp_bwd_scratch_bytes(const find_mlp_params* p, int64_t pos_batch, int64_t n_feet, int64_t n_pts);
int find_mlp_bwd(find_ctx* ctx, const find_mlp_params* p, const float* pos, int64_t pos_batch, int64_t n_feet, int64_t n_pts,
				 const float* lat_disp, const float* lat_col, const float* d_disp, const float* d_col,
				 const void* ws, int64_t ws_bytes, void* scratch, int64_t scratch_bytes,
				 const find_mlp_grads* grads, void* stream);

int find_ctx_join(find_ctx* ctx, void* stream);

int find_linear_relu_fwd(find_ctx* ctx, const float* x, const float* w, const float* b, int64_t n_feet, int64_t n_pts, float* y, void* stream);

int64_t find_linear_wgrad_scratch_bytes(int64_t n_feet);
int find_linear_wgrad(find_ctx* ctx, const float* dz, const float* x, int64_t n_feet, int64_t n_pts, float* dw, float* db,
					  void* scratch, int64_t scratch_bytes, void* stream);


int find_render_switches(int64_t bits);
int find_latent_gather_fwd(const float* table, int64_t n_rows, int64_t dim, const int64_t* idx, int64_t n_idx, float* out, void* stream);
int find_latent_gather_bwd(const float* d_out, const int64_t* idx, int64_t n_idx, int64_t n_rows, int64_t dim, float* d_table, void* stream);
int find_latent_gather_many_fwd(int64_t n_tables, const float* const* tables, const int64_t* n_rows, const int64_t* dims,
								const int64_t* const* idx, int64_t n_idx, float* const* outs, void* stream);
int find_latent_gather_many_bwd(int64_t n_tables, const float* const* d_outs, const int64_t* n_rows, const int64_t* dims,
								const int64_t* const* idx, int64_t n_idx, float* const* d_tables, void* stream);

int find_weighted_terms_fwd(int64_t n, const float* const* terms, const float* weights, float* scaled, float* total, void* stream);
int find_weighted_terms_bwd(int64_t n, const float* weights, const float* g_total, const float* g_scaled, float* d_terms, void* stream);

int find_contrastive_fwd(const float* vecs, int64_t N, int64_t K, const float* codes, int64_t C, const int32_t* pairs, int64_t P, float margin,
						 float* loss_out, float* coef_ws, void* stream);
int find_contrastive_bwd(const float* vecs, int64_t N, int64_t K, const int32_t* pairs, int64_t P, const float* coef_ws, const float* d_loss,
						 float* d_vecs, void* stream);

#define FIND_PART_AUTO 0
#define FIND_PART_DIRECT 1
#define FIND_PART_STAGED 2
int find_part_labels(const float* gt_logits, int64_t B, int64_t C, int64_t h, int64_t w, int64_t H, int64_t W, int32_t* labels, void* stream);
int find_part_ce_fwd(const float* logits, const int32_t* labels, const float* mask, int64_t P, int64_t C, float* loss_out, float* ce_out,
					 double* partial_ws, int64_t form, void* stream);
int find_part_ce_bwd(const float* logits, const int32_t* labels, const float* mask, int64_t P, int64_t C, const float* d_loss, float* d_logits,
					 float* d_mask, int64_t form, void* stream);

int find_vertex_normals_fwd(const float* verts, const int32_t* faces, int64_t faces_batch, const int32_t* vf_off, const int32_t* vf_items, int64_t N,
							int64_t V, int64_t F, float* normals_out, void* stream);
int find_vertex_normals_bwd(const float* verts, const int32_t* faces, int64_t faces_batch, const int32_t* vf_off, const int32_t* vf_items, int64_t N,
							int64_t V, int64_t F, const float* d_normals, float* d_raw_ws, float* d_verts, void* stream);
int find_normal_map_fwd(const float* raw, const float* R, int64_t n_images, int64_t n_views, int64_t H, int64_t W, int world, float* out, void* stream);
int find_normal_map_bwd(const float* raw, const float* R, const float* d_out, int64_t n_images, int64_t n_views, int64_t H, int64_t W, int world,
						float* d_raw, void* stream);
int64_t find_normal_loss_ws_bytes(int64_t P);
int find_normal_loss_fwd(const float* pred, const float* target, const float* weight, int64_t P, float* loss_out, void* ws, int64_t ws_bytes, void* stream);
int find_normal_loss_bwd(const float* pred, const float* target, const float* weight, int64_t P, const float* d_loss, const void* ws, float* d_pred,
						 void* stream);

int64_t find_point_face_ws_bytes(int64_t n_meshes, int64_t n_points);
int find_point_face_fwd(const float* points, const int32_t* p_len, const float* verts, const int32_t* faces, int64_t faces_batch, int64_t n_meshes,
						int64_t n_points, int64_t n_verts, int64_t n_faces, float* dist2, int32_t* idx, float* bary, void* ws, int64_t ws_bytes, void* stream);
int find_point_face_bwd(const float* points, const float* verts, const int32_t* faces, int64_t faces_batch, const int32_t* idx, const float* bary,
						const float* g, int64_t n_meshes, int64_t n_points, int64_t n_verts, int64_t n_faces, float* d_points, float* d_verts, void* stream);

int find_register_fwd(const float* verts, int64_t verts_batch, const float* disp, const float* reg,
					  int64_t n_feet, int64_t n_pts, float* out, void* stream);
int64_t find_register_bwd_ws_bytes(int64_t n_feet, int64_t n_pts);
int find_register_bwd(const float* verts, int64_t verts_batch, const float* disp, const float* reg,
					  const float* d_out, int64_t n_feet, int64_t n_pts, float* d_disp, float* d_reg,
					  void* ws, int64_t ws_bytes, void* stream);

int find_pca_fwd(const float* coefs, int64_t V, int64_t B, const float* shapevec, int64_t n_feet, float* offsets, void* stream);
int64_t find_pca_bwd_ws_bytes(int64_t n_feet, int64_t V, int64_t B);
int find_pca_bwd(const float* coefs, int64_t V, int64_t B, const float* d_offsets, int64_t n_feet, float* d_shapevec, void* ws, int64_t ws_bytes,
				 void* stream);

int find_sample_points_fwd(const float* verts, const int32_t* faces, int64_t faces_batch, const int32_t* face_idx,
						   const float* uv, int64_t n_meshes, int64_t n_verts, int64_t n_faces, int64_t n_samples,
						   float* out, const float* attr, float* attr_out, void* stream);
int find_sample_points_bwd(const int32_t* faces, int64_t faces_batch, const int32_t* face_idx, const float* uv,
						   const float* d_out, int64_t n_meshes, int64_t n_verts, int64_t n_faces, int64_t n_samples,
						   float* d_verts, void* stream);
int find_face_areas(const float* verts, const int32_t* faces, int64_t faces_batch, int64_t n_meshes, int64_t n_verts,
					int64_t n_faces, float* areas, void* stream);
int64_t find_sample_surface_ws_bytes(int64_t n_meshes, int64_t n_faces);
int find_sample_surface_fwd(const float* verts, const int32_t* faces, int64_t faces_batch, const float* rnd, int64_t n_meshes,
							int64_t n_verts, int64_t n_faces, int64_t n_samples, int32_t* face_idx, float* uv, float* out,
							const float* attr, float* attr_out, void* ws, int64_t ws_bytes, void* stream);
int find_sample_surface_again(const float* verts, const int32_t* faces, int64_t faces_batch, const float* rnd, int64_t n_meshes,
							  int64_t n_verts, int64_t n_faces, int64_t n_samples, int32_t* face_idx, float* uv, float* out,
							  const float* attr, float* attr_out, const void* ws, int64_t ws_bytes, void* stream);

int find_nn_fwd(const float* x, const int32_t* x_len, const float* y, const int32_t* y_len, int64_t n,
				int64_t p1_max, int64_t p2_max, float* dist, int32_t* idx, void* stream);
int find_nn_bwd(const float* x, const int32_t* x_len, const float* y, const int32_t* idx, const float* w, int64_t n,
// ... 110 lines not shown
```

Baseline: 70.90 million vertices*views/s.

## Fold registration transform into MLP displacement head forward and backward

```diff
diff --git a/find_amd/_lib.py b/find_amd/_lib.py
--- a/find_amd/_lib.py
+++ b/find_amd/_lib.py
@@ -63,6 +63,8 @@
 	'find_mlp_fwd': (c_int, [_P, POINTER(MlpParams), _P, _I, _I, _I, _P, _P, _P, _P, _P, _I, c_int, _P]),
 	'find_mlp_bwd_scratch_bytes': (c_int64, [POINTER(MlpParams), _I, _I, _I]),
 	'find_mlp_bwd': (c_int, [_P, POINTER(MlpParams), _P, _I, _I, _I, _P, _P, _P, _P, _P, _I, _P, _I, POINTER(MlpGrads), _P]),
+	'find_mlp_fwd_reg': (c_int, [_P, POINTER(MlpParams), _P, _I, _I, _I, _P, _P, _P, _P, _P, _P, _I, _P, POINTER(c_int32), _P, _I, c_int, _P]),
+	'find_mlp_bwd_reg': (c_int, [_P, POINTER(MlpParams), _P, _I, _I, _I, _P, _P, _P, _P, _P, _P, _P, _I, _P, _P, _P, _I, _P, _I, POINTER(MlpGrads), _P]),
 	'find_linear_relu_fwd': (c_int, [_P, _P, _P, _P, _I, _I, _P, _P]),
 	'find_linear_wgrad_scratch_bytes': (c_int64, [_I]),
 	'find_linear_wgrad': (c_int, [_P, _P, _P, _I, _I, _P, _P, _P, _I, _P]),
diff --git a/find_amd/csrc/mlp.hip b/find_amd/csrc/mlp.hip
--- a/find_amd/csrc/mlp.hip
+++ b/find_amd/csrc/mlp.hip
@@ -149,6 +149,8 @@
 	float* pwo[2];
 	float* pbo[2];
 	int nblk_out;
+	float* regp;
+	float* regd;
 	int64_t max_split;
 	float* grp_pw;
 	int64_t grp_slabs;
@@ -207,6 +209,8 @@
 		o->pwo[i] = c.take<float>((int64_t)o->nblk_out * 3 * W);
 		o->pbo[i] = c.take<float>((int64_t)o->nblk_out * 4);
 	}
+	o->regp = c.take<float>(reg::register_partial_floats(d.n_feet, d.V));
+	o->regd = c.take<float>(d.rows_h * 3);
 	o->bytes = c.off;
 }
 
@@ -435,10 +439,30 @@
 	return c->x3 && !c->f16 && shared && n_feet > 1 && units >= c->gemm6_min_units;
 }
 static void note_act16(find_ctx* c, const void* ws, bool a16, bool fold) {
-	for (auto& n : c->act16_notes) if (n.ws == ws) { n.a16 = a16; n.fold = fold; return; }
-	c->act16_notes[c->act16_next] = find_ctx::Act16Note{ws, a16, fold};
+	for (auto& n : c->act16_notes) if (n.ws == ws) { n.a16 = a16; n.fold = fold; n.regf = false; return; }
+	c->act16_notes[c->act16_next] = find_ctx::Act16Note{ws, a16, fold, false};
 	c->act16_next = (c->act16_next + 1) & 15;
 }
+static bool use_reg_fold(const find_ctx* c, bool per_layer_out, bool disp_head, int64_t n_feet) {
+	return c->reg_fold != 0 && per_layer_out && disp_head && n_feet <= reg::REG_FOLD_MAX_FEET;
+}
+static void note_reg_fold(find_ctx* c, const void* ws) {
+	for (auto& n : c->act16_notes) if (n.ws == ws) { n.regf = true; return; }
+}
+static int noted_reg_fold(const find_ctx* c, const void* ws) {
+	for (const auto& n : c->act16_notes) if (n.ws == ws) return n.regf ? 1 : 0;
+	return -1;
+}
+struct RegArgs {
+	const float* reg = nullptr;
+	const float* tmpl = nullptr;
+	int64_t tmpl_stride = 0;
+	float* verts = nullptr;
+	bool folded = false;
+	const float* gverts = nullptr;
+	const float* disp = nullptr;
+	float* d_reg = nullptr;
+};
 static int noted_act16(const find_ctx* c, const void* ws, bool by_rule, bool fold_by_rule) {
 	for (const auto& n : c->act16_notes) if (n.ws == ws) return (n.a16 ? 1 : 0) | (n.fold ? 2 : 0);
 	return (by_rule ? 1 : 0) | (fold_by_rule ? 2 : 0);
@@ -463,6 +487,8 @@
 	float* hp;
 	float* out;
 	const float* gout;
+	const float* gverts;
+	bool live() const { return gout != nullptr || gverts != nullptr; }
 	float* const* gw; float* const* gb; float* glat;
 	float* const* dz; int cur;
 	float* const* wt;
@@ -505,7 +531,7 @@
 	d.pS = b->pS; c.pS = b->pS2;
 }
 
-static int mlp_fwd_body(Fork& fk, const find_mlp_params* p, const Dims& d, const FwdWs& w, const float* pos, Head* heads) {
+static int mlp_fwd_body(Fork& fk, const find_mlp_params* p, const Dims& d, const FwdWs& w, const float* pos, Head* heads, RegArgs& rg) {
 	find_ctx* c = fk.c;
 	hipStream_t s = fk.s;
 	const int64_t V = d.V, n_feet = d.n_feet;
@@ -587,6 +613,8 @@
 
 	const float* hl = w.H[p->n_trunk - 1];
 	const int64_t hl_stride = d.shared ? 0 : V * W;
+	rg.folded = rg.reg != nullptr && use_reg_fold(c, true, hd.out != nullptr, n_feet);
+	if (rg.folded) note_reg_fold(c, w.fbd);
 	auto head_first = [&](const Head& h, hipStream_t st) -> int {
 		if (h.hp) {
 			if (!fused) {
@@ -618,9 +646,14 @@
 		h.rows = d.rows_h;
 		h.head0 = head;
 		h.x_half = a16 ? 1 : 0;
+		int lds = 0;
+		if (head == 0 && rg.folded) {
+			h.reg = rg.reg; h.tmpl = rg.tmpl; h.tmpl_foot_stride = rg.tmpl_stride; h.verts = rg.verts; h.V = (int)V; h.n_feet = (int)n_feet;
+			lds = (int)n_feet * reg::REG_TAB * (int)sizeof(float);
+		}
 		const unsigned gx = (unsigned)std::min<int64_t>(cdiv(d.rows_h, 32), 2048);
-		if (a16) hipLaunchKernelGGL(head_out_fwd_h16_kernel, dim3(gx, 1), dim3(256), 0, st, h);
-		else hipLaunchKernelGGL(head_out_fwd_kernel, dim3(gx, 1), dim3(256), 0, st, h);
+		if (a16) hipLaunchKernelGGL(head_out_fwd_h16_kernel, dim3(gx, 1), dim3(256), lds, st, h);
+		else hipLaunchKernelGGL(head_out_fwd_kernel, dim3(gx, 1), dim3(256), lds, st, h);
 	};
 	auto head = [&](const Head& h, hipStream_t st) -> int {
 		FIND_TRY(head_first(h, st));
@@ -863,7 +896,7 @@
 	return FIND_OK;
 }
 
-static int mlp_bwd_body(Fork& fk, const find_mlp_params* p, const Dims& d, const FwdWs& w, const BwdWs& b, const float* pos, Head* heads, const find_mlp_grads* g) {
+static int mlp_bwd_body(Fork& fk, const find_mlp_params* p, const Dims& d, const FwdWs& w, const BwdWs& b, const float* pos, Head* heads, const find_mlp_grads* g, const RegArgs& rg) {
 	find_ctx* c = fk.c;
 	hipStream_t s = fk.s;
 	const bool defer = fk.deferring;
@@ -871,9 +904,14 @@
 	const int K0 = p->in_dim + 2 * p->pe_size;
 	Head& hd = heads[0];
 	Head& hc = heads[1];
-	const bool act_d = hd.gout != nullptr, act_c = hc.gout != nullptr;
+	const bool act_d = hd.live(), act_c = hc.live();
 	const bool frozen = g->trunk_w[0] == nullptr;
 	enum { Q = 0, T1 = 1, T2 = 2, R = 3 };
+
+	if (rg.gverts && rg.d_reg) {
+		fk.fork_to(T2);
+		FIND_TRY(reg::launch_register_bwd(rg.tmpl, rg.tmpl_stride, rg.disp, rg.reg, rg.gverts, n_feet, V, b.regd, rg.d_reg, b.regp, fk.stream(T2)));
+	}
 
 	ZeroArgs za;
 	memset(&za, 0, sizeof(za));
@@ -890,7 +928,7 @@
 	};
 	for (int k = 0; k < 2; ++k) {
 		const Head& h = heads[k];
-		if (h.gout) continue;
+		if (h.live()) continue;
 		zero(h.gw[0], (int64_t)W * h.ld0); zero(h.gb[0], W);
 		for (int i = 1; i < h.nl; ++i) { zero(h.gw[i], (int64_t)W * W); zero(h.gb[i], W); }
 		zero(h.gw[h.nl], 3 * W); zero(h.gb[h.nl], 3);
@@ -953,11 +991,16 @@
 			h.dy[k] = hk.dz[hk.cur];
 			h.pw[k] = b.pwo[k]; h.pb[k] = b.pbo[k];
 			hr.pw[k] = b.pwo[k]; hr.pb[k] = b.pbo[k];
-			hr.dw[k] = hk.gout ? hk.gw[hk.nl] : nullptr; hr.db[k] = hk.gb[hk.nl];
+			hr.dw[k] = hk.live() ? hk.gw[hk.nl] : nullptr; hr.db[k] = hk.gb[hk.nl];
 		}
 		h.rows = d.rows_h;
 		h.half = a16 ? 1 : 0;
-		hipLaunchKernelGGL(head_out_bwd_kernel, dim3((unsigned)b.nblk_out, 2), dim3(256), 0, s, h);
+		int lds = 0;
+		if (rg.gverts) {
+			h.gverts = rg.gverts; h.reg = rg.reg; h.V = (int)V; h.n_feet = (int)n_feet;
+			lds = (int)n_feet * reg::REG_TAB * (int)sizeof(float);
+		}
+		hipLaunchKernelGGL(head_out_bwd_kernel, dim3((unsigned)b.nblk_out, 2), dim3(256), lds, s, h);
 		hr.nblk = b.nblk_out;
 		if (!frozen) {
 			fk.fork_to(T2);
@@ -1037,7 +1080,7 @@
 		FIND_TRY(chain_prepare(c, tch, V, d.feet_t, s, b.w6, chain_w6_bytes(p)));
 	}
 	if (frozen) {
-		auto want = [&](const Head& h) { return h.gout && h.L > 0 && h.glat != nullptr; };
+		auto want = [&](const Head& h) { return h.live() && h.L > 0 && h.glat != nullptr; };
 		if (!want(hd) && !want(hc)) return FIND_OK;
 		if (small_chain) {
 			Chain ch;
@@ -1253,9 +1296,15 @@
 	return w.bytes;
 }
 
-extern "C" int find_mlp_fwd(find_ctx* c, const find_mlp_params* p, const float* pos, int64_t pos_batch, int64_t n_feet, int64_t n_pts,
-							const float* lat_disp, const float* lat_col, float* disp, float* col, void* ws,
-							int64_t ws_bytes, int save_for_bwd, void* stream) {
+static int check_reg(const char* who, const float* reg, const float* tmpl, int64_t tmpl_batch, int64_t n_feet) {
+	FIND_REQUIRE(reg != nullptr && tmpl != nullptr, "%s: reg / tmpl is NULL", who);
+	FIND_REQUIRE(tmpl_batch == 1 || tmpl_batch == n_feet, "%s: tmpl_batch must be 1 or n_feet", who);
+	return FIND_OK;
+}
+
+static int mlp_fwd_entry(find_ctx* c, const find_mlp_params* p, const float* pos, int64_t pos_batch, int64_t n_feet, int64_t n_pts,
+						 const float* lat_disp, const float* lat_col, float* disp, float* col, RegArgs& rg, void* ws,
+						 int64_t ws_bytes, int save_for_bwd, void* stream) {
 	FIND_TRY(check_ctx(c, "find_mlp_fwd"));
 	Dims d;
 	FIND_TRY(make_dims(p, pos_batch, n_feet, n_pts, &d));
@@ -1277,9 +1326,29 @@
 	Head heads[2];
 	make_heads(heads, p, w, lat_disp, lat_col, nullptr, nullptr);
 	heads[0].out = disp; heads[1].out = col;
-	const int rc = mlp_fwd_body(fk, p, d, w, pos, heads);
+	const int rc = mlp_fwd_body(fk, p, d, w, pos, heads, rg);
 	const int rj = fk.join();
 	return rc != FIND_OK ? rc : rj;
+}
+
+extern "C" int find_mlp_fwd(find_ctx* c, const find_mlp_params* p, const float* pos, int64_t pos_batch, int64_t n_feet, int64_t n_pts,
+							const float* lat_disp, const float* lat_col, float* disp, float* col, void* ws,
+							int64_t ws_bytes, int save_for_bwd, void* stream) {
+	RegArgs rg;
+	return mlp_fwd_entry(c, p, pos, pos_batch, n_feet, n_pts, lat_disp, lat_col, disp, col, rg, ws, ws_bytes, save_for_bwd, stream);
+}
+
+extern "C" int find_mlp_fwd_reg(find_ctx* c, const find_mlp_params* p, const float* pos, int64_t pos_batch, int64_t n_feet, int64_t n_pts,
+								const float* lat_disp, const float* lat_col, float* disp, float* col, const float* reg, const float* tmpl,
+								int64_t tmpl_batch, float* verts, int32_t* folded, void* ws, int64_t ws_bytes, int save_for_bwd, void* stream) {
+	FIND_REQUIRE(folded != nullptr && verts != nullptr, "find_mlp_fwd_reg: verts / folded is NULL");
+	*folded = 0;
+	FIND_TRY(check_reg("find_mlp_fwd_reg", reg, tmpl, tmpl_batch, n_feet));
+	RegArgs rg;
+	rg.reg = reg; rg.tmpl = tmpl; rg.tmpl_stride = tmpl_batch == 1 ? 0 : n_pts * 3; rg.verts = verts;
+	const int rc = mlp_fwd_entry(c, p, pos, pos_batch, n_feet, n_pts, lat_disp, lat_col, disp, col, rg, ws, ws_bytes, save_for_bwd, stream);
+	if (rc == FIND_OK) *folded = rg.folded ? 1 : 0;
+	return rc;
 }
 
 extern "C" int find_linear_relu_fwd(find_ctx* c, const float* x, const float* w, const float* b, int64_t n_feet, int64_t n_pts, float* y, void* stream) {
@@ -1330,23 +1399,24 @@
 	return b.bytes;
 }
 
-extern "C" int find_mlp_bwd(find_ctx* c, const find_mlp_params* p, const float* pos, int64_t pos_batch, int64_t n_feet, int64_t n_pts,
-							const float* lat_disp, const float* lat_col, const float* d_disp, const float* d_col,
-							const void* ws, int64_t ws_bytes, void* scratch, int64_t scratch_bytes,
-							const find_mlp_grads* g, void* stream) {
+static int mlp_bwd_entry(find_ctx* c, const find_mlp_params* p, const float* pos, int64_t pos_batch, int64_t n_feet, int64_t n_pts,
+						 const float* lat_disp, const float* lat_col, const float* d_disp, const float* d_col, const RegArgs& rg,
+						 const void* ws, int64_t ws_bytes, void* scratch, int64_t scratch_bytes,
+						 const find_mlp_grads* g, void* stream) {
 	FIND_TRY(check_ctx(c, "find_mlp_bwd"));
+	const bool live_d = d_disp != nullptr || rg.gverts != nullptr;
 	Dims d;
 	FIND_TRY(make_dims(p, pos_batch, n_feet, n_pts, &d));
 	FIND_TRY(check_weights(p));
 	FIND_REQUIRE(pos && ws && scratch && g, "find_mlp_bwd: NULL argument");
-	FIND_REQUIRE(p->lat_disp == 0 ? lat_disp == nullptr : (lat_disp != nullptr || d_disp == nullptr), "find_mlp_bwd: lat_disp pointer does not match params");
+	FIND_REQUIRE(p->lat_disp == 0 ? lat_disp == nullptr : (lat_disp != nullptr || !live_d), "find_mlp_bwd: lat_disp pointer does not match params");
 	FIND_REQUIRE(p->lat_col == 0 ? lat_col == nullptr : (lat_col != nullptr || d_col == nullptr), "find_mlp_bwd: lat_col pointer does not match params");
 	FIND_REQUIRE(p->precision >= 0 && p->precision <= 3, "find_mlp_bwd: params.precision must be 0, 1, 2 or 3 (got %d)", p->precision);
 	{
 		const bool frozen = g->trunk_w[0] == nullptr;
 		bool ok = true;
 		for (int i = 0; i < p->n_trunk; ++i) ok = ok && ((g->trunk_w[i] == nullptr) == frozen) && ((g->trunk_b[i] == nullptr) == frozen);
-		for (int i = 0; i <= p->n_disp; ++i) ok = ok && (frozen ? !g->disp_w[i] && !g->disp_b[i] : (d_disp == nullptr || (g->disp_w[i] && g->disp_b[i])));
+		for (int i = 0; i <= p->n_disp; ++i) ok = ok && (frozen ? !g->disp_w[i] && !g->disp_b[i] : (!live_d || (g->disp_w[i] && g->disp_b[i])));
 		for (int i = 0; i <= p->n_col; ++i) ok = ok && (frozen ? !g->col_w[i] && !g->col_b[i] : (d_col == nullptr || (g->col_w[i] && g->col_b[i])));
 		FIND_REQUIRE(ok, "find_mlp_bwd: grads must name every weight-gradient buffer of the evaluated heads and the trunk, or none at all (frozen network)");
 	}
@@ -1356,6 +1426,9 @@
 		set_error("find_mlp_bwd: forward workspace too small (%lld < %lld)", (long long)ws_bytes, (long long)w.bytes);
 		return FIND_EWORKSPACE;
 	}
+	if (rg.gverts) {
+		FIND_REQUIRE(noted_reg_fold(c, w.fbd) != 0 && n_feet <= reg::REG_FOLD_MAX_FEET, "find_mlp_bwd_reg: d_verts given, but the forward of this workspace did not form the registration");
+	}
 	BwdWs b;
 	carve_bwd(p, d, scratch, &b);
 	if (scratch_bytes < b.bytes) {
@@ -1365,15 +1438,39 @@
 	c->f16 = call_f16(c, p);
 	c->x3 = call_x3(c, p);
 	Fork fk(c, reinterpret_cast<hipStream_t>(stream), c->bwd_streams != 0);
-	const bool defer = c->defer_join != 0 && fk.on && !fk.capturing && !d.shared && use_fused(c, d.V, d.feet_t) && p->pe_size > 0 && g->trunk_w[0] != nullptr;
+	const bool defer = c->defer_join != 0 && fk.on && !fk.capturing && !rg.gverts && !d.shared && use_fused(c, d.V, d.feet_t) && p->pe_size > 0 && g->trunk_w[0] != nullptr;
 	c->defer_join = 0;
 	fk.deferring = defer;
 	Head heads[2];
 	make_heads(heads, p, w, lat_disp, lat_col, &b, g);
 	heads[0].gout = d_disp; heads[1].gout = d_col;
-	const int rc = mlp_bwd_body(fk, p, d, w, b, pos, heads, g);
+	heads[0].gverts = rg.gverts;
+	const int rc = mlp_bwd_body(fk, p, d, w, b, pos, heads, g, rg);
 	const int rj = (defer && rc == FIND_OK) ? fk.defer() : fk.join();
 	return rc != FIND_OK ? rc : rj;
+}
+
+extern "C" int find_mlp_bwd(find_ctx* c, const find_mlp_params* p, const float* pos, int64_t pos_batch, int64_t n_feet, int64_t n_pts,
+							const float* lat_disp, const float* lat_col, const float* d_disp, const float* d_col,
+							const void* ws, int64_t ws_bytes, void* scratch, int64_t scratch_bytes,
+							const find_mlp_grads* g, void* stream) {
+	RegArgs rg;
+	return mlp_bwd_entry(c, p, pos, pos_batch, n_feet, n_pts, lat_disp, lat_col, d_disp, d_col, rg, ws, ws_bytes, scratch, scratch_bytes, g, stream);
+}
+
+extern "C" int find_mlp_bwd_reg(find_ctx* c, const find_mlp_params* p, const float* pos, int64_t pos_batch, int64_t n_feet, int64_t n_pts,
+								const float* lat_disp, const float* lat_col, const float* d_disp, const float* d_col, const float* d_verts,
+								const float* reg, const float* tmpl, int64_t tmpl_batch, const float* disp, float* d_reg,
+								const void* ws, int64_t ws_bytes, void* scratch, int64_t scratch_bytes,
+								const find_mlp_grads* g, void* stream) {
+	RegArgs rg;
+	if (d_verts) {
+		FIND_TRY(check_reg("find_mlp_bwd_reg", reg, tmpl, tmpl_batch, n_feet));
+		FIND_REQUIRE(disp != nullptr || d_reg == nullptr, "find_mlp_bwd_reg: d_reg needs the forward's disp");
+		rg.reg = reg; rg.tmpl = tmpl; rg.tmpl_stride = tmpl_batch == 1 ? 0 : n_pts * 3;
+		rg.gverts = d_verts; rg.disp = disp; rg.d_reg = d_reg;
+	}
+	return mlp_bwd_entry(c, p, pos, pos_batch, n_feet, n_pts, lat_disp, lat_col, d_disp, d_col, rg, ws, ws_bytes, scratch, scratch_bytes, g, stream);
 }
 
 extern "C" int find_render_switches(int64_t bits) {
diff --git a/find_amd/csrc/mlp_ctx.h b/find_amd/csrc/mlp_ctx.h
--- a/find_amd/csrc/mlp_ctx.h
+++ b/find_amd/csrc/mlp_ctx.h
@@ -29,6 +29,7 @@
 	int defer_join = 0;
 	int act16 = 1;
 	int bcast_fold = 1;
+	int reg_fold = 1;
 	int footsum_fold = 1;
 	hipStream_t side[N_SIDE] = {nullptr, nullptr, nullptr, nullptr};
 	bool side_bound = false;
@@ -39,7 +40,7 @@
 	hipEvent_t pend_ev[N_SIDE] = {nullptr, nullptr, nullptr, nullptr};
 	bool pend[N_SIDE] = {};
 	bool attr_done[K_COUNT] = {};
-	struct Act16Note { const void* ws; bool a16; bool fold; };
+	struct Act16Note { const void* ws; bool a16; bool fold; bool regf; };
 	Act16Note act16_notes[16] = {};
 	int act16_next = 0;
 	bool f16 = false;
@@ -368,6 +369,7 @@
 	{"act16", &find_ctx::act16, 0, 1},
 	{"bcast_fold", &find_ctx::bcast_fold, 0, 1},
 	{"footsum_fold", &find_ctx::footsum_fold, 0, 1},
+	{"reg_fold", &find_ctx::reg_fold, 0, 1},
 };
 }
 
diff --git a/find_amd/csrc/mlp_kernels.h b/find_amd/csrc/mlp_kernels.h
--- a/find_amd/csrc/mlp_kernels.h
+++ b/find_amd/csrc/mlp_kernels.h
@@ -1,5 +1,6 @@
 #pragma once
 #include "common.h"
+#include "register_math.h"
 
 namespace find {
 namespace mlp {
@@ -543,7 +544,43 @@
 	int64_t rows;
 	int head0;
 	int x_half;
+	const float* reg;
+	const float* tmpl;
+	int64_t tmpl_foot_stride;
+	float* verts;
+	int V, n_feet;
 };
+
+struct RowAt { int foot, v; };
+struct RowWalk {
+	int foot, v, dfoot, dv, V;
+	__device__ __forceinline__ RowWalk(int64_t row0, int64_t stride, int V_) : V(V_) {
+		const unsigned r = __builtin_amdgcn_readfirstlane((unsigned)row0), s = (unsigned)stride, d = (unsigned)V_;
+		foot = (int)(r / d); v = (int)(r - (unsigned)foot * d);
+		dfoot = (int)(s / d); dv = (int)(s - (unsigned)dfoot * d);
+	}
+	__device__ __forceinline__ void step() {
+		foot += dfoot; v += dv;
+		if (v >= V) { v -= V; foot += 1; }
+	}
+	__device__ __forceinline__ RowAt at(int off) const {
+		RowAt r{foot, v + off};
+		while (r.v >= V) { r.v -= V; r.foot += 1; }
+		return r;
+	}
+};
+
+__device__ __forceinline__ void store_registered(const HeadOutArgs& g, const float* tab, float dv, int c, int64_t row, RowAt at) {
+	const float d0 = __int_as_float(__builtin_amdgcn_update_dpp(0, __float_as_int(dv), 0x00, 0xF, 0xF, false));
+	const float d1 = __int_as_float(__builtin_amdgcn_update_dpp(0, __float_as_int(dv), 0x55, 0xF, 0xF, false));
+	const float d2 = __int_as_float(__builtin_amdgcn_update_dpp(0, __float_as_int(dv), 0xAA, 0xF, 0xF, false));
+	const float* tb = tab + at.foot * reg::REG_TAB;
+	const float* vp = g.tmpl + at.foot * g.tmpl_foot_stride + (int64_t)at.v * 3;
+	const float qx = reg::pinned::scaled_point(vp[0], d0, tb[12]);
+	const float qy = reg::pinned::scaled_point(vp[1], d1, tb[13]);
+	const float qz = reg::pinned::scaled_point(vp[2], d2, tb[14]);
+	g.verts[row * 3 + c] = reg::pinned::rotated_point(qx, qy, qz, tb[c], tb[3 + c], tb[6 + c], tb[9 + c]);
+}
 
 __device__ __forceinline__ float row16_sum(float t) {
 	t += __int_as_float(__builtin_amdgcn_update_dpp(0, __float_as_int(t), 0xB1, 0xF, 0xF, false));
@@ -562,6 +599,9 @@
 	float* z = head ? g.z[1] : g.z[0];
 	float* out = head ? g.out[1] : g.out[0];
 	if (out == nullptr) return;
+	extern __shared__ float reg_tab[];
+	const bool regf = head == 0 && g.reg != nullptr;
+	if (regf) reg::build_reg_table(g.reg, g.n_feet, reg_tab);
 	const int part = lane & 15, sub = lane >> 4;
 	float4 wv[3][4];
 #pragma unroll
@@ -572,7 +612,8 @@
 	const float bc = b[c3];
 	const float av = (head && g.avg_col) ? g.avg_col[c3] : 0.f;
 	constexpr int U = 2;
-	for (int64_t r0 = ((int64_t)blockIdx.x * 4 + wave) * (4 * U); r0 < g.rows; r0 += (int64_t)gridDim.x * 4 * (4 * U)) {
+	RowWalk walk(((int64_t)blockIdx.x * 4 + wave) * (4 * U), (int64_t)gridDim.x * 4 * (4 * U), regf ? g.V : 1);
+	for (int64_t r0 = ((int64_t)blockIdx.x * 4 + wave) * (4 * U); r0 < g.rows; r0 += (int64_t)gridDim.x * 4 * (4 * U), walk.step()) {
 		float4 xv[U][4];
 #pragma unroll
 		for (int u = 0; u < U; ++u) {
@@ -596,7 +637,9 @@
 				const float zz = (part == 0 ? sc[0] : (part == 1 ? sc[1] : sc[2])) + bc;
 				const float t = tanhf(zz);
 				if (z) z[row * 3 + part] = zz;
-				out[row * 3 + part] = head ? (av + 0.5f * (1.0f + t)) : 0.1f * t;
+				const float o = head ? (av + 0.5f * (1.0f + t)) : 0.1f * t;
+				out[row * 3 + part] = o;
+				if (regf) store_registered(g, reg_tab, o, part, row, walk.at(u * 4 + sub));
 			}
 		}
 	}
@@ -613,6 +656,9 @@
 	float* z = head ? g.z[1] : g.z[0];
 	float* out = head ? g.out[1] : g.out[0];
 	if (out == nullptr) return;
+	extern __shared__ float reg_tab[];
+	const bool regf = head == 0 && g.reg != nullptr;
+	if (regf) reg::build_reg_table(g.reg, g.n_feet, reg_tab);
 	const int m = lane & 15, kq = lane >> 4;
 	const int ch = m < 3 ? m : 0;
 	find_h8 wh[8], wl[8];
@@ -629,7 +675,8 @@
 	const float av = (head && g.avg_col) ? g.avg_col[ch] : 0.f;
 	constexpr int U = 4;
 	const int64_t nblk = (g.rows + 15) >> 4;
-	for (int64_t b0 = ((int64_t)blockIdx.x * 4 + wave) * U; b0 < nblk; b0 += (int64_t)gridDim.x * 4 * U) {
+	RowWalk walk(((int64_t)blockIdx.x * 4 + wave) * U * 16, (int64_t)gridDim.x * 4 * U * 16, regf ? g.V : 1);
+	for (int64_t b0 = ((int64_t)blockIdx.x * 4 + wave) * U; b0 < nblk; b0 += (int64_t)gridDim.x * 4 * U, walk.step()) {
 		find_h8 xa[U][8];
 #pragma unroll
 		for (int u = 0; u < U; ++u) {
@@ -654,7 +701,9 @@
 						const float zz = acc[i] * 0.0625f + bc;
 						const float t = tanhf(zz);
 						if (z) z[row * 3 + m] = zz;
-						out[row * 3 + m] = head ? (av + 0.5f * (1.0f + t)) : 0.1f * t;
+						const float o = head ? (av + 0.5f * (1.0f + t)) : 0.1f * t;
+						out[row * 3 + m] = o;
+						if (regf) store_registered(g, reg_tab, o, m, row, walk.at(u * 16 + 4 * kq + i));
 					}
 				}
 			}
@@ -672,13 +721,17 @@
 	float* pb[2];
 	int64_t rows;
 	int half;
+	const float* gverts;
+	const float* reg;
+	int V, n_feet;
 };
 
 template <int U>
-__device__ __forceinline__ void head_out_bwd_body(const HeadOutBwdArgs& g) {
+__device__ __forceinline__ void head_out_bwd_body(const HeadOutBwdArgs& g, const float* reg_tab) {
 	const int head = blockIdx.y;
 	const float* gout = head ? g.gout[1] : g.gout[0];
-	if (gout == nullptr) return;
+	const float* gverts = head ? nullptr : g.gverts;
+	if (gout == nullptr && gverts == nullptr) return;
 	const int lane = threadIdx.x & 63, wave = threadIdx.x >> 6;
 	const float* y = head ? g.y[1] : g.y[0];
 	const float* w = head ? g.w[1] : g.w[0];
@@ -692,7 +745,8 @@
 	const float scale = head ? 0.5f : 0.1f;
 	float4 aw0 = make_float4(0, 0, 0, 0), aw1 = aw0, aw2 = aw0;
 	float ab0 = 0.f, ab1 = 0.f, ab2 = 0.f;
-	for (int64_t r0 = ((int64_t)blockIdx.x * 4 + wave) * U; r0 < g.rows; r0 += (int64_t)gridDim.x * 4 * U) {
+	RowWalk walk(((int64_t)blockIdx.x * 4 + wave) * U, (int64_t)gridDim.x * 4 * U, gverts ? g.V : 1);
+	for (int64_t r0 = ((int64_t)blockIdx.x * 4 + wave) * U; r0 < g.rows; r0 += (int64_t)gridDim.x * 4 * U, walk.step()) {
 		float4 yv[U];
 		float d[U][3];
 #pragma unroll
@@ -705,7 +759,18 @@
 			const int64_t e = r0 * 3 + lane;
 			if (e < g.rows * 3) {
 				const float t = tanhf(z[e]);
-				dmine = gout[e] * scale * (1.f - t * t);
+				float gin;
+				if (gverts) {
+					const int u = lane / 3, c = lane - 3 * u;
+					const RowAt at = walk.at(u);
+					const float* tb = reg_tab + at.foot * reg::REG_TAB;
+					const float* gv = gverts + (r0 + u) * 3;
+					const float folded = reg::pinned::disp_grad(c, gv[0], gv[1], gv[2], tb[3 * c], tb[3 * c + 1], tb[3 * c + 2], tb[12 + c]);
+					gin = gout ? reg::pinned::add(gout[e], folded) : folded;
+				} else {
+					gin = gout[e];
+				}
+				dmine = gin * scale * (1.f - t * t);
 			}
 		}
 #pragma unroll
@@ -742,8 +807,10 @@
 	if (k < 3) pb[(int64_t)blockIdx.x * 4 + k] = redb[0][k] + redb[1][k] + redb[2][k] + redb[3][k];
 }
 __global__ __launch_bounds__(256) void head_out_bwd_kernel(const HeadOutBwdArgs g) {
-	if (g.half) head_out_bwd_body<8>(g);
-	else head_out_bwd_body<4>(g);
+	extern __shared__ float reg_tab[];
+	if (blockIdx.y == 0 && g.gverts != nullptr) reg::build_reg_table(g.reg, g.n_feet, reg_tab);
+	if (g.half) head_out_bwd_body<8>(g, reg_tab);
+	else head_out_bwd_body<4>(g, reg_tab);
 }
 
 struct HeadOutReduceArgs {
diff --git a/find_amd/csrc/register.hip b/find_amd/csrc/register.hip
--- a/find_amd/csrc/register.hip
+++ b/find_amd/csrc/register.hip
@@ -1,23 +1,9 @@
-#include "common.h"
+#include "register_math.h"
 
 namespace find {
 namespace reg {
 
 constexpr int VPB = 1024;
-
-struct Rot {
-	float m[9];
-};
-
-__device__ __forceinline__ void euler_xyz(const float* e, float* R) {
-	float s0, c0, s1, c1, s2, c2;
-	sincosf(e[0], &s0, &c0);
-	sincosf(e[1], &s1, &c1);
-	sincosf(e[2], &s2, &c2);
-	R[0] = c1 * c2;                  R[1] = -c1 * s2;                 R[2] = s1;
-	R[3] = c0 * s2 + s0 * s1 * c2;   R[4] = c0 * c2 - s0 * s1 * s2;   R[5] = -s0 * c1;
-	R[6] = s0 * s2 - c0 * s1 * c2;   R[7] = s0 * c2 + c0 * s1 * s2;   R[8] = c0 * c1;
-}
 
 __global__ __launch_bounds__(256) void register_fwd_kernel(const float* __restrict__ verts, int64_t verts_foot_stride,
 															const float* __restrict__ disp, const float* __restrict__ reg,
@@ -34,12 +20,12 @@
 	for (int i = 0; i < 4; ++i) {
 		const int v = blockIdx.x * VPB + i * 256 + threadIdx.x;
 		if (v >= V) break;
-		const float qx = (vp[v * 3 + 0] + dp[v * 3 + 0]) * sx;
-		const float qy = (vp[v * 3 + 1] + dp[v * 3 + 1]) * sy;
-		const float qz = (vp[v * 3 + 2] + dp[v * 3 + 2]) * sz;
-		op[v * 3 + 0] = qx * R[0] + qy * R[3] + qz * R[6] + tx;
-		op[v * 3 + 1] = qx * R[1] + qy * R[4] + qz * R[7] + ty;
-		op[v * 3 + 2] = qx * R[2] + qy * R[5] + qz * R[8] + tz;
+		const float qx = scaled_point(vp[v * 3 + 0], dp[v * 3 + 0], sx);
+		const float qy = scaled_point(vp[v * 3 + 1], dp[v * 3 + 1], sy);
+		const float qz = scaled_point(vp[v * 3 + 2], dp[v * 3 + 2], sz);
+		op[v * 3 + 0] = rotated_point(qx, qy, qz, R[0], R[3], R[6], tx);
+		op[v * 3 + 1] = rotated_point(qx, qy, qz, R[1], R[4], R[7], ty);
+		op[v * 3 + 2] = rotated_point(qx, qy, qz, R[2], R[5], R[8], tz);
 	}
 }
 
@@ -66,12 +52,12 @@
 		if (v >= V) break;
 		const float ux = vp[v * 3 + 0] + dp[v * 3 + 0], uy = vp[v * 3 + 1] + dp[v * 3 + 1], uz = vp[v * 3 + 2] + dp[v * 3 + 2];
 		const float gx = gp[v * 3 + 0], gy = gp[v * 3 + 1], gz = gp[v * 3 + 2];
-		const float dqx = gx * R[0] + gy * R[1] + gz * R[2];
-		const float dqy = gx * R[3] + gy * R[4] + gz * R[5];
-		const float dqz = gx * R[6] + gy * R[7] + gz * R[8];
-		ddp[v * 3 + 0] = dqx * sx;
-		ddp[v * 3 + 1] = dqy * sy;
-		ddp[v * 3 + 2] = dqz * sz;
+		const float dqx = rotated_grad(gx, gy, gz, R[0], R[1], R[2]);
+		const float dqy = rotated_grad(gx, gy, gz, R[3], R[4], R[5]);
+		const float dqz = rotated_grad(gx, gy, gz, R[6], R[7], R[8]);
+		ddp[v * 3 + 0] = disp_grad(dqx, sx);
+		ddp[v * 3 + 1] = disp_grad(dqy, sy);
+		ddp[v * 3 + 2] = disp_grad(dqz, sz);
 		acc[0] += gx; acc[1] += gy; acc[2] += gz;
 		acc[3] += ux * dqx; acc[4] += uy * dqy; acc[5] += uz * dqz;
 		const float qx = ux * sx, qy = uy * sy, qz = uz * sz;
@@ -131,6 +117,18 @@
 	}
 }
 
+int64_t register_partial_floats(int64_t n_feet, int64_t n_pts) { return n_feet * cdiv(n_pts, VPB) * 16; }
+
+int launch_register_bwd(const float* verts, int64_t verts_foot_stride, const float* disp, const float* reg, const float* d_out,
+						int64_t n_feet, int64_t n_pts, float* d_disp, float* d_reg, float* partial, hipStream_t stream) {
+	const int nblk = (int)cdiv(n_pts, VPB);
+	dim3 grid((unsigned)nblk, (unsigned)n_feet);
+	hipLaunchKernelGGL(register_bwd_kernel, grid, dim3(256), 0, stream, verts, verts_foot_stride, disp, reg, d_out, (int)n_pts, d_disp, partial);
+	hipLaunchKernelGGL(register_finalize_kernel, dim3((unsigned)n_feet), dim3(64), 0, stream, reg, partial, nblk, d_reg);
+	FIND_LAUNCH_CHECK("register_bwd");
+	return FIND_OK;
+}
+
 }
 }
 
@@ -149,7 +147,7 @@
 }
 
 extern "C" int64_t find_register_bwd_ws_bytes(int64_t n_feet, int64_t n_pts) {
-	return align_up(n_feet * cdiv(n_pts, reg::VPB) * 16 * (int64_t)sizeof(float), 256);
+	return align_up(reg::register_partial_floats(n_feet, n_pts) * (int64_t)sizeof(float), 256);
 }
 
 extern "C" int find_register_bwd(const float* verts, int64_t verts_batch, const float* disp, const float* reg,
@@ -162,12 +160,6 @@
 		set_error("find_register_bwd: workspace too small");
 		return FIND_EWORKSPACE;
 	}
-	hipStream_t s = reinterpret_cast<hipStream_t>(stream);
-	const int nblk = (int)cdiv(n_pts, reg::VPB);
-	dim3 grid((unsigned)nblk, (unsigned)n_feet);
-	hipLaunchKernelGGL(reg::register_bwd_kernel, grid, dim3(256), 0, s, verts, verts_batch == 1 ? 0 : n_pts * 3, disp, reg, d_out,
-					   (int)n_pts, d_disp, reinterpret_cast<float*>(ws));
-	hipLaunchKernelGGL(reg::register_finalize_kernel, dim3((unsigned)n_feet), dim3(64), 0, s, reg, reinterpret_cast<const float*>(ws), nblk, d_reg);
-	FIND_LAUNCH_CHECK("register_bwd");
-	return FIND_OK;
+	return reg::launch_register_bwd(verts, verts_batch == 1 ? 0 : n_pts * 3, disp, reg, d_out, n_feet, n_pts, d_disp, d_reg, reinterpret_cast<float*>(ws),
+									reinterpret_cast<hipStream_t>(stream));
 }
diff --git a/find_amd/csrc/register_math.h b/find_amd/csrc/register_math.h
--- /dev/null
+++ b/find_amd/csrc/register_math.h
@@ -0,0 +1,79 @@
+#pragma once
+#include "common.h"
+
+namespace find {
+namespace reg {
+
+__device__ __forceinline__ void euler_xyz(const float* e, float* R) {
+	float s0, c0, s1, c1, s2, c2;
+	sincosf(e[0], &s0, &c0);
+	sincosf(e[1], &s1, &c1);
+	sincosf(e[2], &s2, &c2);
+	R[0] = c1 * c2;                  R[1] = -c1 * s2;                 R[2] = s1;
+	R[3] = c0 * s2 + s0 * s1 * c2;   R[4] = c0 * c2 - s0 * s1 * s2;   R[5] = -s0 * c1;
+	R[6] = s0 * s2 - c0 * s1 * c2;   R[7] = s0 * c2 + c0 * s1 * s2;   R[8] = c0 * c1;
+}
+
+__device__ __forceinline__ float scaled_point(float v, float d, float s) { return (v + d) * s; }
+__device__ __forceinline__ float rotated_point(float qx, float qy, float qz, float r0, float r1, float r2, float t) {
+	return qx * r0 + qy * r1 + qz * r2 + t;
+}
+
+__device__ __forceinline__ float rotated_grad(float gx, float gy, float gz, float r0, float r1, float r2) { return gx * r0 + gy * r1 + gz * r2; }
+__device__ __forceinline__ float disp_grad(float dq, float s) { return dq * s; }
+
+namespace pinned {
+__device__ __forceinline__ float mul(float a, float b) {
+#pragma clang fp contract(off)
+	return a * b;
+}
+__device__ __forceinline__ float add(float a, float b) {
+#pragma clang fp contract(off)
+	return a + b;
+}
+__device__ __forceinline__ float sub(float a, float b) {
+#pragma clang fp contract(off)
+	return a - b;
+}
+__device__ __forceinline__ float fma(float a, float b, float c) { return __builtin_fmaf(a, b, c); }
+
+__device__ __forceinline__ void euler_xyz(const float* e, float* R) {
+	float s0, c0, s1, c1, s2, c2;
+	sincosf(e[0], &s0, &c0);
+	sincosf(e[1], &s1, &c1);
+	sincosf(e[2], &s2, &c2);
+	const float s0s1 = mul(s0, s1), c0s1 = mul(c0, s1);
+	R[0] = mul(c1, c2);                         R[1] = mul(-c1, s2);                            R[2] = s1;
+	R[3] = fma(s0s1, c2, mul(c0, s2));          R[4] = sub(mul(c0, c2), mul(s0s1, s2));         R[5] = mul(-s0, c1);
+	R[6] = fma(-c0s1, c2, mul(s0, s2));         R[7] = add(mul(s0, c2), mul(c0s1, s2));         R[8] = mul(c0, c1);
+}
+__device__ __forceinline__ float scaled_point(float v, float d, float s) { return mul(add(v, d), s); }
+__device__ __forceinline__ float rotated_point(float qx, float qy, float qz, float r0, float r1, float r2, float t) {
+	return add(fma(qz, r2, fma(qx, r0, mul(qy, r1))), t);
+}
+__device__ __forceinline__ float disp_grad(int c, float gx, float gy, float gz, float r0, float r1, float r2, float s) {
+	const float dq0 = add(fma(gy, r1, mul(gx, r0)), mul(gz, r2));
+	const float dq12 = fma(gz, r2, fma(gx, r0, mul(gy, r1)));
+	return mul(c == 0 ? dq0 : dq12, s);
+}
+}
+
+constexpr int REG_TAB = 16;
+constexpr int REG_FOLD_MAX_FEET = 64;
+__device__ __forceinline__ void build_reg_table(const float* __restrict__ reg, int n_feet, float* tab) {
+	if ((int)threadIdx.x < n_feet) {
+		const float* rg = reg + (int64_t)threadIdx.x * 9;
+		float* t = tab + threadIdx.x * REG_TAB;
+		pinned::euler_xyz(rg + 3, t);
+		t[9] = rg[0]; t[10] = rg[1]; t[11] = rg[2];
+		t[12] = rg[6]; t[13] = rg[7]; t[14] = rg[8];
+	}
+	__syncthreads();
+}
+
+int launch_register_bwd(const float* verts, int64_t verts_foot_stride, const float* disp, const float* reg, const float* d_out,
+						int64_t n_feet, int64_t n_pts, float* d_disp, float* d_reg, float* partial, hipStream_t stream);
+int64_t register_partial_floats(int64_t n_feet, int64_t n_pts);
+
+}
+}
diff --git a/find_amd/functional.py b/find_amd/functional.py
--- a/find_amd/functional.py
+++ b/find_amd/functional.py
@@ -129,16 +129,16 @@
 class _MLP(torch.autograd.Function):
 
 	@staticmethod
-	def forward(ctx, spec, pos, lat_disp, lat_col, B, avg_col, *weights):
+	def forward(ctx, spec, pos, lat_disp, lat_col, B, avg_col, reg, template, *weights):
 		spec, heads, defer = spec if isinstance(spec, tuple) else (spec, 3, False)
 		if len(weights) != spec.n_weights:
 			raise RuntimeError(f'find_amd.mlp: expected {spec.n_weights} weight tensors, got {len(weights)}')
-		_require_gpu(pos, lat_disp, lat_col, B, avg_col, *weights)
+		_require_gpu(pos, lat_disp, lat_col, B, avg_col, reg, template, *weights)
 		if pos.requires_grad:
 			raise RuntimeError('find_amd.mlp: gradient w.r.t. positions is not part of the FIND path (template / sampled '
 							   'GT points carry no grad, model.py:285, losses.py:39-51)')
 		L = _lib.lib()
-		pos, lat_disp, lat_col, B, avg_col = _c(pos), _c(lat_disp), _c(lat_col), _c(B), _c(avg_col)
+		pos, lat_disp, lat_col, B, avg_col, reg, template = _c(pos), _c(lat_disp), _c(lat_col), _c(B), _c(avg_col), _c(reg), _c(template)
 		leaves = all(w.is_leaf for w in weights)
 		weights = tuple(w.contiguous() for w in weights)
 		if pos.dim() != 3 or pos.shape[-1] != spec.in_dim:
@@ -168,8 +168,22 @@
 		ws = _ws(nbytes, pos.device)
 		disp = torch.empty(n_feet, V, 3, device=pos.device, dtype=torch.float32) if heads & 1 else None
 		col = torch.empty(n_feet, V, 3, device=pos.device, dtype=torch.float32) if heads & 2 else None
-		check(L.find_mlp_fwd(_lib.ctx(pos.device), ctypes.byref(p), ptr(pos), pos_batch, n_feet, V, ptr(lat_disp), ptr(lat_col), ptr(disp), ptr(col),
-							 ptr(ws), ws.numel(), int(save), current_stream(pos.device)), 'find_mlp_fwd')
+		verts = None
+		if reg is not None and disp is not None:
+			if template.requires_grad:
+				raise RuntimeError('find_amd.mlp: template vertices carry no gradient in FIND (model.py:285)')
+			if template.dim() != 3 or template.shape[0] not in (1, n_feet) or tuple(template.shape[1:]) != (V, 3) or tuple(reg.shape) != (n_feet, 9):
+				raise RuntimeError(f'find_amd.mlp: bad shapes template {tuple(template.shape)} reg {tuple(reg.shape)} for {n_feet} feet x {V} points')
+			verts = torch.empty_like(disp)
+			folded = ctypes.c_int32(0)
+			check(L.find_mlp_fwd_reg(_lib.ctx(pos.device), ctypes.byref(p), ptr(pos), pos_batch, n_feet, V, ptr(lat_disp), ptr(lat_col), ptr(disp), ptr(col),
+									 ptr(reg), ptr(template), template.shape[0], ptr(verts), ctypes.byref(folded),
+									 ptr(ws), ws.numel(), int(save), current_stream(pos.device)), 'find_mlp_fwd_reg')
+			if not folded.value:
+				verts = None
+		else:
+			check(L.find_mlp_fwd(_lib.ctx(pos.device), ctypes.byref(p), ptr(pos), pos_batch, n_feet, V, ptr(lat_disp), ptr(lat_col), ptr(disp), ptr(col),
+								 ptr(ws), ws.numel(), int(save), current_stream(pos.device)), 'find_mlp_fwd')
 		if save:
 			ctx.spec = spec
 			ctx.precision = p.precision
@@ -178,24 +192,29 @@
 			ctx.leaves = leaves
 			ctx.defer = bool(defer)
 			ctx.set_materialize_grads(False)
-			ctx.save_for_backward(pos, lat_disp, lat_col, B, avg_col, *weights)
-		return disp, col
-
-	@staticmethod
-	def backward(ctx, g_disp, g_col):
+			ctx.folded = verts is not None
+			if ctx.folded:
+				ctx.save_for_backward(pos, lat_disp, lat_col, B, avg_col, reg, template, disp, *weights)
+			else:
+				ctx.save_for_backward(pos, lat_disp, lat_col, B, avg_col, None, None, None, *weights)
+		return disp, col, verts
+
+	@staticmethod
+	def backward(ctx, g_disp, g_col, g_verts):
 		L = _lib.lib()
 		spec = ctx.spec
-		pos, lat_disp, lat_col, B, avg_col, *weights = ctx.saved_tensors
+		pos, lat_disp, lat_col, B, avg_col, reg, template, disp, *weights = ctx.saved_tensors
 		pos_batch, n_feet, V = ctx.dims
-		g_disp, g_col = _c(g_disp), _c(g_col)
+		g_disp, g_col, g_verts = _c(g_disp), _c(g_col), _c(g_verts)
+		read_d = g_disp is not None or g_verts is not None
 		p = _fill_params(spec, B, avg_col, weights)
 		p.precision = ctx.precision
 		nt, nd = 2 * spec.n_trunk, 2 * (spec.n_disp + 1)
-		frozen = not any(ctx.needs_input_grad[6:])
+		frozen = not any(ctx.needs_input_grad[8:])
 		live = [False] * len(weights)
-		if not frozen and (g_disp is not None or g_col is not None):
+		if not frozen and (read_d or g_col is not None):
 			live[:nt] = [True] * nt
-			if g_disp is not None:
+			if read_d:
 				live[nt:nt + nd] = [True] * nd
 			if g_col is not None:
 				live[nt + nd:] = [True] * (len(weights) - nt - nd)
@@ -206,14 +225,15 @@
 		task = _graph_task_id()
 		key = tuple(w.data_ptr() for w in weights)
 		pending = _PENDING_WGRADS.get(key)
-		can_park = ctx.leaves and not torch.is_grad_enabled() and task >= 0 and all(ctx.needs_input_grad[6:])
+		can_park = ctx.leaves and not torch.is_grad_enabled() and task >= 0 and all(ctx.needs_input_grad[8:])
 		cur = torch.cuda.current_stream(pos.device)
 		fold = pending is not None and can_park and pending[0] == task
 		cross = fold and pending[2] != cur
-		g_lat_disp = torch.empty_like(lat_disp) if (lat_disp is not None and g_disp is not None and ctx.needs_input_grad[2]) else None
+		g_lat_disp = torch.empty_like(lat_disp) if (lat_disp is not None and read_d and ctx.needs_input_grad[2]) else None
 		g_lat_col = torch.empty_like(lat_col) if (lat_col is not None and g_col is not None and ctx.needs_input_grad[3]) else None
-		if not idx and g_lat_disp is None and g_lat_col is None:
-			return (None,) * (6 + len(weights))
+		d_reg = torch.empty_like(reg) if (g_verts is not None and ctx.needs_input_grad[6]) else None
+		if not idx and g_lat_disp is None and g_lat_col is None and d_reg is None:
+			return (None,) * (8 + len(weights))
 		G = MlpGrads()
 		it = iter(grads)
 		for i in range(spec.n_trunk):
@@ -235,9 +255,15 @@
 						 and (not getattr(w, '_post_accumulate_grad_hooks', None) or getattr(w, '_find_hooks_are_stream_safe', False)) for w in weights))
 		if defer:
 			check(L.find_ctx_set(h, b'defer_join', 1), 'find_ctx_set(defer_join)')
-		check(L.find_mlp_bwd(h, ctypes.byref(p), ptr(pos), pos_batch, n_feet, V, ptr(lat_disp), ptr(lat_col), ptr(g_disp), ptr(g_col),
-							 ptr(ctx.ws), ctx.ws.numel(), ptr(scratch), scratch.numel(), ctypes.byref(G),
-							 current_stream(pos.device)), 'find_mlp_bwd')
+		if g_verts is not None:
+			check(L.find_mlp_bwd_reg(h, ctypes.byref(p), ptr(pos), pos_batch, n_feet, V, ptr(lat_disp), ptr(lat_col), ptr(g_disp), ptr(g_col), ptr(g_verts),
+									 ptr(reg), ptr(template), template.shape[0], ptr(disp), ptr(d_reg),
+									 ptr(ctx.ws), ctx.ws.numel(), ptr(scratch), scratch.numel(), ctypes.byref(G),
+									 current_stream(pos.device)), 'find_mlp_bwd_reg')
+		else:
+			check(L.find_mlp_bwd(h, ctypes.byref(p), ptr(pos), pos_batch, n_feet, V, ptr(lat_disp), ptr(lat_col), ptr(g_disp), ptr(g_col),
+								 ptr(ctx.ws), ctx.ws.numel(), ptr(scratch), scratch.numel(), ctypes.byref(G),
+								 current_stream(pos.device)), 'find_mlp_bwd')
 		if defer and _lib.get_tuning('pending', pos.device):
 			bases = {id(g._base): g._base for g in grads if g is not None and g._base is not None}
 			_hold_until_join(pos.device, [scratch, ctx.ws, g_disp, g_col, pos, lat_disp, lat_col, *weights, *bases.values()])
@@ -259,13 +285,13 @@
 				else:
 					torch._foreach_add_([slots[i][0][slots[i][1]:slots[i][1] + grads[i].numel()].view(grads[i].shape) for i in both], [grads[i] for i in both])
 			out = [None if slots[i] is not None else grads[i] for i in range(len(weights))]
-			return (None, None, g_lat_disp, g_lat_col, None, None, *out)
+			return (None, None, g_lat_disp, g_lat_col, None, None, d_reg, None, *out)
 		_PENDING_WGRADS.clear()
 		if can_park and idx and all(grads[i]._base is not None and grads[i]._base.dim() == 1 for i in idx):
 			done = torch.cuda.Event()
 			done.record(cur)
 			_PENDING_WGRADS[key] = (task, [(g._base, g.storage_offset()) if g is not None else None for g in grads], cur, done)
-		return (None, None, g_lat_disp, g_lat_col, None, None, *grads)
+		return (None, None, g_lat_disp, g_lat_col, None, None, d_reg, None, *grads)
 
 
 import os as _os
@@ -321,11 +347,15 @@
 	return int(f()) if f is not None else -1
 
 
-def mlp(spec, pos, lat_disp, lat_col, B, avg_col, weights, want=('disp', 'col'), defer_wgrad_join=False):
+def mlp(spec, pos, lat_disp, lat_col, B, avg_col, weights, want=('disp', 'col'), defer_wgrad_join=False, reg=None, template=None):
 	heads = (1 if 'disp' in want else 0) | (2 if 'col' in want else 0)
 	if heads == 0:
 		raise ValueError("find_amd.mlp: want must name 'disp', 'col' or both")
-	return _MLP.apply((spec, heads, defer_wgrad_join), pos, lat_disp, lat_col, B, avg_col, *weights)
+	if reg is None:
+		return _MLP.apply((spec, heads, defer_wgrad_join), pos, lat_disp, lat_col, B, avg_col, None, None, *weights)[:2]
+	if template is None:
+		raise ValueError('find_amd.mlp: reg needs the template vertices')
+	return _MLP.apply((spec, heads, defer_wgrad_join), pos, lat_disp, lat_col, B, avg_col, reg, template, *weights)
 
 
 class _LatentGather(torch.autograd.Function):
diff --git a/find_amd/model.py b/find_amd/model.py
--- a/find_amd/model.py
+++ b/find_amd/model.py
@@ -403,7 +403,7 @@
 			return None
 		return vecs[0] if len(vecs) == 1 else torch.cat(vecs, dim=-1)
 
-	def forward(self, pos, shapevec=None, texvec=None, posevec=None, want=('disp', 'col'), defer_wgrad_join=False):
+	def forward(self, pos, shapevec=None, texvec=None, posevec=None, want=('disp', 'col'), defer_wgrad_join=False, reg=None):
 		if self.onnx_mode:
 			raise NotImplementedError('onnx_mode (web export) is out of scope')
 		if pos.dim() != 3 or pos.shape[-1] != self.input_dim:
@@ -418,8 +418,11 @@
 		enc = self.encoder[0] if len(self.encoder) else None
 		B = enc.B(pos.device) if enc is not None else None
 		avg = self.avg_col if self.use_avg_colour else None
-		disp, col = FN.mlp(self._spec, pos, lat_disp, lat_col, B, avg, self._weights(), want=want, defer_wgrad_join=defer_wgrad_join)
-		return {k: v for k, v in (('disp', disp), ('col', col)) if v is not None}
+		if reg is not None and 'disp' in want:
+			disp, col, verts = FN.mlp(self._spec, pos, lat_disp, lat_col, B, avg, self._weights(), want=want, defer_wgrad_join=defer_wgrad_join, reg=reg, template=pos)
+		else:
+			(disp, col), verts = FN.mlp(self._spec, pos, lat_disp, lat_col, B, avg, self._weights(), want=want, defer_wgrad_join=defer_wgrad_join), None
+		return {k: v for k, v in (('disp', disp), ('col', col), ('verts', verts)) if v is not None}
 
 	def get_meshes(self, shapevec=None, reg=None, texvec=None, posevec=None, no_displacement=False, include_texture=True, lazy_colours=False):
 		N = 0 if shapevec is None else shapevec.shape[0]
@@ -430,12 +433,12 @@
 			raise NotImplementedError('use_texvec=False: the template-texture fallback of get_meshes does not exist upstream either (model.py:288-295, 500)')
 		if lazy_colours:
 			cell = _Once(lambda: self(tv, shapevec=shapevec, texvec=texvec, posevec=posevec, want=('col',))['col'])
-			res = _LazyColours(self(tv, shapevec=shapevec, texvec=texvec, posevec=posevec, want=('disp',)), cell)
+			res = _LazyColours(self(tv, shapevec=shapevec, texvec=texvec, posevec=posevec, want=('disp',), reg=reg), cell)
 		else:
-			res = self(tv, shapevec=shapevec, texvec=texvec, posevec=posevec)
+			res = self(tv, shapevec=shapevec, texvec=texvec, posevec=posevec, reg=reg)
 		offsets = res['disp']
 		if reg is not None:
-			X = FN.register_points(tv, offsets, reg)
+			X = res['verts'] if 'verts' in res else FN.register_points(tv, offsets, reg)
 		else:
 			X = tv + offsets
 		if not no_displacement:
diff --git a/include/find_hip.h b/include/find_hip.h
--- a/include/find_hip.h
+++ b/include/find_hip.h
@@ -71,6 +71,15 @@
 				 const void* ws, int64_t ws_bytes, void* scratch, int64_t scratch_bytes,
 				 const find_mlp_grads* grads, void* stream);
 
+int find_mlp_fwd_reg(find_ctx* ctx, const find_mlp_params* p, const float* pos, int64_t pos_batch, int64_t n_feet, int64_t n_pts,
+					 const float* lat_disp, const float* lat_col, float* disp, float* col, const float* reg, const float* tmpl,
+					 int64_t tmpl_batch, float* verts, int32_t* folded, void* ws, int64_t ws_bytes, int save_for_bwd, void* stream);
+int find_mlp_bwd_reg(find_ctx* ctx, const find_mlp_params* p, const float* pos, int64_t pos_batch, int64_t n_feet, int64_t n_pts,
+					 const float* lat_disp, const float* lat_col, const float* d_disp, const float* d_col, const float* d_verts,
+					 const float* reg, const float* tmpl, int64_t tmpl_batch, const float* disp, float* d_reg,
+					 const void* ws, int64_t ws_bytes, void* scratch, int64_t scratch_bytes,
+					 const find_mlp_grads* grads, void* stream);
+
 int find_ctx_join(find_ctx* ctx, void* stream);
 
 int find_linear_relu_fwd(find_ctx* ctx, const float* x, const float* w, const float* b, int64_t n_feet, int64_t n_pts, float* y, void* stream);
```

Result: no change. 70.70 million vertices*views/s (-0.3%).
